# NUS-HPC-AI-Lab/VideoSys

Hardware: AMD Instinct MI355X
Metric: videos/min (Open-Sora 512x512x64f, 30 denoise steps, DiT denoising only) + sec/denoise-step (higher is better)
Workload: dtype bf16; 1 GPU; open-sora-v1.2 STDiT3-XL/2 512x512x64f, latent [4,19,64,64], CFG batch 2 = 38912 token rows, 300 text tokens, depth 28; steps_per_video=30, parallelism=dsp1

## Files before the change

### include/videosys_amd.h

```cpp
#ifndef VIDEOSYS_AMD_H
#define VIDEOSYS_AMD_H

#include <stdint.h>

#ifdef __cplusplus
extern "C" {
#endif

#define VSYS_ABI_VERSION 1

#define VSYS_ERR_SHAPE  (-1)
#define VSYS_ERR_ALIGN  (-2)
#define VSYS_ERR_ARG    (-3)
#define VSYS_ERR_LAUNCH (-4)

#define VSYS_EPI_BIAS      0
#define VSYS_EPI_BIAS_GELU 1
#define VSYS_EPI_GATE_RES  2

#define VSYS_ACT_NONE      0
#define VSYS_ACT_SILU      1
#define VSYS_ACT_GELU_TANH 2

int vsys_abi_version(void);
const char* vsys_strerror(int code);
int vsys_device_count(void);

int vsys_tune_gemm_variant(int variant);
int vsys_tune_flash_variant(int variant);
int vsys_gemm_raster_probe(int64_t tile, int64_t nbm, int64_t nbn, int64_t gw, int64_t ph, int64_t* bm, int64_t* bn);

int vsys_gemm_bf16(const void* x, int64_t ldx, const void* w, int64_t ldw, const void* bias, void* out, int64_t ldo,
                   int64_t M, int64_t N, int64_t K, int epilogue, const void* gate, int64_t gate_sample_stride,
                   int64_t rows_per_sample, const void* res, int64_t ldr, void* aux, int64_t ldaux, void* stream);

int vsys_gemm_bf16_ln(const void* x, int64_t ldx, const void* wp, int64_t ldw, const void* cs, const void* cv, void* out, int64_t ldo,
                      int64_t M, int64_t N, int64_t K, int epilogue, const void* stats, int64_t stats_ld, float eps, void* stream);

int vsys_gemm_bf16_ln_qkv_kv(const void* x, int64_t ldx, const void* wp, int64_t ldw, const void* cs, const void* cv, const void* stats,
                             int64_t stats_ld, const void* k_norm_w, void* q, int64_t ldq, void* kp, void* vt, int64_t M, int64_t K,
                             int64_t S, int64_t heads, float eps, float k_eps, void* stream);
int vsys_gemm_bf16_ln_qkv_kv_dispatched(int64_t M, int64_t N, int64_t K);

int vsys_gemm_bf16_stats(const void* x, int64_t ldx, const void* w, int64_t ldw, const void* bias, void* out, int64_t ldo, int64_t M,
                         int64_t N, int64_t K, const void* gate, int64_t gate_sample_stride, int64_t rows_per_sample, const void* res,
                         int64_t ldr, void* stats, int64_t stats_ld, void* stream);

int vsys_gemm_bf16_gate_res_add(const void* x, int64_t ldx, const void* w, int64_t ldw, const void* bias, void* out, int64_t ldo,
                                int64_t M, int64_t N, int64_t K, const void* gate, int64_t gate_sample_stride, int64_t rows_per_sample,
                                const void* res, int64_t ldr, void* aux, const void* add1, const void* add2, void* stats,
                                int64_t stats_ld, void* stream);

int vsys_adaln_prescale(const void* sites, int64_t nsites, int64_t nblocks, const void* mod, void* stream);

int vsys_ln_row_stats(const void* x, int64_t rows, int64_t C, void* stats, int64_t stats_ld, void* stream);

int vsys_linear_small(const void* x, int64_t ldx, const void* w, int64_t ldw, const void* bias, void* out, int64_t ldo,
                      int64_t M, int64_t N, int64_t K, int act_in, int act_out, void* stream);

int vsys_adaln_modulate(const void* x, const void* shift, const void* scale, void* y, int64_t rows, int64_t C,
                        int64_t rows_per_sample, int64_t mod_sample_stride, float eps, void* stream);

int vsys_mod_table(const void* table, const void* t_mlp, void* out, int64_t nblk, int64_t B, int64_t C6, void* stream);

int vsys_timestep_embedding(const void* t_f32, void* out, int64_t B, int64_t dim, void* stream);

int vsys_patch_embed(const void* z_f32, int64_t Bz, const void* w, const void* bias, const void* pos, void* out, int64_t B,
                     int64_t Cin, int64_t T, int64_t H, int64_t W, int64_t ph, int64_t pw, int64_t C, void* stream);

int vsys_final_layer(const void* x, const void* table, const void* tvec, const void* w, const void* bias, void* out_f32,
                     int64_t B, int64_t T, int64_t Hp, int64_t Wp, int64_t H, int64_t W, int64_t ph, int64_t pw,
                     int64_t Cout, int64_t C, float eps, void* stream);

int vsys_patch_embed_shard(const void* z_f32, int64_t Bz, const void* w, const void* bias, const void* pos, void* out, int64_t B,
                           int64_t Cin, int64_t T, int64_t H, int64_t W, int64_t ph, int64_t pw, int64_t C, int64_t s0, int64_t Sl,
                           void* stream);
int vsys_final_layer_tokens(const void* x, const void* table, const void* tvec, const void* w, const void* bias, void* tokens_f32,
                            int64_t B, int64_t T, int64_t Sl, int64_t n_out, int64_t C, float eps, void* stream);
int vsys_unpatchify_tokens(const void* tokens_f32, void* out_f32, int64_t P, int64_t B, int64_t T, int64_t Sl, int64_t Hp,
                           int64_t Wp, int64_t H, int64_t W, int64_t ph, int64_t pw, int64_t Cout, void* stream);

int vsys_cfg_euler_step(void* z_f32, const void* model_out_f32, int64_t Bz, int64_t Cin, int64_t Cout, int64_t thw,
                        float guidance, float dt, void* stream);

int vsys_cfg_linear_step(void* z_f32, const void* model_out_f32, int64_t Bz, int64_t Cin, int64_t Cout, int64_t thw,
                         float guidance, float c_z, float c_eps, int cond_first, void* stream);

int vsys_add_bcast_rows(void* x, const void* e, int64_t rows, int64_t C, int64_t group, int64_t period, void* stream);

int vsys_add_rows(void* x, const void* y, int64_t n, void* stream);

int vsys_copy_4d(const void* src, void* dst, int64_t n0, int64_t n1, int64_t n2, int64_t C, int64_t ss0, int64_t ss1,
                 int64_t ss2, int64_t ds0, int64_t ds1, int64_t ds2, int64_t n1_valid, int64_t n2_valid, void* stream);

// ... 252 lines not shown
```

### videosys_amd/_opcodes.py

```python
OPCODES = {
    "vsys_gemm_bf16": 1,
    "vsys_linear_small": 2,
    "vsys_adaln_modulate": 3,
    "vsys_mod_table": 4,
    "vsys_timestep_embedding": 5,
    "vsys_patch_embed": 6,
    "vsys_final_layer": 7,
    "vsys_cfg_euler_step": 8,
    "vsys_add_rows": 9,
    "vsys_copy_4d_batch": 10,
    "vsys_attn_prep_kv": 11,
    "vsys_flash_attn_d72": 12,
    "vsys_attn_temporal_d72": 13,
    "vsys_add_bcast_rows": 14,
    "vsys_gemm_bf16_gate2": 15,
    "vsys_ln_modulate": 16,
    "vsys_gate_add_rows": 17,
    "vsys_attn_prep_kv64": 18,
    "vsys_flash_attn_d64": 19,
    "vsys_patch_embed_shard": 20,
    "vsys_final_layer_tokens": 21,
    "vsys_unpatchify_tokens": 22,
    "vsys_gemm_bf16_ln": 23,
    "vsys_gemm_bf16_stats": 24,
    "vsys_adaln_prescale": 25,
    "vsys_ln_row_stats": 26,
    "vsys_gemm_bf16_gate_res_add": 27,
    "vsys_flash_attn_d72_kb": 28,
    "vsys_flash_attn_d64_kb": 29,
    "vsys_flash_attn_d72_exact": 30,
    "vsys_p2p_exchange": 31,
    "vsys_cfg_linear_step": 32,
    "vsys_copy_4d": 33,
    "vsys_im2col_patch": 34,
    "vsys_unpatchify_cvx": 35,
    "vsys_gather_rows": 36,
    "vsys_rms_norm_rows": 37,
    "vsys_geglu": 38,
    "vsys_splitk_reduce_t": 39,
    "vsys_t5_attention": 40,
    "vsys_gemm_skinny_slices": 41,
    "vsys_splitk_reduce": 42,
    "vsys_t5_attention_mfma": 43,
    "vsys_conv_bf16": 44,
    "vsys_gn_stats": 45,
    "vsys_gn_apply": 46,
    "vsys_regrid": 47,
    "vsys_subsample": 48,
    "vsys_spatial_norm_apply": 49,
    "vsys_blend_edge": 50,
    "vsys_d2s_time": 51,
    "vsys_vae_first_im2col": 52,
    "vsys_extract_planar": 53,
    "vsys_softmax_rows": 54,
    "vsys_attn_prep_kv_varlen": 55,
    "vsys_flash_attn_d72_varlen": 56,
    "vsys_gemm_bf16_ln_qkv_kv": 57,
    "vsys_attn_temporal_d64": 58,
    "vsys_scale_add_rows": 59,
}
N_INT, N_FLOAT = 23, 3
ENTRY_POINTS = {
    "vsys_abi_version": ("", "i"),
    "vsys_strerror": ("i", "s"),
    "vsys_device_count": ("", "i"),
    "vsys_tune_gemm_variant": ("i", "i"),
    "vsys_tune_flash_variant": ("i", "i"),
    "vsys_gemm_raster_probe": ("lllllpp", "i"),
    "vsys_gemm_bf16": ("plplppllllipllplplp", "i"),
    "vsys_gemm_bf16_ln": ("plplppplllliplfp", "i"),
    "vsys_gemm_bf16_ln_qkv_kv": ("plplppplpplppllllffp", "i"),
    "vsys_gemm_bf16_ln_qkv_kv_dispatched": ("lll", "i"),
    "vsys_gemm_bf16_stats": ("plplppllllpllplplp", "i"),
    "vsys_gemm_bf16_gate_res_add": ("plplppllllpllplpppplp", "i"),
    "vsys_adaln_prescale": ("pllpp", "i"),
    "vsys_ln_row_stats": ("pllplp", "i"),
    "vsys_linear_small": ("plplpplllliip", "i"),
    "vsys_adaln_modulate": ("ppppllllfp", "i"),
    "vsys_mod_table": ("ppplllp", "i"),
    "vsys_timestep_embedding": ("ppllp", "i"),
    "vsys_patch_embed": ("plppppllllllllp", "i"),
    "vsys_final_layer": ("ppppppllllllllllfp", "i"),
    "vsys_patch_embed_shard": ("plppppllllllllllp", "i"),
    "vsys_final_layer_tokens": ("pppppplllllfp", "i"),
    "vsys_unpatchify_tokens": ("pplllllllllllp", "i"),
    "vsys_cfg_euler_step": ("ppllllffp", "i"),
    "vsys_cfg_linear_step": ("ppllllfffip", "i"),
    "vsys_add_bcast_rows": ("ppllllp", "i"),
    "vsys_add_rows": ("pplp", "i"),
    "vsys_copy_4d": ("ppllllllllllllp", "i"),
    "vsys_attn_prep_kv": ("plplpppllllfp", "i"),
    "vsys_flash_attn_d72": ("plppppllllllfp", "i"),
    "vsys_flash_attn_d72_exact": ("plppppllllllfp", "i"),
    "vsys_attn_prep_kv_varlen": ("plplppppplllfp", "i"),
    "vsys_flash_attn_d72_varlen": ("plpppppplllllfp", "i"),
    "vsys_flash_attn_d72_kb": ("plppppllllllffp", "i"),
    "vsys_gemm_bf16_gate2": ("plplppllllpllllplplp", "i"),
    "vsys_ln_modulate": ("ppppppllllllfp", "i"),
    "vsys_gate_add_rows": ("pppllllllp", "i"),
    "vsys_im2col_patch": ("plpllllllp", "i"),
    "vsys_unpatchify_cvx": ("plpllllllp", "i"),
    "vsys_attn_prep_kv64": ("plplppppllppllllfp", "i"),
    "vsys_flash_attn_d64": ("plppppllpppllllllfp", "i"),
    "vsys_flash_attn_d64_kb": ("plppppllpppllllllffp", "i"),
    "vsys_attn_prep_kv96": ("plplppppllllp", "i"),
    "vsys_flash_attn_d96": ("plppppppllllllp", "i"),
    "vsys_attn_prep_kv96_img": ("plplppppllllllp", "i"),
    "vsys_flash_attn_d96_img": ("plpppppplllllllllp", "i"),
    "vsys_attn_prep_kv_rope": ("plplppppllllp", "i"),
    "vsys_flash_attn_d72_rope": ("plpppppllllllp", "i"),
    "vsys_attn_temporal_d72": ("pllppppplllllfp", "i"),
    "vsys_attn_temporal_d64": ("plplplplplplppplpllllllp", "i"),
    "vsys_attn_temporal_d64_img": ("plplplplplplppplplllllllllp", "i"),
    "vsys_scale_add_rows": ("plplplllfp", "i"),
    "vsys_copy_4d_batch": ("pplpp", "i"),
    "vsys_p2p_exchange": ("plppllplp", "i"),
    "vsys_p2p_alloc": ("llp", "i"),
    "vsys_p2p_free": ("p", "i"),
    "vsys_p2p_ipc_export": ("pp", "i"),
    "vsys_p2p_ipc_open": ("pp", "i"),
    "vsys_p2p_ipc_close": ("p", "i"),
    "vsys_gather_rows": ("ppplllp", "i"),
    "vsys_rms_norm_rows": ("pppllfp", "i"),
    "vsys_geglu": ("ppllp", "i"),
# ... 33 lines not shown
```

### videosys_amd/csrc/adaln_fold.hip

```cpp
#include "common.h"
#include "vsys_internal.h"

namespace vsys {
namespace {

constexpr int SITE_WORDS = 10;

__global__ __launch_bounds__(256) void adaln_prescale_kernel(const int64_t* __restrict__ sites, int nsites,
                                                             const bf16_t* __restrict__ mod) {
  const int lane = threadIdx.x & 63, wave = threadIdx.x >> 6;
  int lo = 0, hi = nsites - 1;
  while (lo < hi) {
    const int mid = (lo + hi + 1) >> 1;
    if (sites[(int64_t)mid * SITE_WORDS + 9] <= (int64_t)blockIdx.x) lo = mid;
    else hi = mid - 1;
  }
  const int64_t* s = sites + (int64_t)lo * SITE_WORDS;
  const bf16_t* W = reinterpret_cast<const bf16_t*>(s[0]);
  const bf16_t* bias = reinterpret_cast<const bf16_t*>(s[1]);
  bf16_t* Wp = reinterpret_cast<bf16_t*>(s[2]);
  float* cs = reinterpret_cast<float*>(s[3]);
  float* cv = reinterpret_cast<float*>(s[4]);
  const bf16_t* shift = mod + s[5];
  const bf16_t* scale = mod + s[6];
  const int N = (int)(s[7] & 0xffffffff), kv_heads = (int)(s[7] >> 32), K = (int)s[8];
  const int n = ((int)blockIdx.x - (int)s[9]) * 4 + wave;
  if (n >= N) return;
  const int nd = (kv_heads > 0 && N == 216 * kv_heads && kv_heads % 4 == 0) ? qkv_kv_column(n, kv_heads) : n;
  const bf16_t* wr = W + (int64_t)n * K;
  bf16_t* wo = Wp + (int64_t)nd * K;
  float a_cs = 0.f, a_cv = 0.f;
  for (int c = lane; c < (K >> 3); c += 64) {
    float w[8], sc[8], sh[8], o[8];
    unpack8(*reinterpret_cast<const uint4*>(wr + c * 8), w);
    unpack8(*reinterpret_cast<const uint4*>(scale + c * 8), sc);
    unpack8(*reinterpret_cast<const uint4*>(shift + c * 8), sh);
#pragma unroll
    for (int e = 0; e < 8; ++e) {
      o[e] = w[e] * (1.0f + sc[e]);
      a_cv = fmaf(sh[e], w[e], a_cv);
    }
    const uint4 pk = pack8(o);
    *reinterpret_cast<uint4*>(wo + c * 8) = pk;
    float r[8];
    unpack8(pk, r);
#pragma unroll
    for (int e = 0; e < 8; ++e) a_cs += r[e];
  }
  a_cs = wave_sum(a_cs);
  a_cv = wave_sum(a_cv);
  if (lane == 0) {
    cs[nd] = a_cs;
    cv[nd] = a_cv + (bias != nullptr ? bf2f(bias[n]) : 0.f);
  }
}

__global__ __launch_bounds__(256) void ln_row_stats_kernel(const bf16_t* __restrict__ x, int64_t rows, int C, float2* __restrict__ stats,
                                                           int64_t ld) {
  const int lane = threadIdx.x & 63;
  const int64_t row = ((int64_t)blockIdx.x * 4 + (threadIdx.x >> 6)) * 2 + (lane >> 5);
  const int q = lane & 31, b = q >> 1, hi = q & 1;
  const bool act = row < rows && b * LN_BLOCK < C;
  const bf16_t* xr = x + (act ? row : 0) * C + (act ? b : 0) * LN_BLOCK + 4 * hi;
  uint2 u[12];
#pragma unroll
  for (int j = 0; j < 3; ++j)
#pragma unroll
    for (int g = 0; g < 4; ++g) u[4 * j + g] = *reinterpret_cast<const uint2*>(xr + 32 * j + 8 * g);
  LnAcc a;
  a.init(bflo(u[0].x));
#pragma unroll
  for (int k = 0; k < 12; ++k) {
    a.add(bflo(u[k].x)); a.add(bfhi(u[k].x)); a.add(bflo(u[k].y)); a.add(bfhi(u[k].y));
  }
  const float2 mine = a.finish(48.f);
  const float2 other = make_float2(__shfl_xor(mine.x, 1, 64), __shfl_xor(mine.y, 1, 64));
  const float2 blk = ln_merge_equal(mine, other, 48.f);
  if (act && hi == 0) stats[(int64_t)b * ld + row] = blk;
}

}
// ... 17 lines not shown
```

### videosys_amd/csrc/attention.hip

```cpp
#include "common.h"
#include "vsys_internal.h"

#include <cstdlib>
#include <type_traits>

namespace vsys {
namespace {

constexpr int HD = 72;
constexpr int HD_ROWS = 96;
constexpr int KROW = 144;
constexpr int VROW = 128;
constexpr int K_TILE_BYTES = 64 * KROW;
constexpr int V_TILE_BYTES = HD_ROWS * VROW;
constexpr int KV_STAGE = K_TILE_BYTES + V_TILE_BYTES;
constexpr float NEG_BIG = -1.0e30f;

template <int N>
__device__ __forceinline__ void rope_pairs(float* x, const float* c, const float* s) {
#pragma clang fp contract(off)
#pragma unroll
  for (int e = 0; e < N; ++e) {
    const float a = x[2 * e], bb = x[2 * e + 1];
    const float ac = a * c[e], bs = bb * s[e], bc = bb * c[e], as = a * s[e];
// ... 50 lines not shown
    }
    KNorm72::apply(x, rstd, k_norm_w != nullptr ? k_norm_w + part * 24 : nullptr, kscale);
    if (active) {
      bf16_t* dst = kp + (((int64_t)bh * kv_pad) + s) * HD + part * 24;
#pragma unroll
      for (int c = 0; c < 3; ++c) *reinterpret_cast<uint4*>(dst + c * 8) = pack8(x + c * 8);
    }
  }
  __syncthreads();

  for (int q = tid; q < HD * 8; q += 256) {
    const int d = q >> 3, c = q & 7;
    uint4 o;
    uint32_t w[4];
#pragma unroll
    for (int e = 0; e < 4; ++e) w[e] = (uint32_t)vs[c * 8 + 2 * e][d] | ((uint32_t)vs[c * 8 + 2 * e + 1][d] << 16);
    o.x = w[0]; o.y = w[1]; o.z = w[2]; o.w = w[3];
    *reinterpret_cast<uint4*>(vt + ((int64_t)bh * HD_ROWS + d) * kv_pad + s0 + c * 8) = o;
  }
  if (tid < 16) {
    const int d = HD + 4 * (tid >> 3), c = tid & 7;
    uint32_t w[4];
#pragma unroll
    for (int e = 0; e < 4; ++e) {
      const int k0 = s0 + c * 8 + 2 * e;
      w[e] = (k0 < kv_len ? 0x3f80u : 0u) | (k0 + 1 < kv_len ? 0x3f800000u : 0u);
    }
    uint4 o;
    o.x = w[0]; o.y = w[1]; o.z = w[2]; o.w = w[3];
    *reinterpret_cast<uint4*>(vt + ((int64_t)bh * HD_ROWS + d) * kv_pad + s0 + c * 8) = o;
  }
}

struct FlashParams {
  const bf16_t* q; int64_t q_stride;
  union {
    const bf16_t* q_norm_w;
    const float* rope_cos;
  };
  const bf16_t* kp;
  const bf16_t* vt;
  bf16_t* out; int64_t out_stride;
  int heads, q_len, kv_len, kv_pad, nqb;
  int chunks;
  float eps;
  unsigned long long* dbg;
  union {
    const int* kv_lens;
    const float* rope_sin;
  };
};

constexpr int ABL_ROPE = 7;
constexpr int RES_MAX_TILES = 5;
constexpr int RES_Q_BYTES = 5 * 1024;
template <int ABL, int WPS, bool RES = false, bool EXACT = false, bool VARLEN = false>
__global__ __launch_bounds__(RES ? 512 : 256, RES ? 2 : WPS) void flash_attn_d72_kernel(FlashParams p) {
#if __HIP_DEVICE_COMPILE__
  extern __shared__ __attribute__((aligned(16))) char smem[];
  const int tid = threadIdx.x, lane = tid & 63, wave = tid >> 6;
  const int l31 = lane & 31, hi = lane >> 5;
  const int tile_id = xcd_remap(blockIdx.x, gridDim.x);
  const int bh = RES ? tile_id / p.chunks : tile_id / p.nqb;
  const int qb = RES ? tile_id - bh * p.chunks : tile_id - bh * p.nqb;
  const int b = bh / p.heads, h = bh - b * p.heads;
  constexpr int NW = RES ? 8 : 4;
  int q0 = qb * 128 + wave * 32;
  int kv_len_ = p.kv_len;
  if constexpr (VARLEN) {
    static_assert(RES && EXACT, "per-sample key counts: resident-K/V kernel with the padding promise only");
    const int cap = p.kv_pad < RES_MAX_TILES * 64 ? p.kv_pad : RES_MAX_TILES * 64;
    const int n = __builtin_amdgcn_readfirstlane(p.kv_lens[b]);
    kv_len_ = n < 1 ? 1 : (n > cap ? cap : n);
  }
  const int kv_len = kv_len_;

  const int wave_u = __builtin_amdgcn_readfirstlane(wave);
  const bf16_t* kbase = p.kp + (int64_t)bh * p.kv_pad * HD;
  const bf16_t* vbase = p.vt + (int64_t)bh * HD_ROWS * p.kv_pad;
  const auto rsrc_k = __builtin_amdgcn_make_buffer_rsrc((void*)kbase, 0, p.kv_pad * HD * 2, 0x00020000);
  const auto rsrc_v = __builtin_amdgcn_make_buffer_rsrc((void*)vbase, 0, HD_ROWS * p.kv_pad * 2, 0x00020000);
  typedef __attribute__((address_space(3))) void* lds_ptr_t;
  const int k_voff = lane * 16;
  const int v_voff = (lane >> 3) * p.kv_pad * 2 + (((lane & 7) ^ (lane >> 4)) << 4);
  const bool s4k = wave_u == 0;
  const int s4j = wave_u == 1 ? 8 : 9;
  const auto rsrc_4 = __builtin_amdgcn_make_buffer_rsrc((void*)(s4k ? kbase : vbase), 0, s4k ? p.kv_pad * HD * 2 : HD_ROWS * p.kv_pad * 2,
                                                        0x00020000);
  const int voff_4 = s4k ? k_voff : (v_voff ^ ((s4j & 1) << 6));
  const int soff_4 = s4k ? 8 * 1024 : s4j * 8 * p.kv_pad * 2, step_4 = s4k ? K_TILE_BYTES : 128;
  const int lds_4 = s4k ? 8 * 1024 : K_TILE_BYTES + s4j * 1024;
  auto stage = [&](int t, int buf) {
    char* base = smem + buf * KV_STAGE;
    if constexpr (RES) {
#pragma unroll
      for (int idx = 0; idx < 3; ++idx) {
        const int piece = wave_u + NW * idx;
        if (piece < 9) {
          __builtin_amdgcn_raw_ptr_buffer_load_lds(rsrc_k, (lds_ptr_t)(base + piece * 1024), 16, k_voff, t * K_TILE_BYTES + piece * 1024, 0, 0);
        } else if (piece < 19) {
          const int j = piece - 9;
          __builtin_amdgcn_raw_ptr_buffer_load_lds(rsrc_v, (lds_ptr_t)(base + K_TILE_BYTES + j * 1024), 16, v_voff ^ ((j & 1) << 6),
                                                   j * 8 * p.kv_pad * 2 + t * 128, 0, 0);
        }
      }
    } else {
// ... 12 lines not shown
    }
  };
  const int ntiles = (kv_len + 63) / 64;
  if constexpr (RES) {
    for (int t = 0; t < ntiles; ++t) stage(t, t);
    for (int q = tid; q < ntiles * 128; q += 512)
      *reinterpret_cast<uint4*>(smem + (q >> 7) * KV_STAGE + K_TILE_BYTES + 80 * VROW + (q & 127) * 16) = make_uint4(0, 0, 0, 0);
  } else {
    stage(0, 0);
    char* z = smem + (tid >> 7) * KV_STAGE + K_TILE_BYTES + 80 * VROW + (tid & 127) * 16;
    *reinterpret_cast<uint4*>(z) = make_uint4(0, 0, 0, 0);
  }

  bf16x8 qf[5];
  uint4 qraw[5];
  float4 qcs[5], qsn[5];
  auto fetch_q = [&](int q0_) {
    int qs = q0_ + l31;
    qs = qs < p.q_len ? qs : p.q_len - 1;
    const bf16_t* qrow = p.q + ((int64_t)b * p.q_len + qs) * p.q_stride + h * HD;
#pragma unroll
    for (int c = 0; c < 5; ++c) {
      const int d0 = 16 * c + 8 * hi;
      qraw[c] = d0 < HD ? *reinterpret_cast<const uint4*>(qrow + d0) : make_uint4(0, 0, 0, 0);
    }
    if constexpr (ABL == ABL_ROPE) {
      static_assert(ABL != ABL_ROPE || !RES, "the rotation lives in the streaming kernel's prologue only");
#pragma unroll
      for (int c = 0; c < 5; ++c) {
        const int d0 = 16 * c + 8 * hi;
        qcs[c] = qsn[c] = make_float4(0.f, 0.f, 0.f, 0.f);
        if (d0 < HD) {
          qcs[c] = *reinterpret_cast<const float4*>(p.rope_cos + (int64_t)qs * (HD / 2) + (d0 >> 1));
          qsn[c] = *reinterpret_cast<const float4*>(p.rope_sin + (int64_t)qs * (HD / 2) + (d0 >> 1));
        }
      }
    }
  };
  auto finish_q = [&]() {
    if constexpr (ABL == ABL_ROPE) {
#pragma unroll
      for (int c = 0; c < 5; ++c) {
        float x[8];
        unpack8(qraw[c], x);
        rope_pairs<1>(x + 0, &qcs[c].x, &qsn[c].x);
        rope_pairs<1>(x + 2, &qcs[c].y, &qsn[c].y);
        rope_pairs<1>(x + 4, &qcs[c].z, &qsn[c].z);
        rope_pairs<1>(x + 6, &qcs[c].w, &qsn[c].w);
#pragma unroll
        for (int e = 0; e < 8; ++e) qf[c][e] = (__bf16)x[e];
      }
      return;
    }
    if (p.q_norm_w == nullptr) {
#pragma unroll
      for (int c = 0; c < 5; ++c) qf[c] = __builtin_bit_cast(bf16x8, qraw[c]);
      return;
    }
    float x[5][8];
    float ss = 0.f;
#pragma unroll
    for (int c = 0; c < 5; ++c) {
      unpack8(qraw[c], x[c]);
#pragma unroll
      for (int e = 0; e < 8; ++e) ss += x[c][e] * x[c][e];
    }
    {
      ss += __shfl_xor(ss, 32, 64);
      const float rstd = rsqrtf(ss / (float)HD + p.eps);
#pragma unroll
      for (int c = 0; c < 5; ++c) {
        const int d0 = 16 * c + 8 * hi;
        if (d0 < HD) {
          float w[8];
          unpack8(*reinterpret_cast<const uint4*>(p.q_norm_w + d0), w);
#pragma unroll
          for (int e = 0; e < 8; ++e) x[c][e] = bf2f(f2bf(x[c][e] * rstd)) * w[e];
        }
      }
    }
#pragma unroll
    for (int c = 0; c < 5; ++c)
#pragma unroll
      for (int e = 0; e < 8; ++e) qf[c][e] = (__bf16)x[c][e];
  };
  if constexpr (!RES) { fetch_q(q0); finish_q(); }

  const int v_roff = K_TILE_BYTES + l31 * VROW + (((2 * hi) ^ ((l31 >> 1) & 7)) << 4);

  const int krow = 16 * ((l31 >> 2) & 1) + 4 * (l31 >> 3) + (l31 & 3);

  f32x16 o[3];
  f32x16 minit;
  auto reset_acc = [&]() {
#pragma unroll
    for (int dt = 0; dt < 3; ++dt)
#pragma unroll
      for (int r = 0; r < 16; ++r) o[dt][r] = 0.f;
#pragma unroll
    for (int r = 0; r < 16; ++r) minit[r] = 0.f;
  };
  reset_acc();
  asm volatile("s_waitcnt vmcnt(0)" ::: "memory");
  __syncthreads();

  const float defer_thr = 8.0f;

// ... 254 lines not shown
          for (int cc = 0; cc < 2; ++cc)
#pragma unroll
            for (int dt = 0; dt < 3; ++dt) o[dt] = __builtin_amdgcn_mfma_f32_32x32x16_bf16(vf1[cc][dt], pa1[cc], o[dt], 0, 0, 0);
          float mxn = 0.f;
          if constexpr (has_next) mxn = tile_max(t + 1, sn, next_masked);
#pragma unroll
          for (int i = 0; i < 6; ++i) { RES_SGB(0x008, 1); RES_SGB(0x400, 3); RES_SGB(0x002, 2); }
#pragma unroll
          for (int i = 0; i < 6; ++i) { RES_SGB(0x008, 1); RES_SGB(0x002, 5); }
          __builtin_amdgcn_sched_barrier(0);
          if constexpr (has_next) rescale(t + 1, sn, mxn);
        };
        qk(0, sa);
        __builtin_amdgcn_sched_barrier(0);
        next_q();
        __builtin_amdgcn_sched_barrier(0);
        rescale(0, sa, (ragged && ntiles == 1) ? tile_max(0, sa, true) : tile_max(0, sa, false));
        int t = 0;
        for (; t + 2 < ntiles; t += 2) {
          step(std::true_type{}, t, sa, sb, false);
          step(std::true_type{}, t + 1, sb, sa, ragged && t + 2 == ntiles - 1);
        }
        if (t + 1 < ntiles) {
          step(std::true_type{}, t, sa, sb, ragged);
          step(std::false_type{}, t + 1, sb, sa, false);
        } else {
          step(std::false_type{}, t, sa, sb, false);
        }
#undef RES_SGB
      }
      if constexpr (EXACT) {
        if (__builtin_amdgcn_ballot_w64(!(o[2][4] >= 0x1p-100f)) != 0) {
          asm volatile("; exact-keys guard (cold): masked recompute of this query block" ::: "memory");
          reset_acc();
          for (int t = 0; t < ntiles; ++t) tile(t, t, t == ntiles - 1 && (kv_len & 63) != 0);
        }
      }
      store_o();
    }
  } else {
    if (ABL == 2) tprev = __builtin_amdgcn_s_memtime();
    for (int t = 0; t < ntiles - 1; ++t) {
      const int cur = t & 1;
      if (ABL != 1 && ABL != 5 && !DMA_BESIDE_QK) stage(t + 1, cur ^ 1);
      __builtin_amdgcn_sched_barrier(0);
      tile(t, cur, false, true);
      __builtin_amdgcn_sched_barrier(0);
      if (ABL == 5) { __builtin_amdgcn_sched_barrier(0); continue; }
      asm volatile("s_waitcnt vmcnt(0)" ::: "memory");
      FLASH_STAMP(3);
      __syncthreads();
      FLASH_STAMP(4);
    }
    constexpr bool WHOLE_TILES_ONLY = ABL == ABL_ROPE && WPS == 3;
    if (!WHOLE_TILES_ONLY && (kv_len & 63)) tile(ntiles - 1, (ntiles - 1) & 1, true);
    else tile(ntiles - 1, (ntiles - 1) & 1, false);

    if (ABL == 2 && lane == 0 && p.dbg != nullptr) {
#pragma unroll
      for (int i = 0; i < 5; ++i) atomicAdd(p.dbg + i, tacc[i]);
    }
    store_o();
  }
#undef FLASH_STAMP
#endif
}

__global__ void attn_temporal_d72_kernel(const bf16_t* __restrict__ qkv, int64_t row_stride, int C,
                                         const bf16_t* __restrict__ q_norm_w, const bf16_t* __restrict__ k_norm_w,
                                         const float* __restrict__ rope_cos, const float* __restrict__ rope_sin,
                                         bf16_t* __restrict__ out, int64_t out_stride, int B, int T, int S, int heads,
                                         int wpb, float eps, float scale) {
  extern __shared__ __attribute__((aligned(16))) char smem[];
  const int lane = threadIdx.x & 63, wave = threadIdx.x >> 6;
  const int hgroups = (heads + wpb - 1) / wpb;
  const int hg = blockIdx.x % hgroups;
  const int64_t bs = blockIdx.x / hgroups;
  const int s = (int)(bs % S), b = (int)(bs / S);
  const int h = hg * wpb + wave;
  if (h >= heads) return;
  float* ks = reinterpret_cast<float*>(smem) + (size_t)wave * 2 * T * HD;
  float* vs = ks + (size_t)T * HD;
  const int g = lane / 3, part = lane - g * 3;
  const bool lane_ok = lane < 63;
  const int npass = (T + 20) / 21;

  auto norm_rope = [&](float* x, const bf16_t* w, int t) {
    float ss = 0.f;
#pragma unroll
    for (int e = 0; e < 24; ++e) ss += x[e] * x[e];
    const int base = g * 3;
    const float tot = __shfl(ss, base, 64) + __shfl(ss, base + 1, 64) + __shfl(ss, base + 2, 64);
    const float rstd = rsqrtf(tot / (float)HD + eps);
    if (w != nullptr) {
#pragma unroll
      for (int e = 0; e < 24; ++e) x[e] = bf2f(f2bf(bf2f(f2bf(x[e] * rstd)) * bf2f(w[part * 24 + e])));
    }
    if (rope_cos != nullptr) {
      const float* cs = rope_cos + (int64_t)t * HD + part * 24;
      const float* sn = rope_sin + (int64_t)t * HD + part * 24;
#pragma unroll
      for (int e = 0; e < 24; e += 2) {
        const float a = x[e], bb = x[e + 1];
        x[e] = bf2f(f2bf(a * cs[e] - bb * sn[e]));
        x[e + 1] = bf2f(f2bf(bb * cs[e + 1] + a * sn[e + 1]));
      }
    }
// ... 487 lines not shown
  const size_t lds = per_wave * wpb;
  const float scale = 0.11785113019775793f;
  const int g_flash_variant = g_flash_variant_a.load(std::memory_order_relaxed);
  if (T <= 64 && g_flash_variant != 9 && g_flash_variant != 4)
    return launch_attn_temporal_d72_v3(qkv, row_stride, C, q_norm_w, k_norm_w, rope_cos, rope_sin, out, out_stride, B, T, S, heads, eps,
                                       scale, stream,  g_flash_variant == 21,  g_flash_variant == 22);
  if (T <= 20 && g_flash_variant != 9) {
    hipLaunchKernelGGL(attn_temporal_d72_v2_kernel<20>, dim3((unsigned)grid), dim3(64 * wpb), lds, stream, qkv, row_stride, C, q_norm_w,
                       k_norm_w, rope_cos, rope_sin, out, out_stride, B, T, S, heads, wpb, eps, scale);
  } else if (T <= 40 && g_flash_variant != 9) {
    hipLaunchKernelGGL(attn_temporal_d72_v2_kernel<40>, dim3((unsigned)grid), dim3(64 * wpb), lds, stream, qkv, row_stride, C, q_norm_w,
                       k_norm_w, rope_cos, rope_sin, out, out_stride, B, T, S, heads, wpb, eps, scale);
  } else {
    if (lds > 64 * 1024)
      (void)hipFuncSetAttribute((const void*)attn_temporal_d72_kernel, hipFuncAttributeMaxDynamicSharedMemorySize, (int)lds);
    hipLaunchKernelGGL(attn_temporal_d72_kernel, dim3((unsigned)grid), dim3(64 * wpb), lds, stream, qkv, row_stride, C, q_norm_w,
                       k_norm_w, rope_cos, rope_sin, out, out_stride, B, T, S, heads, wpb, eps, scale);
  }
  return hipGetLastError() == hipSuccess ? 0 : VSYS_ERR_LAUNCH;
}

int launch_attn_prep_kv_rope(const bf16_t* k, int64_t k_stride, const bf16_t* v, int64_t v_stride, const float* rope_cos,
                             const float* rope_sin, bf16_t* kp, bf16_t* vt, int batch, int heads, int kv_len, int kv_pad,
                             hipStream_t stream) {
  if (batch <= 0 || heads <= 0 || kv_len <= 0) return 0;
  if (kv_pad % 64 != 0 || kv_pad < kv_len || (k_stride % 8) || (v_stride % 8)) return VSYS_ERR_SHAPE;
  dim3 grid(kv_pad / 64, batch * heads);
  hipLaunchKernelGGL(attn_prep_kv_rope_kernel<false>, grid, dim3(256), 0, stream, k, k_stride, v, v_stride, rope_cos, rope_sin, kp, vt,
                     heads, kv_len, kv_pad, 0.11785113019775793f * 1.4426950408889634f );
  return hipGetLastError() == hipSuccess ? 0 : VSYS_ERR_LAUNCH;
}

int launch_flash_attn_d72_rope(const bf16_t* q, int64_t q_stride, const float* rope_cos, const float* rope_sin, const bf16_t* kp,
                               const bf16_t* vt, bf16_t* out, int64_t out_stride, int batch, int heads, int q_len, int kv_len,
                               int kv_pad, hipStream_t stream) {
  if (batch <= 0 || heads <= 0 || q_len <= 0) return 0;
  if (kv_len <= 0 || kv_pad % 64 != 0 || kv_pad < kv_len || (q_stride % 8) || (out_stride % 4)) return VSYS_ERR_SHAPE;
  FlashParams p;
  p.q = q; p.q_stride = q_stride; p.rope_cos = rope_cos; p.kp = kp; p.vt = vt; p.out = out; p.out_stride = out_stride;
  p.heads = heads; p.q_len = q_len; p.kv_len = kv_len; p.kv_pad = kv_pad; p.eps = 0.f;
  p.rope_sin = rope_sin;
  p.dbg = nullptr;
  p.nqb = (q_len + 127) / 128;
  p.chunks = 1;
  const int64_t nblk = (int64_t)p.nqb * batch * heads;
  if (nblk > 0x7fffffff) return VSYS_ERR_SHAPE;
  const size_t lds = 2 * KV_STAGE;
  static const bool wps3_ok = [] { const char* e = getenv("VSYS_FLASH_WPS3"); return !(e && e[0] == '0'); }();
  if (wps3_ok && kv_len >= 512 && (kv_len & 63) == 0) hipLaunchKernelGGL((flash_attn_d72_kernel<ABL_ROPE, 3>), dim3((unsigned)nblk), dim3(256), lds, stream, p);
  else hipLaunchKernelGGL((flash_attn_d72_kernel<ABL_ROPE, 2>), dim3((unsigned)nblk), dim3(256), lds, stream, p);
  return hipGetLastError() == hipSuccess ? 0 : VSYS_ERR_LAUNCH;
}

}
```

### videosys_amd/csrc/attention_w64.hip

```cpp
#include "flash_w64.h"

namespace vsys {
namespace {

using w64::VROW;
using w64::make_rsrc;
using w64::u32x4;
constexpr int HD = 72, HD_ROWS = 96, KROW = 144;
constexpr int K_TILE_BYTES = 64 * KROW;
constexpr int KV_STAGE = K_TILE_BYTES + HD_ROWS * VROW;
constexpr int W64_STAGES = w64::STAGES;

struct FlashW64Params {
  const bf16_t* q; int64_t q_stride;
  const bf16_t* q_norm_w;
  const bf16_t* kp;
  const bf16_t* vt;
  bf16_t* out; int64_t out_stride;
  int heads, q_len, kv_len, kv_pad, nqb;
  float eps;
  float k_bound;
  unsigned long long* dbg;
};

// ... 95 lines not shown
  else if constexpr (VAR == 10)
    asm volatile(FLASH72_W64_ASM_V10 : W64_STAMPS : FLASH72_W64_OPERANDS : FLASH72_W64_CLOBBERS_PHASE);
  else if constexpr (VAR == 8) W64_LOOP(FLASH72_W64_ASM_V8);
  else if constexpr (VAR == 9) W64_LOOP(FLASH72_W64_ASM_V9);
#endif
#undef W64_STAMPS
#undef W64_LOOP

#pragma unroll
  for (int blk = 0; blk < 2; ++blk) {
    float o[3][16];
    if (blk == 0) FLASH72_W64_READ_O_A(o);
    else FLASH72_W64_READ_O_B(o);
    const float inv = 1.0f / o[2][4];
    const int qs = q0 + 32 * blk + l31;
    bf16_t* orow = p.out + ((int64_t)b * p.q_len + (qs < p.q_len ? qs : p.q_len - 1)) * p.out_stride + h * HD + 8 * hi;
#pragma unroll
    for (int dt = 0; dt < 3; ++dt) {
      uint2 w[4];
#pragma unroll
      for (int g = 0; g < 4; ++g) {
        w[g].x = pack2bf(o[dt][4 * g + 0] * inv, o[dt][4 * g + 1] * inv);
        w[g].y = pack2bf(o[dt][4 * g + 2] * inv, o[dt][4 * g + 3] * inv);
      }
#pragma unroll
      for (int k = 0; k < 2; ++k) {
        const auto sx = __builtin_amdgcn_permlane32_swap(w[2 * k].x, w[2 * k + 1].x, false, false);
        const auto sy = __builtin_amdgcn_permlane32_swap(w[2 * k].y, w[2 * k + 1].y, false, false);
        const int d0 = dt * 32 + 16 * k;
        if (qs < p.q_len && d0 + 8 * hi + 8 <= HD) *reinterpret_cast<uint4*>(orow + d0) = make_uint4(sx[0], sy[0], sx[1], sy[1]);
      }
    }
  }
  if constexpr (VAR == 7 || VAR == 10) {
    asm volatile("s_waitcnt vmcnt(0)" ::: "memory");
    stamp[5] = __builtin_amdgcn_s_memtime();
    if (lane == 0 && p.dbg != nullptr) {
      unsigned long long* d = p.dbg + ((size_t)blockIdx.x * 4 + wave) * 8;
#pragma unroll
      for (int i = 0; i < 6; ++i) d[i] = stamp[i];
    }
  }
#endif
}

constexpr int W64P_QIMG = 64 * KROW;

__device__ __forceinline__ unsigned long long uniform_addr(const void* ptr) {
  const unsigned long long a = reinterpret_cast<unsigned long long>(ptr);
  const unsigned lo = __builtin_amdgcn_readfirstlane((unsigned)a), hi_ = __builtin_amdgcn_readfirstlane((unsigned)(a >> 32) & 0xffffu);
  return ((unsigned long long)hi_ << 32) | lo;
}

template <bool STAMP, bool SM = false>
__global__ __launch_bounds__(256, 1) void flash_attn_d72_w64p_kernel(FlashW64Params p, int total_items) {
#if __HIP_DEVICE_COMPILE__
  extern __shared__ __attribute__((aligned(16))) char smem[];
  const int tid = threadIdx.x, lane = tid & 63, wave = tid >> 6;
  const int l31 = lane & 31, hi = lane >> 5;
  const int wave_u = __builtin_amdgcn_readfirstlane(wave);
  const int wgp = xcd_remap(blockIdx.x, gridDim.x), istep = (int)gridDim.x;
  const int i0 = wgp, i1 = total_items;
  if (i0 >= i1) return;

  const unsigned kbytes = (unsigned)(p.kv_pad * HD * 2), vbytes = (unsigned)(HD_ROWS * p.kv_pad * 2);
  const bool s4k = wave_u == 0;
  const int s4j = wave_u == 1 ? 8 : 9;
  const int kvo = lane * 16;
  const int v_voff0 = (lane >> 3) * p.kv_pad * 2 + (((lane & 7) ^ (lane >> 4)) << 4);
  const int vvo = v_voff0 ^ ((wave_u & 1) << 6);
  const int v4o = s4k ? kvo : (v_voff0 ^ ((s4j & 1) << 6));
  const int wl = wave_u * 1024, kvp2 = p.kv_pad * 2;
  const int s4 = s4k ? 8 * 1024 : s4j * 8 * p.kv_pad * 2, st4 = s4k ? K_TILE_BYTES : 128;
  const int l4 = s4k ? 8 * 1024 : K_TILE_BYTES + s4j * 1024;
  const int lb = w64::lds_base(smem);
  const int qlds = lb + W64_STAGES * KV_STAGE + wave_u * W64P_QIMG;
  const int nt = p.kv_len >> 6;
  for (int u = tid; u < W64_STAGES * 128; u += 256)
    *reinterpret_cast<uint4*>(smem + (u >> 7) * KV_STAGE + K_TILE_BYTES + 80 * VROW + (u & 127) * 16) = make_uint4(0, 0, 0, 0);
  const int kfa = w64::frag_krow(l31) * KROW + 16 * hi;
  const w64::VtFrag vf = w64::vt_frag<K_TILE_BYTES>(l31, hi);
  const int vfa0 = vf.vfa0, vfa1 = vf.vfa1, vfa2 = vf.vfa2, vfa3 = vf.vfa3;

  auto item_bh = [&](int it) { return it / p.nqb; };
  auto q_rsrc = [&](int it) {
    const int bh = item_bh(it), b = bh / p.heads, h = bh - b * p.heads;
    return make_rsrc(p.q + (int64_t)b * p.q_len * p.q_stride + h * HD, (unsigned)((int64_t)p.q_len * p.q_stride * 2));
  };
  auto q_row_voff = [&](int it) {
    const int qb = it - item_bh(it) * p.nqb;
    int r = qb * 256 + wave * 64 + lane;
    r = r < p.q_len ? r : p.q_len - 1;
    return r * (int)p.q_stride * 2;
  };
  typedef __attribute__((address_space(3))) void* lds_ptr_t;

  {
    const int bh = item_bh(i0);
    const bf16_t* kbase = p.kp + (int64_t)bh * p.kv_pad * HD;
    const bf16_t* vbase = p.vt + (int64_t)bh * HD_ROWS * p.kv_pad;
    const auto rk = __builtin_amdgcn_make_buffer_rsrc((void*)kbase, 0, (int)kbytes, 0x00020000);
    const auto rv = __builtin_amdgcn_make_buffer_rsrc((void*)vbase, 0, (int)vbytes, 0x00020000);
    const int bq = bh / p.heads, hq = bh - bq * p.heads;
    const auto rq = __builtin_amdgcn_make_buffer_rsrc((void*)(p.q + (int64_t)bq * p.q_len * p.q_stride + hq * HD), 0,
                                                      (int)((int64_t)p.q_len * p.q_stride * 2), 0x00020000);
    const int qv = q_row_voff(i0);
#pragma unroll
    for (int pc = 0; pc < 9; ++pc)
      __builtin_amdgcn_raw_ptr_buffer_load_lds(rq, (lds_ptr_t)(smem + W64_STAGES * KV_STAGE + wave_u * W64P_QIMG + pc * 1024), 16, qv, pc * 16, 0, 0);
#pragma unroll
    for (int t = 0; t < 4; ++t) {
      char* st = smem + t * KV_STAGE;
      __builtin_amdgcn_raw_ptr_buffer_load_lds(rk, (lds_ptr_t)(st + wl), 16, kvo, t * K_TILE_BYTES + wl, 0, 0);
      __builtin_amdgcn_raw_ptr_buffer_load_lds(rk, (lds_ptr_t)(st + wl + 4096), 16, kvo, t * K_TILE_BYTES + wl + 4096, 0, 0);
      __builtin_amdgcn_raw_ptr_buffer_load_lds(rv, (lds_ptr_t)(st + K_TILE_BYTES + wl), 16, vvo, wave_u * 8 * kvp2 + t * 128, 0, 0);
      __builtin_amdgcn_raw_ptr_buffer_load_lds(rv, (lds_ptr_t)(st + K_TILE_BYTES + wl + 4096), 16, vvo, (wave_u + 4) * 8 * kvp2 + t * 128, 0, 0);
      if (s4k) __builtin_amdgcn_raw_ptr_buffer_load_lds(rk, (lds_ptr_t)(st + l4), 16, v4o, s4 + t * st4, 0, 0);
      else __builtin_amdgcn_raw_ptr_buffer_load_lds(rv, (lds_ptr_t)(st + l4), 16, v4o, s4 + t * st4, 0, 0);
    }
  }

  uint4 qnw[5];
#pragma unroll
  for (int c = 0; c < 5; ++c) {
    const int d0 = 16 * c + 8 * hi;
    qnw[c] = (p.q_norm_w != nullptr && d0 < HD) ? *reinterpret_cast<const uint4*>(p.q_norm_w + d0) : make_uint4(0, 0, 0, 0);
  }
  unsigned long long acc[8] = {0, 0, 0, 0, 0, 0, 0, 0}, ta = 0, tb = 0;
  int ring = 0;
  for (int it = i0; it < i1; it += istep) {
    const int bh = item_bh(it), qb = it - bh * p.nqb;
    const int b = bh / p.heads, h = bh - b * p.heads;
    const int q0 = qb * 256 + wave_u * 64;
    unsigned long long t0 = 0, t1 = 0, t2 = 0, t3 = 0, t4 = 0;
    if constexpr (STAMP) t0 = __builtin_amdgcn_s_memtime();
    asm volatile("s_waitcnt vmcnt(0)" ::: "memory");
    if constexpr (STAMP) t1 = __builtin_amdgcn_s_memtime();
    uint4 qw[2][5];
    float nmv[2] = {0.f, 0.f};
#pragma unroll
    for (int blk = 0; blk < 2; ++blk) {
      const char* qimg = smem + W64_STAGES * KV_STAGE + wave_u * W64P_QIMG + (32 * blk + l31) * 16;
      uint4 qraw[5];
#pragma unroll
      for (int c = 0; c < 5; ++c) {
        const int ch = 2 * c + hi;
        qraw[c] = ch < 9 ? *reinterpret_cast<const uint4*>(qimg + ch * 1024) : make_uint4(0, 0, 0, 0);
      }
      float x[5][8];
      float ss = 0.f;
#pragma unroll
      for (int c = 0; c < 5; ++c) {
        unpack8(qraw[c], x[c]);
#pragma unroll
        for (int e = 0; e < 8; ++e) ss += x[c][e] * x[c][e];
      }
      if (p.q_norm_w != nullptr) {
        ss += __shfl_xor(ss, 32, 64);
        const float rstd = rsqrtf(ss / (float)HD + p.eps);
#pragma unroll
        for (int c = 0; c < 5; ++c) {
          const int d0 = 16 * c + 8 * hi;
          if (d0 < HD) {
            float w[8];
            unpack8(qnw[c], w);
#pragma unroll
            for (int e = 0; e < 8; ++e) x[c][e] = bf2f(f2bf(x[c][e] * rstd)) * w[e];
          }
        }
      }
      if constexpr (SM) nmv[blk] = w64::neg_row_bound<5>(x, p.k_bound);
#pragma unroll
      for (int c = 0; c < 5; ++c) qw[blk][c] = pack8(x[c]);
    }
    asm volatile("s_waitcnt lgkmcnt(0)" ::: "memory");
    FLASH72_W64_WRITE_Q_A(qw[0]);
    FLASH72_W64_WRITE_Q_B(qw[1]);
    const float nma = nmv[0], nmb = nmv[1];

    const bool has_next = it + istep < i1;
    const int nit = has_next ? it + istep : it;
    const int nbh = item_bh(nit);
    const unsigned long long kb = uniform_addr(p.kp + (int64_t)bh * p.kv_pad * HD), vb = uniform_addr(p.vt + (int64_t)bh * HD_ROWS * p.kv_pad);
    const unsigned long long kbn = uniform_addr(p.kp + (int64_t)nbh * p.kv_pad * HD), vbn = uniform_addr(p.vt + (int64_t)nbh * HD_ROWS * p.kv_pad);
    const u32x4 rqn = q_rsrc(nit);
    const int qvo = q_row_voff(nit);
    const int hn = __builtin_amdgcn_readfirstlane(has_next ? 1 : 0);
    const int st0 = lb + ring * KV_STAGE, st1 = lb + ((ring + 1) & 3) * KV_STAGE, st2 = lb + ((ring + 2) & 3) * KV_STAGE;
    ring = (ring + nt) & 3;
    if constexpr (STAMP) {
      t2 = __builtin_amdgcn_s_memtime();
#ifdef VSYS_LAB
      asm volatile(FLASH72_W64P_ASM_STAMP : [t0] "=s"(ta), [t1] "=s"(tb) : FLASH72_W64P_OPERANDS : FLASH72_W64_CLOBBERS);
#endif
      t3 = __builtin_amdgcn_s_memtime();
    } else if constexpr (SM)
      asm volatile(FLASH72_W64P_ASM_S : : FLASH72_W64P_OPERANDS_S : FLASH72_W64_CLOBBERS);
    else
      asm volatile(FLASH72_W64P_ASM : : FLASH72_W64P_OPERANDS : FLASH72_W64_CLOBBERS);

// ... 62 lines not shown
  return p;
}

bool flash_w64p_supports(int q_len, int kv_len, int kv_pad, int64_t q_stride) {
  return kv_len >= 256 && kv_len % 64 == 0 && q_len >= 256 && (int64_t)q_len * q_stride * 2 < 0x7fffffff;
}

int launch_flash_attn_d72_w64p(const bf16_t* q, int64_t q_stride, const bf16_t* q_norm_w, const bf16_t* kp, const bf16_t* vt, bf16_t* out,
                               int64_t out_stride, int batch, int heads, int q_len, int kv_len, int kv_pad, float eps, bool stamp,
                               float k_bound, hipStream_t stream) {
  FlashW64Params p = w64_params(q, q_stride, q_norm_w, kp, vt, out, out_stride, heads, q_len, kv_len, kv_pad, eps, k_bound, nullptr);
  const int64_t total = (int64_t)p.nqb * batch * heads;
  if (total > 0x7fffffff) return VSYS_ERR_SHAPE;
  const int ncu = cu_count_this_device();
  const unsigned grid = (unsigned)(total < ncu ? total : ncu);
  const size_t lds = (size_t)W64_STAGES * KV_STAGE + 4 * W64P_QIMG;
  (void)stamp;
#ifdef VSYS_LAB
  if (!stamp)
#endif
    return !(k_bound > 0.f && q_norm_w != nullptr) ? w64::launch<flash_attn_d72_w64p_kernel<false>>(grid, lds, stream, p, (int)total)
                                                    : w64::launch<flash_attn_d72_w64p_kernel<false, true>>(grid, lds, stream, p, (int)total);
#ifdef VSYS_LAB
  p.dbg = reinterpret_cast<unsigned long long*>(get_lab_debug_buffer());
  return w64::launch<flash_attn_d72_w64p_kernel<true>>(grid, lds, stream, p, (int)total);
#endif
}

int launch_flash_attn_d72_w64(const bf16_t* q, int64_t q_stride, const bf16_t* q_norm_w, const bf16_t* kp, const bf16_t* vt, bf16_t* out,
                              int64_t out_stride, int batch, int heads, int q_len, int kv_len, int kv_pad, float eps, int var,
                              float k_bound, hipStream_t stream) {
  const FlashW64Params p = w64_params(q, q_stride, q_norm_w, kp, vt, out, out_stride, heads, q_len, kv_len, kv_pad, eps, k_bound,
                                      reinterpret_cast<unsigned long long*>(get_lab_debug_buffer()));
  const int64_t nblk = (int64_t)p.nqb * batch * heads;
  if (nblk > 0x7fffffff) return VSYS_ERR_SHAPE;
  const size_t lds = (size_t)W64_STAGES * KV_STAGE;
#define W64_CASE(VAR_) w64::launch<flash_attn_d72_w64_kernel<VAR_>>((unsigned)nblk, lds, stream, p)
  switch (var) {
    case 0: return W64_CASE(0);
    case 1: return W64_CASE(1);
    case 3: return W64_CASE(3);
    case 5: return k_bound > 0.f && q_norm_w != nullptr ? W64_CASE(5) : VSYS_ERR_ARG;
#ifdef VSYS_LAB
    case 7: return W64_CASE(7);
    case 10: return W64_CASE(10);
    case 8: return W64_CASE(8);
    case 9: return W64_CASE(9);
#endif
    default: return VSYS_ERR_ARG;
  }
#undef W64_CASE
}

}
```

### videosys_amd/csrc/capi.hip

```cpp
#include "common.h"
#include "vsys_internal.h"

using namespace vsys;

namespace {
inline hipStream_t S(void* s) { return reinterpret_cast<hipStream_t>(s); }
inline const bf16_t* B16(const void* p) { return reinterpret_cast<const bf16_t*>(p); }
inline bf16_t* B16(void* p) { return reinterpret_cast<bf16_t*>(p); }
template <class... T> inline bool fits_int(T... v) { return ((v >= 0 && v <= 0x7fffffff) && ...); }
inline GemmParams gemm_head(const void* a, int64_t lda, const void* w, int64_t ldw, const void* bias, void* out, int64_t ldo, int64_t M,
                            int64_t N, int64_t K) {
  GemmParams p;
  p.A = B16(a); p.lda = lda; p.W = B16(w); p.ldw = ldw; p.bias = B16(bias); p.out = B16(out); p.ldo = ldo;
  p.M = (int)M; p.N = (int)N; p.K = (int)K;
  return p;
}

inline bool to_copy_desc(const int64_t* d, CopyDesc& o) {
  if (!fits_int(d[2], d[3], d[4], d[5], d[12], d[13]) || d[0] < 0 || d[1] < 0) return false;
  o.src_off = d[0]; o.dst_off = d[1];
  o.n0 = (int)d[2]; o.n1 = (int)d[3]; o.n2 = (int)d[4]; o.C = (int)d[5];
  o.ss0 = d[6]; o.ss1 = d[7]; o.ss2 = d[8]; o.ds0 = d[9]; o.ds1 = d[10]; o.ds2 = d[11];
  o.n1_valid = (int)d[12]; o.n2_valid = (int)d[13];
  return true;
// ... 78 lines not shown
  std::vector<int4> v;
  int m = 0;
  if (!sk_plan(ntiles, nt, grid, v, m)) return 0;
  if ((int)v.size() > cap_rows) return VSYS_ERR_ARG;
  for (size_t i = 0; i < v.size(); ++i) {
    segs[4 * i] = v[i].x; segs[4 * i + 1] = v[i].y; segs[4 * i + 2] = v[i].z; segs[4 * i + 3] = v[i].w;
  }
  *nseg_max = m;
  return (int)v.size();
}

int vsys_lab_flash_debug_buffer(void* dev_u64x5) {
  set_flash_debug_buffer(dev_u64x5);
  return 0;
}
#endif

int vsys_gemm_bf16(const void* x, int64_t ldx, const void* w, int64_t ldw, const void* bias, void* out, int64_t ldo,
                   int64_t M, int64_t N, int64_t K, int epilogue, const void* gate, int64_t gate_sample_stride,
                   int64_t rows_per_sample, const void* res, int64_t ldr, void* aux, int64_t ldaux, void* stream) {
  if (!x || !w || !out) return VSYS_ERR_ARG;
  if (!fits_int(M, N, K, rows_per_sample)) return VSYS_ERR_SHAPE;
  if (epilogue != VSYS_EPI_GATE_RES && (gate || res || aux)) return VSYS_ERR_ARG;
  GemmParams p = gemm_head(x, ldx, w, ldw, bias, out, ldo, M, N, K);
  p.gate = B16(gate); p.gate_stride = gate_sample_stride; p.res = B16(res); p.ldr = ldr; p.aux = B16(aux); p.ldaux = ldaux;
  p.rows_per_sample = (int)rows_per_sample;
  return launch_gemm(p, epilogue, S(stream));
}

int vsys_gemm_bf16_ln(const void* x, int64_t ldx, const void* wp, int64_t ldw, const void* cs, const void* cv, void* out, int64_t ldo,
                      int64_t M, int64_t N, int64_t K, int epilogue, const void* stats, int64_t stats_ld, float eps, void* stream) {
  if (!x || !wp || !cs || !cv || !out || !stats) return VSYS_ERR_ARG;
  if (!fits_int(M, N, K)) return VSYS_ERR_SHAPE;
  if (epilogue != VSYS_EPI_BIAS && epilogue != VSYS_EPI_BIAS_GELU) return VSYS_ERR_ARG;
  if (K % LN_BLOCK != 0 || K / LN_BLOCK > 12) return VSYS_ERR_SHAPE;
  GemmParams p = gemm_head(x, ldx, wp, ldw, nullptr, out, ldo, M, N, K);
  p.cs = reinterpret_cast<const float*>(cs); p.cv = reinterpret_cast<const float*>(cv);
  p.ln_stats = reinterpret_cast<const float2*>(stats); p.ln_ld = stats_ld; p.ln_nb = (int)(K / LN_BLOCK); p.ln_eps = eps;
  return launch_gemm(p, epilogue == VSYS_EPI_BIAS ? EPI_LN_BIAS : EPI_LN_GELU, S(stream));
}

int vsys_gemm_bf16_ln_qkv_kv(const void* x, int64_t ldx, const void* wp, int64_t ldw, const void* cs, const void* cv, const void* stats,
                             int64_t stats_ld, const void* k_norm_w, void* q, int64_t ldq, void* kp, void* vt, int64_t M, int64_t K,
                             int64_t S_, int64_t heads, float eps, float k_eps, void* stream) {
  if (!x || !wp || !cs || !cv || !stats || !k_norm_w || !q || !kp || !vt) return VSYS_ERR_ARG;
  if (!fits_int(M, K, S_) || heads <= 0 || heads > 4096) return VSYS_ERR_SHAPE;
  if (K % LN_BLOCK != 0 || K / LN_BLOCK > 12) return VSYS_ERR_SHAPE;
  GemmParams p = gemm_head(x, ldx, wp, ldw, nullptr, q, ldq, M, 216 * heads, K);
  p.cs = reinterpret_cast<const float*>(cs); p.cv = reinterpret_cast<const float*>(cv);
  p.ln_stats = reinterpret_cast<const float2*>(stats); p.ln_ld = stats_ld; p.ln_nb = (int)(K / LN_BLOCK); p.ln_eps = eps;
  p.kp = B16(kp); p.vt = B16(vt); p.k_norm_w = B16(k_norm_w); p.kv_S = (int)S_; p.kv_heads = (int)heads; p.k_eps = k_eps;
  p.kscale = 0.11785113019775793f * 1.4426950408889634f;
  return launch_gemm_qkv_kv(p, S(stream));
}

int vsys_gemm_bf16_ln_qkv_kv_dispatched(int64_t M, int64_t N, int64_t K) { return gemm_ln_qkv_kv_dispatched(M, N, K) ? 1 : 0; }

int vsys_gemm_bf16_stats(const void* x, int64_t ldx, const void* w, int64_t ldw, const void* bias, void* out, int64_t ldo, int64_t M,
                         int64_t N, int64_t K, const void* gate, int64_t gate_sample_stride, int64_t rows_per_sample, const void* res,
                         int64_t ldr, void* stats, int64_t stats_ld, void* stream) {
  if (!x || !w || !out || !stats) return VSYS_ERR_ARG;
  if (!fits_int(M, N, K, rows_per_sample)) return VSYS_ERR_SHAPE;
  GemmParams p = gemm_head(x, ldx, w, ldw, bias, out, ldo, M, N, K);
  p.gate = B16(gate); p.gate_stride = gate_sample_stride; p.res = B16(res); p.ldr = ldr;
  p.rows_per_sample = (int)rows_per_sample;
  p.stats_out = reinterpret_cast<float2*>(stats); p.stats_ld = stats_ld;
  return launch_gemm(p, EPI_GATE_RES_STATS, S(stream));
}

int vsys_gemm_bf16_gate_res_add(const void* x, int64_t ldx, const void* w, int64_t ldw, const void* bias, void* out, int64_t ldo,
                                int64_t M, int64_t N, int64_t K, const void* gate, int64_t gate_sample_stride, int64_t rows_per_sample,
                                const void* res, int64_t ldr, void* aux, const void* add1, const void* add2, void* stats,
                                int64_t stats_ld, void* stream) {
  if (!x || !w || !out || !res) return VSYS_ERR_ARG;
  if (!fits_int(M, N, K, rows_per_sample)) return VSYS_ERR_SHAPE;
  GemmParams p = gemm_head(x, ldx, w, ldw, bias, out, ldo, M, N, K);
  p.gate = B16(gate); p.gate_stride = gate_sample_stride; p.res = B16(res); p.ldr = ldr; p.aux = B16(aux); p.ldaux = ldr;
  p.rows_per_sample = (int)rows_per_sample;
  p.add1 = B16(add1 ? add1 : add2); p.add2 = add1 ? B16(add2) : nullptr;
  p.stats_out = reinterpret_cast<float2*>(stats); p.stats_ld = stats_ld;
  return launch_gemm(p, EPI_GATE_RES, S(stream));
}

int vsys_adaln_prescale(const void* sites, int64_t nsites, int64_t nblocks, const void* mod, void* stream) {
  if (!sites || !mod) return VSYS_ERR_ARG;
  if (!fits_int(nsites)) return VSYS_ERR_SHAPE;
  return launch_adaln_prescale(reinterpret_cast<const int64_t*>(sites), (int)nsites, nblocks, B16(mod), S(stream));
}

int vsys_ln_row_stats(const void* x, int64_t rows, int64_t C, void* stats, int64_t stats_ld, void* stream) {
  if (!x || !stats) return VSYS_ERR_ARG;
  if (!fits_int(C)) return VSYS_ERR_SHAPE;
  return launch_ln_row_stats(B16(x), rows, (int)C, reinterpret_cast<float2*>(stats), stats_ld, S(stream));
}

int vsys_gemm_bf16_gate2(const void* x, int64_t ldx, const void* w, int64_t ldw, const void* bias, void* out, int64_t ldo,
                         int64_t M, int64_t N, int64_t K, const void* gate, int64_t gate_sample_stride,
                         int64_t rows_per_sample, int64_t seg_split, int64_t gate_alt, const void* res, int64_t ldr,
                         void* aux, int64_t ldaux, void* stream) {
  if (!x || !w || !out || !gate) return VSYS_ERR_ARG;
  if (!fits_int(M, N, K, rows_per_sample, seg_split)) return VSYS_ERR_SHAPE;
  if (seg_split < 0 || seg_split > rows_per_sample) return VSYS_ERR_SHAPE;
  GemmParams p = gemm_head(x, ldx, w, ldw, bias, out, ldo, M, N, K);
  p.gate = B16(gate); p.gate_stride = gate_sample_stride; p.res = B16(res); p.ldr = ldr; p.aux = B16(aux); p.ldaux = ldaux;
  p.rows_per_sample = (int)rows_per_sample;
  p.seg_split = (int)seg_split; p.gate_alt = gate_alt;
// ... 642 lines not shown
```

### videosys_amd/csrc/common.h

```cpp
#pragma once
#include <hip/hip_runtime.h>
#include <stdint.h>

namespace vsys {

typedef uint16_t bf16_t;
typedef __attribute__((ext_vector_type(8))) __bf16 bf16x8;
typedef __attribute__((ext_vector_type(4))) __bf16 bf16x4;
typedef __attribute__((ext_vector_type(16))) float f32x16;
typedef __attribute__((ext_vector_type(4))) float f32x4;

__device__ __forceinline__ float bf2f(bf16_t v) { return __uint_as_float(((uint32_t)v) << 16); }
__device__ __forceinline__ bf16_t f2bf(float f) { return __builtin_bit_cast(bf16_t, (__bf16)f); }
__device__ __forceinline__ uint32_t pack2bf(float lo, float hi) {
  return (uint32_t)f2bf(lo) | ((uint32_t)f2bf(hi) << 16);
}
typedef __attribute__((ext_vector_type(2))) float f32x2;
typedef __attribute__((ext_vector_type(2))) __bf16 bf16x2;
__device__ __forceinline__ uint32_t pack2bf(f32x2 v) { return __builtin_bit_cast(uint32_t, __builtin_convertvector(v, bf16x2)); }
__device__ __forceinline__ float bflo(uint32_t u) { return __uint_as_float(u << 16); }
__device__ __forceinline__ float bfhi(uint32_t u) { return __uint_as_float(u & 0xffff0000u); }

__device__ __forceinline__ void unpack8(const uint4& v, float* f) {
  f[0] = bflo(v.x); f[1] = bfhi(v.x); f[2] = bflo(v.y); f[3] = bfhi(v.y);
  f[4] = bflo(v.z); f[5] = bfhi(v.z); f[6] = bflo(v.w); f[7] = bfhi(v.w);
}
__device__ __forceinline__ uint4 pack8(const float* f) {
  uint4 v;
  v.x = pack2bf(f[0], f[1]); v.y = pack2bf(f[2], f[3]); v.z = pack2bf(f[4], f[5]); v.w = pack2bf(f[6], f[7]);
  return v;
}

__device__ __forceinline__ float wave_sum(float v) {
#pragma unroll
  for (int o = 32; o > 0; o >>= 1) v += __shfl_xor(v, o, 64);
  return v;
}
__device__ __forceinline__ float wave_max(float v) {
#pragma unroll
  for (int o = 32; o > 0; o >>= 1) v = fmaxf(v, __shfl_xor(v, o, 64));
  return v;
}

__device__ __forceinline__ float gelu_tanh(float x) {
  const float k0 = 0.7978845608028654f, k1 = 0.044715f;
  const float u = k0 * x * (1.0f + k1 * x * x);
  const float e = __builtin_amdgcn_exp2f(u * -2.8853900817779268f);
  return x * __builtin_amdgcn_rcpf(1.0f + e);
}
__device__ __forceinline__ float silu(float x) { return x / (1.0f + __expf(-x)); }

struct KNorm72 {
  static __device__ __forceinline__ float sumsq(const float* x) {
    float ss = 0.f;
#pragma unroll
    for (int e = 0; e < 24; ++e) ss += x[e] * x[e];
    return ss;
  }
  static __device__ __forceinline__ float rstd(float ss0, float ss1, float ss2, float eps) {
    const float tot = ss0 + ss1 + ss2;
    return rsqrtf(tot / 72.0f + eps);
  }
  static __device__ __forceinline__ void apply(float* x, float rstd_, const bf16_t* w24, float kscale) {
    if (w24 != nullptr) {
#pragma unroll
      for (int e = 0; e < 24; ++e) {
        const float nrm = bf2f(f2bf(x[e] * rstd_));
        x[e] = nrm * bf2f(w24[e]);
      }
    }
#pragma unroll
    for (int e = 0; e < 24; ++e) x[e] *= kscale;
  }
};

__device__ __forceinline__ void ln_combine(const float2* __restrict__ st, int64_t ld, int nb, int64_t row, float eps, float& mu,
                                           float& rstd) {
  float2 v[12];
#pragma unroll
  for (int b = 0; b < 12; ++b) v[b] = b < nb ? st[b * ld + row] : make_float2(0.f, 0.f);
  float sd = 0.f, sdd = 0.f, m2 = v[0].y;
#pragma unroll
  for (int b = 1; b < 12; ++b) {
    if (b < nb) {
      const float d = v[b].x - v[0].x;
      sd += d;
      sdd += d * d;
      m2 += v[b].y;
    }
  }
  const float inv = 1.0f / (float)nb;
  mu = v[0].x + sd * inv;
  m2 += 96.0f * (sdd - sd * sd * inv);
  rstd = rsqrtf(fmaxf(m2, 0.f) / (96.0f * (float)nb) + eps);
}
__device__ __forceinline__ void ln_stage_tile(float2* __restrict__ lds, const float2* __restrict__ st, int64_t ld, int nb, float eps,
                                              int M, int row0, int nrows, const float* __restrict__ cs, const float* __restrict__ cv,
                                              int col0, int ncols, int tid, int nthreads) {
  const int c = nthreads - 1 - tid;
  float c_s = 0.f, c_v = 0.f;
  if (c < ncols) {
    c_s = cs[col0 + c];
    c_v = cv[col0 + c];
  }
  if (tid < nrows) {
    int grow = row0 + tid;
    grow = grow < M ? grow : M - 1;
    float mu, rstd;
    ln_combine(st, ld, nb, grow, eps, mu, rstd);
    lds[tid] = make_float2(mu, rstd);
  }
  if (c < ncols) lds[nrows + c] = make_float2(c_s, c_v);
}

struct LnAcc {
  float p, s1, s2;
  __device__ __forceinline__ void init(float pivot) { p = pivot; s1 = 0.f; s2 = 0.f; }
  __device__ __forceinline__ void add(float x) { const float d = x - p; s1 += d; s2 = fmaf(d, d, s2); }
  __device__ __forceinline__ void add2(f32x2 x) {
    const f32x2 d = x - f32x2{p, p};
    s1 += d.x; s2 = fmaf(d.x, d.x, s2);
    s1 += d.y; s2 = fmaf(d.y, d.y, s2);
  }
  __device__ __forceinline__ float2 finish(float n) const { return make_float2(p + s1 / n, fmaxf(s2 - s1 * s1 / n, 0.f)); }
};
// ... 52 lines not shown
```

### videosys_amd/csrc/gemm2_bf16.hip

```cpp
#include "common.h"
#include "vsys_internal.h"

namespace vsys {
namespace {

constexpr int BM = 256, BK = 32;
constexpr int A_SLOT = BM * BK * 2;
constexpr int W_BASE = 3 * A_SLOT;
constexpr int OUT_ROW_BYTES = 96 * 2 + 16;
constexpr int OUT_WAVE_BYTES = 64 * OUT_ROW_BYTES;

template <int NWN>
struct G2 {
  static constexpr int NW = 2 * NWN;
  static constexpr int NT = 64 * NW;
  static constexpr int BN = 96 * NWN;
  static constexpr int NA = 16 / NW;
  static constexpr int W_SLOT = BN * BK * 2;
  static constexpr int WLEAD = NWN == 4 ? 2 : 1;
  static constexpr int NWSLOT = WLEAD + 1;
  static constexpr int STAGING = W_BASE + NWSLOT * W_SLOT;
  static constexpr int LDS_BYTES = STAGING > NW * OUT_WAVE_BYTES ? STAGING : NW * OUT_WAVE_BYTES;
  static constexpr int LN_BYTES = (BM + BN) * 8;
  static constexpr int KW_BYTES = 160;
};

template <int EPI, int NWN, int STAMP = 0, int MF = 0>
__global__ __launch_bounds__(G2<NWN>::NT, 2) void gemm2_kernel(GemmParams p) {
  using G = G2<NWN>;
  constexpr int BN = G::BN, NA = G::NA, W_SLOT = G::W_SLOT, WLEAD = G::WLEAD;
#if __HIP_DEVICE_COMPILE__
  extern __shared__ __attribute__((aligned(16))) char smem[];
  const int tid = threadIdx.x, lane = tid & 63, wave = tid >> 6;
  const int wm = wave / NWN, wn = wave % NWN;
  const int l31 = lane & 31, hi = lane >> 5;
  const int l15 = lane & 15, lq = lane >> 4;
  static_assert(!MF || (EPI != EPI_F32_SLICES && !STAMP), "the 16x16x32 form covers the token-row epilogues only");
  static_assert(EPI != EPI_LN_QKV_KV || (MF && NWN == 2), "the K/V epilogue exists on the 256 x 192 tile of the 16x16x32 form only");
  const int wave_u = __builtin_amdgcn_readfirstlane(wave);
  const int nbn = p.N / BN;
  int tile = xcd_remap(blockIdx.x, gridDim.x);
  int kslice = 0;
  if constexpr (EPI == EPI_F32_SLICES) {
    const int ntile = ((p.M + BM - 1) / BM) * nbn;
    kslice = tile / ntile;
    tile -= kslice * ntile;
  }
  int bm, bn;
  gemm_raster(tile, (p.M + BM - 1) / BM, nbn, p.raster_gw, p.raster_ph, bm, bn);
  const int row0 = bm * BM, col0 = bn * BN;

  const int dchunk = ((lane & 3) ^ (MF ? ((0x78 >> (2 * ((lane >> 4) & 3))) & 3) : ((lane >> 4) & 3))) * 16;
  int a_off[NA], b_off[3];
#pragma unroll
  for (int i = 0; i < NA; ++i) {
    const int r = wave_u * (16 * NA) + i * 16 + (lane >> 2);
    const int rl = row0 + r < p.M ? r : p.M - 1 - row0;
    a_off[i] = rl * (int)p.lda * 2 + dchunk;
  }
#pragma unroll
  for (int i = 0; i < 3; ++i) b_off[i] = (wave_u * 48 + i * 16 + (lane >> 2)) * (int)p.ldw * 2 + dchunk;
  const int64_t a_bytes = ((int64_t)(p.M - 1 - row0) * p.lda + p.K) * 2, b_bytes = ((int64_t)(p.N - 1 - col0) * p.ldw + p.K) * 2;
  const auto rsrc_a = __builtin_amdgcn_make_buffer_rsrc((void*)(p.A + (int64_t)row0 * p.lda), 0,
                                                        (int)(a_bytes < 0x7fffffff ? a_bytes : 0x7fffffff), 0x00020000);
  const auto rsrc_b = __builtin_amdgcn_make_buffer_rsrc((void*)(p.W + (int64_t)col0 * p.ldw), 0,
                                                        (int)(b_bytes < 0x7fffffff ? b_bytes : 0x7fffffff), 0x00020000);
  typedef __attribute__((address_space(3))) void* lds_ptr_t;
  const int kbase2 = EPI == EPI_F32_SLICES ? kslice * p.ks * 2 : 0;
  auto dma_a = [&](int i, int t, int slot) {
    __builtin_amdgcn_raw_ptr_buffer_load_lds(rsrc_a, (lds_ptr_t)(smem + slot * A_SLOT + (wave_u * (16 * NA) + i * 16) * 64), 16, a_off[i],
                                             kbase2 + t * (BK * 2), 0, 0);
  };
  auto dma_w = [&](int i, int t, int slot) {
    __builtin_amdgcn_raw_ptr_buffer_load_lds(rsrc_b, (lds_ptr_t)(smem + W_BASE + slot * W_SLOT + (wave_u * 48 + i * 16) * 64), 16,
                                             b_off[i], kbase2 + t * (BK * 2), 0, 0);
  };

  const int fsw = MF ? ((lq ^ ((0x78 >> (2 * ((l15 >> 2) & 3))) & 3)) << 4) : ((hi ^ ((l31 >> 2) & 3)) << 4);
  const int frow = MF ? l15 : l31;
  const int xo = (wm * 128 + frow) * 64 + fsw;
  const int wo = W_BASE + (wn * 96 + frow) * 64 + fsw;

  f32x16 acc[MF ? 1 : 4][MF ? 1 : 3];
  f32x4 acc16[MF ? 8 : 1][MF ? 6 : 1];
#pragma unroll
  for (int i = 0; i < (MF ? 1 : 4); ++i)
#pragma unroll
    for (int j = 0; j < (MF ? 1 : 3); ++j)
#pragma unroll
      for (int r = 0; r < 16; ++r) acc[i][j][r] = 0.f;
#pragma unroll
  for (int i = 0; i < (MF ? 8 : 1); ++i)
#pragma unroll
    for (int j = 0; j < (MF ? 6 : 1); ++j)
#pragma unroll
      for (int r = 0; r < 4; ++r) acc16[i][j][r] = 0.f;

  constexpr bool LN = EPI == EPI_LN_BIAS || EPI == EPI_LN_GELU || EPI == EPI_LN_QKV_KV;
  float2* ln_lds = reinterpret_cast<float2*>(smem + G::LDS_BYTES);
  const int nt = (EPI == EPI_F32_SLICES ? (p.ks < p.K - kslice * p.ks ? p.ks : p.K - kslice * p.ks) : p.K) / BK;
#pragma unroll
  for (int i = 0; i < NA; ++i) dma_a(i, 0, 0);
#pragma unroll
  for (int i = 0; i < 3; ++i) dma_w(i, 0, 0);
  if (nt > 1) {
#pragma unroll
    for (int i = 0; i < NA; ++i) dma_a(i, 1, 1);
    if constexpr (WLEAD == 2) {
#pragma unroll
      for (int i = 0; i < 3; ++i) dma_w(i, 1, 1);
    }
  }
  if constexpr (LN) {
    __builtin_amdgcn_sched_barrier(0);
    ln_stage_tile(ln_lds, p.ln_stats, p.ln_ld, p.ln_nb, p.ln_eps, p.M, row0, BM, p.cs, p.cv, col0, BN, tid, G::NT);
    if constexpr (EPI == EPI_LN_QKV_KV) {
      if (tid < 9) *reinterpret_cast<uint4*>(smem + G::LDS_BYTES + G::LN_BYTES + tid * 16) = *reinterpret_cast<const uint4*>(p.k_norm_w + tid * 8);
    }
    __builtin_amdgcn_sched_barrier(0);
  }
  if (nt > 1) {
    if constexpr (WLEAD == 2) {
      asm volatile("s_waitcnt vmcnt(5)" ::: "memory");
    } else if constexpr (NA == 4) {
      asm volatile("s_waitcnt vmcnt(4)" ::: "memory");
    } else {
      asm volatile("s_waitcnt vmcnt(2)" ::: "memory");
    }
  } else {
    asm volatile("s_waitcnt vmcnt(0)" ::: "memory");
  }
  if constexpr (LN) asm volatile("s_waitcnt lgkmcnt(0)" ::: "memory");
  __builtin_amdgcn_sched_barrier(0);
  __builtin_amdgcn_s_barrier();
  __builtin_amdgcn_sched_barrier(0);

  int sa = 0, sw = 0;
  uint64_t st_read = 0, st_mfma = 0, st_wait = 0, st_bar = 0, st_t0 = 0, st_begin = 0;
  if constexpr (STAMP) { st_begin = __builtin_amdgcn_s_memtime(); st_t0 = st_begin; }
  for (int t = 0; t < nt; ++t) {
    const int sa1 = sa == 2 ? 0 : sa + 1, sa2 = sa1 == 2 ? 0 : sa1 + 1;
    const int sw1 = WLEAD == 2 ? sa1 : (sw ^ 1);
    const int swn = WLEAD == 2 ? sa2 : sw1;
    const int tw = t + WLEAD;
    const bool n2 = t + 2 < nt;
    const bool n1 = WLEAD == 2 ? n2 : (t + 1 < nt);
    const char* ab = smem + sa * A_SLOT;
    const char* wb = smem + sw * W_SLOT;
    bf16x8 x0, x1, x2, x3, w0, w1, w2, v0, v1, v2;
    if constexpr (MF) {
      x0 = *reinterpret_cast<const bf16x8*>(ab + xo);
      w0 = *reinterpret_cast<const bf16x8*>(wb + wo);
      w1 = *reinterpret_cast<const bf16x8*>(wb + wo + 1024);
      w2 = *reinterpret_cast<const bf16x8*>(wb + wo + 2048);
      v0 = *reinterpret_cast<const bf16x8*>(wb + wo + 3072);
      v1 = *reinterpret_cast<const bf16x8*>(wb + wo + 4096);
      v2 = *reinterpret_cast<const bf16x8*>(wb + wo + 5120);
      x1 = *reinterpret_cast<const bf16x8*>(ab + xo + 1024);
      x2 = *reinterpret_cast<const bf16x8*>(ab + xo + 2048);
      x3 = *reinterpret_cast<const bf16x8*>(ab + xo + 3072);
      __builtin_amdgcn_sched_barrier(0);
#define G16_ROW(i_, X_)                                                                                \
  acc16[i_][0] = __builtin_amdgcn_mfma_f32_16x16x32_bf16(w0, X_, acc16[i_][0], 0, 0, 0);               \
  acc16[i_][1] = __builtin_amdgcn_mfma_f32_16x16x32_bf16(w1, X_, acc16[i_][1], 0, 0, 0);               \
  acc16[i_][2] = __builtin_amdgcn_mfma_f32_16x16x32_bf16(w2, X_, acc16[i_][2], 0, 0, 0);               \
  acc16[i_][3] = __builtin_amdgcn_mfma_f32_16x16x32_bf16(v0, X_, acc16[i_][3], 0, 0, 0);               \
  acc16[i_][4] = __builtin_amdgcn_mfma_f32_16x16x32_bf16(v1, X_, acc16[i_][4], 0, 0, 0);               \
  acc16[i_][5] = __builtin_amdgcn_mfma_f32_16x16x32_bf16(v2, X_, acc16[i_][5], 0, 0, 0)
      G16_ROW(0, x0);
      __builtin_amdgcn_sched_barrier(0);
// ... 326 lines not shown
        gate_row = p.gate + (int64_t)sample * p.gate_stride + ncol0 + 4 * hi;
        if (p.seg_split > 0 && grow - sample * p.rows_per_sample < p.seg_split) gate_row += p.gate_alt;
      }
#pragma unroll
      for (int j = 0; j < 3; ++j) {
        uint2 gg[4];
        if (EPI == EPI_GATE_RES) {
#pragma unroll
          for (int g = 0; g < 4; ++g) gg[g] = make_uint2(0x3f803f80u, 0x3f803f80u);
          if (gate_row != nullptr) {
#pragma unroll
            for (int g = 0; g < 4; ++g) gg[g] = *reinterpret_cast<const uint2*>(gate_row + j * 32 + 8 * g);
          }
        }
#pragma unroll
        for (int g = 0; g < 4; ++g) {
          const int n_local = j * 32 + 8 * g + 4 * hi;
          float v[4];
#pragma unroll
          for (int r = 0; r < 4; ++r) v[r] = acc[i][j][4 * g + r];
          v[0] += bflo(bb[j][g].x); v[1] += bfhi(bb[j][g].x); v[2] += bflo(bb[j][g].y); v[3] += bfhi(bb[j][g].y);
          if (EPI == EPI_BIAS_GELU) {
#pragma unroll
            for (int r = 0; r < 4; ++r) v[r] = gelu_tanh(v[r]);
          }
          if (EPI == EPI_GATE_RES) {
            v[0] *= bflo(gg[g].x); v[1] *= bfhi(gg[g].x); v[2] *= bflo(gg[g].y); v[3] *= bfhi(gg[g].y);
          }
          uint2 o;
          o.x = pack2bf(v[0], v[1]);
          o.y = pack2bf(v[2], v[3]);
          *reinterpret_cast<uint2*>(st + m_local * OUT_ROW_BYTES + n_local * 2) = o;
        }
      }
    }
    }
    uint4 rres[12];
    if (EPI == EPI_GATE_RES && !MF) {
#pragma unroll
      for (int it = 0; it < 12; ++it) rres[it] = make_uint4(0, 0, 0, 0);
      if (p.res != nullptr) {
#pragma unroll
        for (int it = 0; it < 12; ++it) {
          const int q = lane + 64 * it;
          const int m_local = q / 12, c = q - m_local * 12;
          int grow = wrow0 + m_local;
          grow = grow < p.M ? grow : p.M - 1;
          rres[it] = *reinterpret_cast<const uint4*>(p.res + (int64_t)grow * p.ldr + ncol0 + c * 8);
        }
      }
    }
    asm volatile("s_waitcnt lgkmcnt(0)" ::: "memory");
    __builtin_amdgcn_wave_barrier();
    if constexpr (EPI == EPI_LN_QKV_KV) {
      const int H = p.kv_heads, nq = (H * 3) >> 2;
      const int win = __builtin_amdgcn_readfirstlane(ncol0 / 96);
      if (win >= nq) {
        if (wrow0 < p.M) {
          const int bt = __builtin_amdgcn_readfirstlane(wrow0 / p.kv_S), key0 = __builtin_amdgcn_readfirstlane(wrow0 - bt * p.kv_S);
          int vf0 = 24 * H + 96 * (win - nq - H);
          if (win < nq + H) {
            const int h = win - nq;
            vf0 = 24 * h;
            char* rowp = st + lane * OUT_ROW_BYTES;
            const uint4* wl = reinterpret_cast<const uint4*>(smem + G::LDS_BYTES + G::LN_BYTES);
            uint4 kk[9];
#pragma unroll
            for (int c = 0; c < 9; ++c) kk[c] = *reinterpret_cast<const uint4*>(rowp + c * 16);
            float ss[3];
#pragma unroll
            for (int part = 0; part < 3; ++part) {
              float x[24];
#pragma unroll
              for (int c = 0; c < 3; ++c) unpack8(kk[part * 3 + c], x + c * 8);
              ss[part] = KNorm72::sumsq(x);
            }
            const float rstd = KNorm72::rstd(ss[0], ss[1], ss[2], p.k_eps);
#pragma unroll
            for (int part = 0; part < 3; ++part) {
              float x[24];
              union { uint4 u[3]; bf16_t w[24]; } kw;
#pragma unroll
              for (int c = 0; c < 3; ++c) {
                unpack8(kk[part * 3 + c], x + c * 8);
                kw.u[c] = wl[part * 3 + c];
              }
              KNorm72::apply(x, rstd, kw.w, p.kscale);
#pragma unroll
              for (int c = 0; c < 3; ++c) *reinterpret_cast<uint4*>(rowp + (part * 3 + c) * 16) = pack8(x + c * 8);
            }
            asm volatile("s_waitcnt lgkmcnt(0)" ::: "memory");
            __builtin_amdgcn_wave_barrier();
            bf16_t* kdst = p.kp + (((int64_t)bt * H + h) * p.kv_S + key0) * 72;
            uint4 kq[9];
#pragma unroll
            for (int it = 0; it < 9; ++it) {
              const int q = lane + 64 * it;
              const int m_local = q / 9, c = q - m_local * 9;
              kq[it] = *reinterpret_cast<const uint4*>(st + m_local * OUT_ROW_BYTES + c * 16);
            }
#pragma unroll
            for (int it = 0; it < 9; ++it) *reinterpret_cast<uint4*>(kdst + (lane + 64 * it) * 8) = kq[it];
          }
          const bool kwin = win < nq + H;
          bf16_t* vdst = p.vt + (int64_t)bt * H * 96 * p.kv_S + key0;
#pragma unroll
          for (int g = 0; g < 3; ++g) {
            uint4 o[4];
            int64_t off[4];
#pragma unroll
            for (int k = 0; k < 4; ++k) {
              const int it = g * 4 + k;
              if (kwin && it >= 3) continue;
              int col, c;
              if (kwin) {
                const int q = lane + 64 * it;
                c = q / 24;
                col = q - c * 24;
              } else {
                col = (it >> 2) * 32 + (lane & 31);
                c = 2 * (it & 3) + (lane >> 5);
              }
              const int f = vf0 + col, hv = f / 72, d = f - hv * 72;
              off[k] = ((int64_t)hv * 96 + d) * p.kv_S + c * 8;
              const char* src = st + (c * 8) * OUT_ROW_BYTES + ((kwin ? 72 : 0) + col) * 2;
              uint32_t w[4];
#pragma unroll
              for (int e = 0; e < 4; ++e)
                w[e] = (uint32_t)*reinterpret_cast<const uint16_t*>(src + (2 * e) * OUT_ROW_BYTES) |
                       ((uint32_t)*reinterpret_cast<const uint16_t*>(src + (2 * e + 1) * OUT_ROW_BYTES) << 16);
              o[k] = make_uint4(w[0], w[1], w[2], w[3]);
            }
#pragma unroll
            for (int k = 0; k < 4; ++k)
              if (!(kwin && g * 4 + k >= 3)) *reinterpret_cast<uint4*>(vdst + off[k]) = o[k];
            if (kwin) break;
          }
        }
        asm volatile("s_waitcnt lgkmcnt(0)" ::: "memory");
        __builtin_amdgcn_wave_barrier();
        continue;
      }
    }
    uint4 val[12];
#pragma unroll
    for (int it = 0; it < 12; ++it) {
      const int q = lane + 64 * it;
      const int m_local = q / 12, c = q - m_local * 12;
      val[it] = *reinterpret_cast<const uint4*>(st + m_local * OUT_ROW_BYTES + c * 16);
    }
#pragma unroll
    for (int it = 0; it < 12; ++it) {
      const int q = lane + 64 * it;
      const int m_local = q / 12, c = q - m_local * 12;
      const int64_t grow = wrow0 + m_local;
      const int gcol = ncol0 + c * 8;
      const bool ok = full || grow < p.M;
// ... 12 lines not shown
      if (ok) *reinterpret_cast<uint4*>(p.out + grow * p.ldo + gcol) = v;
    }
    asm volatile("s_waitcnt lgkmcnt(0)" ::: "memory");
    __builtin_amdgcn_wave_barrier();
  }
  if constexpr (STAMP) {
    if (lane == 0 && p.aux != nullptr) {
      int64_t* d = reinterpret_cast<int64_t*>(p.aux) + ((int64_t)blockIdx.x * G::NW + wave) * 8;
      const uint64_t end = __builtin_amdgcn_s_memtime();
      d[0] = (int64_t)st_read; d[1] = (int64_t)st_mfma; d[2] = (int64_t)st_wait; d[3] = (int64_t)st_bar;
      d[4] = (int64_t)(st_t0 - st_begin); d[5] = (int64_t)(end - st_t0); d[6] = (int64_t)st_begin; d[7] = nt;
    }
  }
#endif
}

}

template <int NWN, int MF = 0>
static int launch_gemm2_t(const GemmParams& p, int epi, hipStream_t stream) {
  using G = G2<NWN>;
  if (p.N % G::BN != 0) return VSYS_ERR_SHAPE;
  const int nbm = (p.M + BM - 1) / BM, nbn = p.N / G::BN;
  const int grid = nbm * nbn;
  static std::atomic<unsigned long long> attr_seen{0};
  for (DeviceOnce once(attr_seen); once.todo(); once.done()) {
    (void)hipFuncSetAttribute((const void*)gemm2_kernel<EPI_BIAS, NWN, 0, MF>, hipFuncAttributeMaxDynamicSharedMemorySize, G::LDS_BYTES);
    (void)hipFuncSetAttribute((const void*)gemm2_kernel<EPI_BIAS_GELU, NWN, 0, MF>, hipFuncAttributeMaxDynamicSharedMemorySize, G::LDS_BYTES);
    (void)hipFuncSetAttribute((const void*)gemm2_kernel<EPI_GATE_RES, NWN, 0, MF>, hipFuncAttributeMaxDynamicSharedMemorySize, G::LDS_BYTES);
    (void)hipFuncSetAttribute((const void*)gemm2_kernel<EPI_LN_BIAS, NWN, 0, MF>, hipFuncAttributeMaxDynamicSharedMemorySize, G::LDS_BYTES + G::LN_BYTES);
    (void)hipFuncSetAttribute((const void*)gemm2_kernel<EPI_LN_GELU, NWN, 0, MF>, hipFuncAttributeMaxDynamicSharedMemorySize, G::LDS_BYTES + G::LN_BYTES);
    if constexpr (MF)
      (void)hipFuncSetAttribute((const void*)gemm2_kernel<EPI_GATE_RES_STATS, NWN, 0, MF>, hipFuncAttributeMaxDynamicSharedMemorySize, G::LDS_BYTES);
  }
  switch (epi) {
    case EPI_LN_BIAS: hipLaunchKernelGGL((gemm2_kernel<EPI_LN_BIAS, NWN, 0, MF>), dim3(grid), dim3(G::NT), G::LDS_BYTES + G::LN_BYTES, stream, p); break;
    case EPI_LN_GELU: hipLaunchKernelGGL((gemm2_kernel<EPI_LN_GELU, NWN, 0, MF>), dim3(grid), dim3(G::NT), G::LDS_BYTES + G::LN_BYTES, stream, p); break;
    case EPI_BIAS: hipLaunchKernelGGL((gemm2_kernel<EPI_BIAS, NWN, 0, MF>), dim3(grid), dim3(G::NT), G::LDS_BYTES, stream, p); break;
    case EPI_BIAS_GELU: hipLaunchKernelGGL((gemm2_kernel<EPI_BIAS_GELU, NWN, 0, MF>), dim3(grid), dim3(G::NT), G::LDS_BYTES, stream, p); break;
    case EPI_GATE_RES:
      if (MF && (p.aux || p.add1 || p.add2 || p.stats_out)) return VSYS_ERR_ARG;
      hipLaunchKernelGGL((gemm2_kernel<EPI_GATE_RES, NWN, 0, MF>), dim3(grid), dim3(G::NT), G::LDS_BYTES, stream, p); break;
    case EPI_GATE_RES_STATS:
      if constexpr (MF) {
        hipLaunchKernelGGL((gemm2_kernel<EPI_GATE_RES_STATS, NWN, 0, MF>), dim3(grid), dim3(G::NT), G::LDS_BYTES, stream, p);
        break;
      }
      return VSYS_ERR_ARG;
    default: return VSYS_ERR_ARG;
  }
  return hipGetLastError() == hipSuccess ? 0 : VSYS_ERR_LAUNCH;
}

int launch_gemm2_qkv_kv(const GemmParams& p_, hipStream_t stream) {
  using G = G2<2>;
  if (p_.M <= 0) return 0;
  GemmParams p = p_;
  const int H = p.kv_heads;
  if (H <= 0 || H % 8 != 0 || p.N != 216 * H || p.kv_S <= 0 || p.kv_S % 64 != 0 || p.M % p.kv_S != 0 || p.K <= 0 || p.K % BK != 0)
    return VSYS_ERR_SHAPE;
  if (!p.cs || !p.cv || !p.ln_stats || p.ln_nb < 1 || p.ln_nb > 12 || p.ln_nb * LN_BLOCK != p.K || p.ln_ld < p.M) return VSYS_ERR_SHAPE;
  if (!p.out || !p.kp || !p.vt || !p.k_norm_w || p.ldo < 72 * H) return VSYS_ERR_ARG;
  if ((p.lda % 8) || (p.ldw % 8) || (p.ldo % 8) || ((uintptr_t)p.kp % 16) || ((uintptr_t)p.vt % 16) || ((uintptr_t)p.k_norm_w % 16)) return VSYS_ERR_ALIGN;
  if (p.lda * 512 + (int64_t)p.K * 2 >= 0x7fffffff || p.ldw * 384 + (int64_t)p.K * 2 >= 0x7fffffff) return VSYS_ERR_SHAPE;
  constexpr int LDS = G::LDS_BYTES + G::LN_BYTES + G::KW_BYTES;
  static std::atomic<unsigned long long> attr_seen{0};
  for (DeviceOnce once(attr_seen); once.todo(); once.done())
    (void)hipFuncSetAttribute((const void*)gemm2_kernel<EPI_LN_QKV_KV, 2, 0, 1>, hipFuncAttributeMaxDynamicSharedMemorySize, LDS);
  const int grid = ((p.M + BM - 1) / BM) * (p.N / G::BN);
  hipLaunchKernelGGL((gemm2_kernel<EPI_LN_QKV_KV, 2, 0, 1>), dim3(grid), dim3(G::NT), LDS, stream, p);
  return hipGetLastError() == hipSuccess ? 0 : VSYS_ERR_LAUNCH;
}

#ifdef VSYS_LAB
int launch_gemm2_stamp(const GemmParams& p_, hipStream_t stream) {
  using G = G2<4>;
  GemmParams p = p_;
  p.aux = reinterpret_cast<bf16_t*>(get_lab_debug_buffer());
  if (p.N % G::BN != 0 || p.aux == nullptr) return VSYS_ERR_SHAPE;
  const int grid = ((p.M + BM - 1) / BM) * (p.N / G::BN);
  (void)hipFuncSetAttribute((const void*)gemm2_kernel<EPI_BIAS, 4, 1>, hipFuncAttributeMaxDynamicSharedMemorySize, G::LDS_BYTES);
  hipLaunchKernelGGL((gemm2_kernel<EPI_BIAS, 4, 1>), dim3(grid), dim3(G::NT), G::LDS_BYTES, stream, p);
  return hipGetLastError() == hipSuccess ? 0 : VSYS_ERR_LAUNCH;
}

#endif

int launch_gemm2_slices(const GemmParams& p, int slices, hipStream_t stream) {
  using G = G2<4>;
  if (p.M <= 0) return 0;
  if (p.N % G::BN != 0 || slices < 1 || slices > 65535 || p.ks <= 0 || p.ks % BK != 0 || p.K % BK != 0 || (int64_t)p.ks * slices < p.K ||
      (int64_t)p.ks * (slices - 1) >= p.K || p.out32 == nullptr || (p.lda % 8) || (p.ldw % 8) || p.rows_per_sample <= 0)
    return VSYS_ERR_SHAPE;
  if (p.lda * 512 + (int64_t)p.K * 2 >= 0x7fffffff || p.ldw * 768 + (int64_t)p.K * 2 >= 0x7fffffff) return VSYS_ERR_SHAPE;
  const int nbm = (p.M + BM - 1) / BM, nbn = p.N / G::BN;
  static std::atomic<unsigned long long> attr_seen{0};
  for (DeviceOnce once(attr_seen); once.todo(); once.done())
    (void)hipFuncSetAttribute((const void*)gemm2_kernel<EPI_F32_SLICES, 4>, hipFuncAttributeMaxDynamicSharedMemorySize, G::LDS_BYTES);
  hipLaunchKernelGGL((gemm2_kernel<EPI_F32_SLICES, 4>), dim3(nbm * nbn * slices), dim3(G::NT), G::LDS_BYTES, stream, p);
  return hipGetLastError() == hipSuccess ? 0 : VSYS_ERR_LAUNCH;
}

int launch_gemm2(const GemmParams& p, int epi, int wide, hipStream_t stream) {
  if (wide == 2) return launch_gemm2_t<2, 1>(p, epi, stream);
  if (wide == 3) return launch_gemm2_t<4, 1>(p, epi, stream);
  return wide ? launch_gemm2_t<4>(p, epi, stream) : launch_gemm2_t<2>(p, epi, stream);
}

}
```

### videosys_amd/csrc/gemm_bf16.hip

```cpp
#include <map>
#include <mutex>

#include "common.h"
#include "vsys_internal.h"

namespace vsys {

namespace {

constexpr int BN = 192, BK = 64;
constexpr int B_BYTES = BN * BK * 2;
constexpr int OUT_ROW_BYTES = 96 * 2 + 16;
constexpr int OUT_WAVE_BYTES = 64 * OUT_ROW_BYTES;

template <int BM_>
struct Geo {
  static constexpr int NW = BM_ / 32;
  static constexpr int NT = NW * 64;
  static constexpr int A_BYTES = BM_ * BK * 2;
  static constexpr int STAGE = A_BYTES + B_BYTES;
  static constexpr int NA = 4;
  static constexpr int NB = BN / NW / 8;
  static_assert(NW * OUT_WAVE_BYTES <= 2 * STAGE, "epilogue image must fit in the staging buffers");
};
// ... 1183 lines not shown
  return on;
}

namespace {
struct SplitKWs { float* ws = nullptr; int* flags = nullptr; int tiles = 0; };
std::mutex g_splitk_mutex;
std::map<hipStream_t, SplitKWs> g_splitk_ws;
}
static bool splitk_workspace(hipStream_t stream, int tiles, GemmParams& p) {
  std::lock_guard<std::mutex> lock(g_splitk_mutex);
  SplitKWs& w = g_splitk_ws[stream];
  if (w.ws == nullptr) {
    const int cap = cu_count_this_device();
    hipStreamCaptureStatus cs = hipStreamCaptureStatusNone;
    if (hipStreamIsCapturing(stream, &cs) == hipSuccess && cs != hipStreamCaptureStatusNone) return false;
    if (hipMalloc(&w.ws, (size_t)cap * 4 * 24 * 64 * sizeof(float4)) != hipSuccess) { w.ws = nullptr; return false; }
    if (hipMalloc(&w.flags, (size_t)cap * 4 * sizeof(int)) != hipSuccess || hipMemset(w.flags, 0, (size_t)cap * 4 * sizeof(int)) != hipSuccess) {
      (void)hipFree(w.ws);
      w.ws = nullptr;
      return false;
    }
    (void)hipDeviceSynchronize();
    w.tiles = cap;
  }
  if (tiles > w.tiles) return false;
  p.sk_ws = w.ws;
  p.sk_flags = w.flags;
  return true;
}
static int launch_rows128(const GemmParams& p_, int epi, hipStream_t stream, bool force_split = false) {
  if (!mf16_default() && !force_split) return launch_gemm_t<3, 128>(p_, epi, stream);
  static const bool splitk_on = [] { const char* e = getenv("VSYS_GEMM_SPLITK"); return e && e[0] == '1'; }();
  const int tiles = ((p_.M + 127) / 128) * (p_.N / BN);
  if ((splitk_on || force_split) && tiles >= 64 && tiles <= cu_count_this_device() && p_.K / BK >= 8) {
    GemmParams p = p_;
    if (splitk_workspace(stream, tiles, p)) return launch_gemm_t<3, 128, 1, 0, 1, 1>(p, epi, stream);
  }
  static const bool s8_on = [] { const char* e = getenv("VSYS_GEMM_ROWS128_S8"); return e && e[0] == '1'; }();
  if (s8_on && tiles <= cu_count_this_device() && p_.K / BK >= 3) return launch_gemm_t<8, 128, 1, 0, 1>(p_, epi, stream);
  static const bool ring_off = [] { const char* e = getenv("VSYS_GEMM_ROWS128_RING"); return e && e[0] == '0'; }();
  if (!ring_off && tiles <= cu_count_this_device() && p_.K / BK >= 3) return launch_gemm_t<9, 128, 1, 0, 1>(p_, epi, stream);
  return launch_gemm_t<3, 128, 1, 0, 1>(p_, epi, stream);
}
static int launch_sched8(const GemmParams& p, int epi, hipStream_t stream) {
  return mf16_default() ? launch_gemm_t<8, 256, 1, 0, 1>(p, epi, stream) : launch_gemm_t<8, 256>(p, epi, stream);
}

static bool ln_on_two_workgroup_tile(int64_t M, int64_t N, int64_t K) {
  return (int64_t)((M + 255) / 256) * (N / BN) >= 400 && K <= 1536 && N >= 2304 && g_gemm_variant_a.load(std::memory_order_relaxed) != 8;
}
bool gemm_ln_qkv_kv_dispatched(int64_t M, int64_t N, int64_t K) {
  return N > 0 && N % BN == 0 && K > 0 && K % BK == 0 && ln_on_two_workgroup_tile(M, N, K) && mf16_default();
}
int launch_gemm_qkv_kv(const GemmParams& p_, hipStream_t stream) {
  GemmParams p = p_;
  const int ras = g_gemm_raster_a.load(std::memory_order_relaxed);
  p.raster_gw = ras / 100;
  p.raster_ph = ras % 100;
  return launch_gemm2_qkv_kv(p, stream);
}

int launch_gemm(const GemmParams& p_, int epi, hipStream_t stream) {
  if (p_.M <= 0) return 0;
  GemmParams p = p_;
  {
    const int ras = g_gemm_raster_a.load(std::memory_order_relaxed);
    p.raster_gw = ras / 100;
    p.raster_ph = ras % 100;
  }
  if (p.N % BN != 0 || p.K % BK != 0 || p.N <= 0 || p.K <= 0) return VSYS_ERR_SHAPE;
  if ((p.lda % 8) || (p.ldw % 8) || (p.ldo % 8) || (p.res && (p.ldr % 8)) || (p.aux && (p.ldaux % 8))) return VSYS_ERR_ALIGN;
  if (p.lda * 512 + (int64_t)p.K * 2 >= 0x7fffffff || p.ldw * 384 + (int64_t)p.K * 2 >= 0x7fffffff) return VSYS_ERR_SHAPE;
  if ((epi == EPI_GATE_RES || epi == EPI_GATE_RES_STATS) && p.gate && p.rows_per_sample <= 0) return VSYS_ERR_SHAPE;
  if ((epi == EPI_GATE_RES || epi == EPI_GATE_RES_STATS) && (p.ldo * 128 >= 0x7fffffff || (p.res && p.ldr * 128 >= 0x7fffffff) || (p.aux && p.ldaux * 128 >= 0x7fffffff)))
    return VSYS_ERR_SHAPE;
  const bool ln = epi == EPI_LN_BIAS || epi == EPI_LN_GELU;
  if (ln && (!p.cs || !p.cv || !p.ln_stats || p.ln_nb < 1 || p.ln_nb > 12 || p.ln_nb * LN_BLOCK != p.K || p.ln_ld < p.M)) return VSYS_ERR_SHAPE;
  if (epi == EPI_GATE_RES_STATS && (!p.stats_out || p.stats_ld < p.M || p.aux)) return VSYS_ERR_ARG;
  if (epi != EPI_GATE_RES && (p.add1 || p.add2)) return VSYS_ERR_ARG;
  if (epi == EPI_GATE_RES && (p.add1 || p.add2 || p.stats_out)) {
    if ((p.add2 && !p.add1) || ((p.add1 || p.add2) && (!p.res || (p.ldr % 8))) || (p.stats_out && p.stats_ld < p.M)) return VSYS_ERR_ARG;
    if ((int64_t)((p.M + 255) / 256) * (p.N / BN) < 400) return launch_rows128(p, epi, stream, g_gemm_variant_a.load(std::memory_order_relaxed) == 123);
    return g_gemm_variant_a.load(std::memory_order_relaxed) == 8 ? launch_gemm_t<8, 256>(p, epi, stream) : launch_sched8(p, epi, stream);
  }
  if (epi == EPI_GATE_RES_STATS) {
    if ((int64_t)((p.M + 255) / 256) * (p.N / BN) < 400) return launch_rows128(p, epi, stream, g_gemm_variant_a.load(std::memory_order_relaxed) == 123);
    if (g_gemm_variant_a.load(std::memory_order_relaxed) == 24) return launch_gemm2(p, epi, 2, stream);
    return g_gemm_variant_a.load(std::memory_order_relaxed) == 8 ? launch_gemm_t<8, 256>(p, epi, stream) : launch_sched8(p, epi, stream);
  }
  if (ln) {
    if ((int64_t)((p.M + 255) / 256) * (p.N / BN) < 400) return launch_rows128(p, epi, stream, g_gemm_variant_a.load(std::memory_order_relaxed) == 123);
    if (ln_on_two_workgroup_tile(p.M, p.N, p.K)) return launch_gemm2(p, epi, mf16_default() ? 2 : 0, stream);
    return g_gemm_variant_a.load(std::memory_order_relaxed) == 8 ? launch_gemm_t<8, 256>(p, epi, stream) : launch_sched8(p, epi, stream);
  }
  const int g_gemm_variant = g_gemm_variant_a.load(std::memory_order_relaxed);
  switch (g_gemm_variant == 50 ? 0 : g_gemm_variant) {
    case 6: return launch_gemm_t<6, 256>(p, epi, stream);
#ifdef VSYS_LAB
    case 18: return launch_gemm_t<18, 256>(p, epi, stream);
    case 48: return launch_gemm_t<48, 256>(p, epi, stream);
    case 38: return launch_gemm_t<38, 256>(p, epi, stream);
    case 40: return launch_gemm3(p, epi, stream);
    case 31: return (epi == EPI_BIAS && p.N % 384 == 0) ? launch_gemm2_stamp(p, stream) : VSYS_ERR_ARG;
    case 61: case 62: case 63: case 64: return epi == EPI_BIAS ? launch_gemm4_lab(p, g_gemm_variant - 60, 0, stream) : VSYS_ERR_ARG;
    case 71: case 72: case 73: case 74: case 78: return epi == EPI_BIAS ? launch_gemm4_lab(p, g_gemm_variant - 70, 1, stream) : VSYS_ERR_ARG;
    case 60: case 70: case 80:
      if (!gemm4_supports(p, epi)) return launch_gemm_t<8, 256>(p, epi, stream);
      return launch_gemm4(p, epi, (g_gemm_variant - 60) / 10, stream);
    case 81: case 82: case 83: case 84:
      return gemm4_supports(p, epi) ? launch_gemm4(p, epi, 2 + g_gemm_variant - 80, stream) : VSYS_ERR_ARG;
#endif
    case 103: return launch_gemm_t<3, 128>(p, epi, stream);
    case 113: return launch_gemm_t<3, 128, 1, 0, 1>(p, epi, stream);
// ... 38 lines not shown
```

### videosys_amd/csrc/gen/program_gen.py

```python
#!/usr/bin/env python
import os
import re
import sys

ROOT = os.path.dirname(os.path.dirname(os.path.dirname(os.path.dirname(os.path.abspath(__file__)))))
HDR = os.path.join(ROOT, "include", "videosys_amd.h")
LAB_HDR = os.path.join(ROOT, "include", "videosys_amd_lab.h")
INC = os.path.join(ROOT, "videosys_amd", "csrc", "program_ops.inc")
PYM = os.path.join(ROOT, "videosys_amd", "_opcodes.py")
NO_OP = {"vsys_vae_first_im2col_nc", "vsys_pixels_to_u8", "vsys_clip_attention_d64", "vsys_splitk_reduce_bias_act",
         "vsys_attn_temporal_d64_img", "vsys_attn_prep_kv96", "vsys_flash_attn_d96", "vsys_upsample_trilinear2x",
         "vsys_cfg_ancestral_step", "vsys_pixels_to_u8_trunc", "vsys_attn_prep_kv96_img", "vsys_flash_attn_d96_img",
         "vsys_attn_prep_kv_rope", "vsys_flash_attn_d72_rope", "vsys_upsample_time2x", "vsys_cfg_pndm_step"}
BEGIN, END = "/* >>> VSYS_OP codes (generated: csrc/gen/program_gen.py) */", "/* <<< VSYS_OP codes */"


def parse(h):
    out = []
    for ret, name, args in re.findall(r"\n(int|const char\*) (vsys_\w+)\(([^;]*?)\);", h, flags=re.S):
        params = [x.strip() for x in re.sub(r"\s+", " ", args).split(",")]
        kinds = []
        for p in ([] if params == ["void"] else params):
            ty = p.rsplit(" ", 1)[0].strip()
            kind = "f" if ty == "float" else "p" if ty.endswith("*") else {"int64_t": "l", "int": "i"}.get(ty)
            if kind is None:
                raise SystemExit(f"{name}: parameter type {ty!r} has no vsys_cmd / ctypes representation")
            kinds.append((kind, ty))
        out.append((name, kinds, "i" if ret == "int" else "s", params[-1] == "void* stream"))
    return out


def ops_of(protos):
    return [(name, kinds[:-1]) for name, kinds, _, launches in protos if launches and name not in NO_OP]


def build():
    h = open(HDR).read()
    protos, lab_protos = parse(h), parse(open(LAB_HDR).read())
    entries = ops_of(protos)
    old = {m.group(1): int(m.group(2)) for m in re.finditer(r"#define VSYS_OP_(\w+)\s+(\d+)", h) if m.group(1) != "COUNT"}
    codes, nxt = {}, max(old.values(), default=0) + 1
    for name, _ in entries:
        key = name[len("vsys_"):].upper()
        if key in old:
            codes[name] = old[key]
    for name, _ in entries:
        if name not in codes:
            codes[name] = nxt
            nxt += 1
    count = max(codes.values()) + 1
    by_code = sorted(entries, key=lambda e: codes[e[0]])
    max_i = max(sum(1 for k, _ in kinds if k != "f") for _, kinds in entries)
    max_f = max(sum(1 for k, _ in kinds if k == "f") for _, kinds in entries)
    lines = [BEGIN]
    for name, _ in by_code:
        lines.append(f"#define VSYS_OP_{name[5:].upper():28s} {codes[name]}")
    lines += [f"#define VSYS_OP_COUNT {count}", END]
    block = "\n".join(lines)
    if BEGIN in h:
        h2 = h[:h.index(BEGIN)] + block + h[h.index(END) + len(END):]
    else:
        m = list(re.finditer(r"#define VSYS_OP_\w+[^\n]*\n", h))
        h2 = h[:m[0].start()] + block + "\n" + h[m[-1].end():]
    inc = ["// GENERATED by csrc/gen/program_gen.py from include/videosys_amd.h — do not edit.",
           f"static_assert(VSYS_CMD_MAX_INT >= {max_i} && VSYS_CMD_MAX_FLOAT >= {max_f}, \"vsys_cmd is too small for the widest entry point\");",
           "#ifdef VSYS_PROGRAM_TABLE", "constexpr OpInfo kOps[VSYS_OP_COUNT] = {", "    {0, 0},"]
# ... 51 lines not shown
```

### videosys_amd/csrc/vsys_internal.h

```cpp
#pragma once
#include <hip/hip_runtime.h>
#include <stdint.h>

#include <atomic>
#include <vector>

#include "../../include/videosys_amd.h"

namespace vsys {

typedef uint16_t bf16_t;

class DeviceOnce {
 public:
  explicit DeviceOnce(std::atomic<unsigned long long>& seen) : seen_(seen) {
    int dev = 0;
    if (hipGetDevice(&dev) == hipSuccess && dev >= 0 && dev <= 63) bit_ = 1ull << dev;
    todo_ = bit_ == 0 || (seen_.load(std::memory_order_acquire) & bit_) == 0;
  }
  bool todo() const { return todo_; }
  void done() {
    if (bit_ != 0) seen_.fetch_or(bit_, std::memory_order_release);
    todo_ = false;
  }

 private:
  std::atomic<unsigned long long>& seen_;
  unsigned long long bit_ = 0;
  bool todo_ = false;
};
inline int cu_count_this_device() {
  static std::atomic<int> cache[64];
  int dev = 0;
  if (hipGetDevice(&dev) != hipSuccess || dev < 0 || dev > 63) return 256;
  int n = cache[dev].load(std::memory_order_relaxed);
  if (n == 0) {
    hipDeviceProp_t prop;
    n = (hipGetDeviceProperties(&prop, dev) == hipSuccess && prop.multiProcessorCount > 0) ? prop.multiProcessorCount : 256;
    cache[dev].store(n, std::memory_order_relaxed);
  }
  return n;
}

enum { EPI_BIAS = VSYS_EPI_BIAS, EPI_BIAS_GELU = VSYS_EPI_BIAS_GELU, EPI_GATE_RES = VSYS_EPI_GATE_RES,
       EPI_LN_BIAS = 3, EPI_LN_GELU = 4,
       EPI_GATE_RES_STATS = 5,
       EPI_LN_QKV_KV = 6,
       EPI_F32_SLICES = 100  };
constexpr int LN_BLOCK = 96;
enum { ACT_NONE = VSYS_ACT_NONE, ACT_SILU = VSYS_ACT_SILU, ACT_GELU_TANH = VSYS_ACT_GELU_TANH };

struct GemmParams {
  const bf16_t* A = nullptr; int64_t lda = 0;
  const bf16_t* W = nullptr; int64_t ldw = 0;
  const bf16_t* bias = nullptr;
  bf16_t* out = nullptr; int64_t ldo = 0;
  int M = 0, N = 0, K = 0;
  const bf16_t* gate = nullptr; int64_t gate_stride = 0;
  const bf16_t* res = nullptr; int64_t ldr = 0;
  bf16_t* aux = nullptr; int64_t ldaux = 0;
  int rows_per_sample = 0;
  int seg_split = 0; int64_t gate_alt = 0;
  int ks = 0; float* out32 = nullptr; int64_t slab = 0, ldo32 = 0;
  const float* cs = nullptr; const float* cv = nullptr;
  const float2* ln_stats = nullptr; int64_t ln_ld = 0; int ln_nb = 0; float ln_eps = 0.f;
  float2* stats_out = nullptr; int64_t stats_ld = 0;
  const bf16_t* add1 = nullptr; const bf16_t* add2 = nullptr;
  int raster_gw = 6, raster_ph = 0;
  float* sk_ws = nullptr; int* sk_flags = nullptr;
  bf16_t* kp = nullptr; bf16_t* vt = nullptr; const bf16_t* k_norm_w = nullptr;
  int kv_S = 0, kv_heads = 0; float k_eps = 0.f, kscale = 0.f;
};

__host__ __device__ inline int qkv_kv_column(int n, int heads) {
  const int C = 72 * heads, nq = C / 96;
  if (n < C) return n;
  if (n < 2 * C) return (nq + (n - C) / 72) * 96 + (n - C) % 72;
  const int f = n - 2 * C;
  return f < 24 * heads ? (nq + f / 24) * 96 + 72 + f % 24 : (nq + heads) * 96 + (f - 24 * heads);
}

struct ConvParams {
  const bf16_t* A = nullptr; int64_t lda = 0;
  const bf16_t* W = nullptr; int64_t ldw = 0;
  const bf16_t* bias = nullptr;
  const bf16_t* res = nullptr; int64_t ldr = 0;
  bf16_t* out = nullptr; float* out32 = nullptr; int64_t ldo = 0;
  int M = 0, N = 0, K = 0;
  int cin = 0, taps = 0, cshift = 0, taps_hw = 0, kw = 0, row_pitch = 0, plane_pitch = 0, max_tap_rows = 0;
  int batch = 0; int64_t batch_a = 0, batch_w = 0, batch_o = 0;
  float out_scale = 0.f;
};
int launch_conv(const ConvParams& p, hipStream_t stream);

struct VaeGrid {
  int T, H, W, pad, tf;
  int64_t sample_rows;
};
int launch_gn_stats(const bf16_t* x, const VaeGrid& g, int N, int C, int groups, float eps, float* partial, int nblk, float* stats,
                    hipStream_t stream);
int launch_gn_apply(const bf16_t* x, const VaeGrid& gs, bf16_t* y, const VaeGrid& gd, int N, int C, int groups, const float* stats,
                    const bf16_t* gamma, const bf16_t* beta, int act, hipStream_t stream);
int launch_regrid(const bf16_t* x, const VaeGrid& gs, bf16_t* y, const VaeGrid& gd, int N, int C, int up, int tmode, hipStream_t stream);
int launch_subsample(const bf16_t* x, const VaeGrid& gs, bf16_t* y, const VaeGrid& gd, int N, int C, int st, int ss, int t0, int s0,
                     hipStream_t stream);
int launch_spatial_norm_apply(const bf16_t* x, const VaeGrid& gs, bf16_t* y, const VaeGrid& gd, int N, int C, int groups,
                              const float* stats, const bf16_t* gamma, const bf16_t* beta, const bf16_t* yb, int zT, int zH, int zW,
                              hipStream_t stream);
int launch_blend_edge(const bf16_t* a, bf16_t* b, int64_t outer, int Ha, int Wa, int Hb, int Wb, int ext, int axis, hipStream_t stream);
int launch_d2s_time(const bf16_t* x, const VaeGrid& gs, bf16_t* y, const VaeGrid& gd, int N, int Cout, hipStream_t stream);
int launch_vae_first_im2col(const bf16_t* z, int F, int H, int W, int kt, int kcols, const float* scale, const float* shift,
                            const float* pq_w, const float* pq_b, bf16_t* out, hipStream_t stream);
int launch_extract_planar(const bf16_t* x, const VaeGrid& g, int N, int ldx, int nc, int tskip, bf16_t* out, int64_t Ftot, int f0,
                          hipStream_t stream);
int launch_softmax_rows(const float* s, bf16_t* p, int64_t rows, int n, int ld, hipStream_t stream);

int launch_vae_first_im2col_nc(const float* z, int F, int Cz, int H, int W, int kcols, float scaling, float shift, bf16_t* out,
                               hipStream_t stream);
int launch_pixels_to_u8(const bf16_t* x, const VaeGrid& g, int N, int64_t ldx, uint8_t* out, int64_t Ftot, int64_t f0,
                        hipStream_t stream);
int launch_upsample_trilinear2x(const bf16_t* x, const VaeGrid& gs, bf16_t* y, const VaeGrid& gd, int N, int C, hipStream_t stream);
int launch_cfg_ancestral_step(float* z, const float* model_out, const float* noise, bf16_t* model_in, int Bz, int Cin, int Cout,
                              int64_t thw, float guidance, float dt, float sigma_up, float in_scale, hipStream_t stream);
int launch_pixels_to_u8_trunc(const bf16_t* x, const VaeGrid& g, int N, int64_t ldx, uint8_t* out, int64_t Ftot, int64_t f0,
                              hipStream_t stream);
int launch_upsample_time2x(const bf16_t* x, const VaeGrid& gs, bf16_t* y, const VaeGrid& gd, bf16_t* y_res, const VaeGrid* g_res,
                           float alpha, int N, int C, hipStream_t stream);
int launch_cfg_pndm_step(const float* model_out, float* e_out, const float* const* src, const float* base, float* z_out, float* aux_out,
                         bf16_t* model_in, int Bz, int Cin, int Cout, int64_t thw, const double* coef, hipStream_t stream);

int launch_gather_rows(const bf16_t* table, const int64_t* ids, bf16_t* out, int64_t n, int C, int64_t vocab, hipStream_t stream);
int launch_rms_norm_rows(const bf16_t* x, const bf16_t* w, bf16_t* y, int64_t rows, int C, float eps, hipStream_t stream);
int launch_geglu(const bf16_t* h, bf16_t* out, int64_t rows, int F, hipStream_t stream);
int launch_t5_attention(const bf16_t* qkv, int64_t row_stride, int inner, const float* relbias, const int* klen, bf16_t* out,
                        int64_t out_stride, int B, int L, int heads, hipStream_t stream);
int launch_splitk_reduce_t(const float* part, int S, int64_t slab, int ldp, const bf16_t* res, int64_t ldr, bf16_t* out, int64_t ldo,
                           int M, int N, hipStream_t stream);
int launch_splitk_reduce(const float* part, int S, int64_t slab, int64_t ldp, const bf16_t* res, int64_t ldr, bf16_t* out, int64_t ldo,
                         int M, int N, hipStream_t stream);
int launch_t5_attention_mfma(const bf16_t* qkv, int64_t row_stride, int inner, const float* bias, int bias_ld, int bias_center,
                             int kv_len, bf16_t* kp, bf16_t* vt, bf16_t* out, int64_t out_stride, int L, int heads,
                             hipStream_t stream);

int launch_clip_attention_d64(const bf16_t* qkv, int64_t row_stride, int inner, bf16_t* out, int64_t out_stride, int B, int L,
                              hipStream_t stream);
int launch_splitk_reduce_bias_act(const float* part, int S, int64_t slab, int64_t ldp, const bf16_t* res, int64_t ldr, bf16_t* out,
                                  int64_t ldo, int M, int N, const bf16_t* bias, int act, hipStream_t stream);

int launch_gemm(const GemmParams& p, int epi, hipStream_t stream);
int launch_gemm2(const GemmParams& p, int epi, int wide, hipStream_t stream);
int launch_gemm2_qkv_kv(const GemmParams& p, hipStream_t stream);
int launch_gemm_qkv_kv(const GemmParams& p, hipStream_t stream);
bool gemm_ln_qkv_kv_dispatched(int64_t M, int64_t N, int64_t K);
int launch_gemm2_slices(const GemmParams& p, int slices, hipStream_t stream);
int launch_gemm3(const GemmParams& p, int epi, hipStream_t stream);
int launch_gemm4(const GemmParams& p, int epi, int persistent, hipStream_t stream);
bool gemm4_supports(const GemmParams& p, int epi);
bool sk_plan(int ntiles, int nt, int grid, std::vector<int4>& segs, int& nseg_max);
int launch_gemm4_lab(const GemmParams& p, int abl, int persistent, hipStream_t stream);
int launch_gemm2_stamp(const GemmParams& p, hipStream_t stream);
int set_gemm_variant(int v);
int set_flash_variant(int v);
int get_flash_variant();
void set_flash_debug_buffer(void* p);
void* get_lab_debug_buffer();
int launch_linear_small(const bf16_t* x, int64_t ldx, const bf16_t* w, int64_t ldw, const bf16_t* bias, bf16_t* out,
                        int64_t ldo, int M, int N, int K, int act_in, int act_out, hipStream_t stream);
int launch_adaln_modulate(const bf16_t* x, const bf16_t* shift, const bf16_t* scale, bf16_t* y, int64_t rows, int C,
                          int64_t rows_per_sample, int64_t mod_stride, float eps, hipStream_t stream);
int launch_adaln_prescale(const int64_t* sites, int nsites, int64_t nblocks, const bf16_t* mod, hipStream_t stream);
int launch_ln_row_stats(const bf16_t* x, int64_t rows, int C, float2* stats, int64_t ld, hipStream_t stream);
int launch_mod_table(const bf16_t* table, const bf16_t* t_mlp, bf16_t* out, int nblk, int B, int C6, hipStream_t stream);
int launch_timestep_embedding(const float* t, bf16_t* out, int B, int dim, hipStream_t stream);
int launch_patch_embed(const float* x, int Bz, const bf16_t* w, const bf16_t* bias, const bf16_t* pos, bf16_t* out, int B,
                       int Cin, int T, int H, int W, int ph, int pw, int C, int s0, int Sl, hipStream_t stream);
int launch_unpatchify_tokens(const float* tok, float* out, int P, int B, int T, int Sl, int Hp, int Wp, int H, int W, int ph,
                             int pw, int Cout, hipStream_t stream);
int launch_final_layer(const bf16_t* x, const bf16_t* table, const bf16_t* tvec, const bf16_t* w, const bf16_t* bias,
                       float* out, int B, int T, int Hp, int Wp, int H, int W, int ph, int pw, int Cout, int C, float eps,
                       int Sl, float* tokens, hipStream_t stream);
int launch_cfg_euler(float* z, const float* model_out, int Bz, int Cin, int Cout, int64_t thw, float guidance, float dt,
                     hipStream_t stream);
int launch_cfg_axpby(float* z, const float* model_out, int Bz, int Cin, int Cout, int64_t thw, float guidance, float c_z,
                     float c_eps, int cond_first, hipStream_t stream);
int launch_add_bcast_rows(bf16_t* x, const bf16_t* e, int64_t rows, int C, int64_t group, int64_t period, hipStream_t stream);
int launch_add_rows(bf16_t* x, const bf16_t* y, int64_t n, hipStream_t stream);
int launch_copy_4d(const bf16_t* src, bf16_t* dst, int n0, int n1, int n2, int C, int64_t ss0, int64_t ss1, int64_t ss2,
                   int64_t ds0, int64_t ds1, int64_t ds2, int n1_valid, int n2_valid, hipStream_t stream);
constexpr int VSYS_COPY_BATCH_MAX = 16;
struct CopyDesc {
  int64_t src_off, dst_off;
  int n0, n1, n2, C;
  int64_t ss0, ss1, ss2, ds0, ds1, ds2;
  int n1_valid, n2_valid;
};
int launch_copy_4d_batch(const bf16_t* src, bf16_t* dst, const CopyDesc* ops, int nops, hipStream_t stream);
int launch_p2p_exchange(const bf16_t* src, const CopyDesc* ops, bf16_t* const* dsts, unsigned* const* peer_flags, const int* remote, int nops,
                        const unsigned* my_flags, int n_flags, int self_index, unsigned* state, long long timeout_ticks,
                        hipStream_t stream);
int launch_attn_prep_kv(const bf16_t* k, int64_t k_stride, const bf16_t* v, int64_t v_stride, const bf16_t* k_norm_w,
                        bf16_t* kp, bf16_t* vt, int batch, int heads, int kv_len, int kv_pad, float eps,
                        hipStream_t stream);
int launch_flash_attn_d72(const bf16_t* q, int64_t q_stride, const bf16_t* q_norm_w, const bf16_t* kp, const bf16_t* vt,
                          bf16_t* out, int64_t out_stride, int batch, int heads, int q_len, int kv_len, int kv_pad,
                          float eps, float k_bound, hipStream_t stream,
                          bool keys_exact = false);
int launch_attn_prep_kv_varlen(const bf16_t* k, int64_t k_stride, const bf16_t* v, int64_t v_stride, const bf16_t* k_norm_w,
                               const int* cu_seqlens, const int* cu_seqlens_host, bf16_t* kp, bf16_t* vt, int batch, int heads,
                               int kv_pad, float eps, hipStream_t stream);
int launch_flash_attn_d72_varlen(const bf16_t* q, int64_t q_stride, const bf16_t* q_norm_w, const bf16_t* kp, const bf16_t* vt,
                                 const int* kv_lens, const int* kv_lens_host, bf16_t* out, int64_t out_stride, int batch, int heads,
                                 int q_len, int kv_pad, float eps, hipStream_t stream);
bool flash_w64_supports(int q_len, int kv_len, int kv_pad);
int launch_flash_attn_d72_w64(const bf16_t* q, int64_t q_stride, const bf16_t* q_norm_w, const bf16_t* kp, const bf16_t* vt, bf16_t* out,
                              int64_t out_stride, int batch, int heads, int q_len, int kv_len, int kv_pad, float eps, int var,
                              float k_bound, hipStream_t stream);
bool flash64_w64_supports(int q_len, int kv_len);
int launch_flash_attn_d64_w64(const bf16_t* q, int64_t q_stride, const bf16_t* ln_w, const bf16_t* ln_b, const float* rope_cos,
                              const float* rope_sin, int rope_start, int rope_len, const bf16_t* kp, const bf16_t* vt, bf16_t* out,
                              int64_t out_stride, int batch, int heads, int q_len, int kv_len, int kv_pad, float eps, int var,
                              float k_bound, hipStream_t stream);
bool flash_w64p_supports(int q_len, int kv_len, int kv_pad, int64_t q_stride);
int launch_flash_attn_d72_w64p(const bf16_t* q, int64_t q_stride, const bf16_t* q_norm_w, const bf16_t* kp, const bf16_t* vt, bf16_t* out,
                               int64_t out_stride, int batch, int heads, int q_len, int kv_len, int kv_pad, float eps, bool stamp,
                               float k_bound, hipStream_t stream);
int launch_attn_prep_kv64(const bf16_t* k, int64_t k_stride, const bf16_t* v, int64_t v_stride, const bf16_t* ln_w,
                          const bf16_t* ln_b, const float* rope_cos, const float* rope_sin, int rope_start, int rope_len,
                          bf16_t* kp, bf16_t* vt, int batch, int heads, int kv_len, int kv_pad, float eps, hipStream_t stream);
int launch_flash_attn_d64(const bf16_t* q, int64_t q_stride, const bf16_t* ln_w, const bf16_t* ln_b, const float* rope_cos,
                          const float* rope_sin, int rope_start, int rope_len, const bf16_t* kp, const bf16_t* vt, bf16_t* out,
                          int64_t out_stride, int batch, int heads, int q_len, int kv_len, int kv_pad, float eps, float k_bound,
                          hipStream_t stream);
int launch_attn_prep_kv_rope(const bf16_t* k, int64_t k_stride, const bf16_t* v, int64_t v_stride, const float* rope_cos,
                             const float* rope_sin, bf16_t* kp, bf16_t* vt, int batch, int heads, int kv_len, int kv_pad,
                             hipStream_t stream);
int launch_flash_attn_d72_rope(const bf16_t* q, int64_t q_stride, const float* rope_cos, const float* rope_sin, const bf16_t* kp,
                               const bf16_t* vt, bf16_t* out, int64_t out_stride, int batch, int heads, int q_len, int kv_len,
                               int kv_pad, hipStream_t stream);
int launch_attn_prep_kv96(const bf16_t* k, int64_t k_stride, const bf16_t* v, int64_t v_stride, const float* rope_cos,
                          const float* rope_sin, bf16_t* kp, bf16_t* vt, int batch, int heads, int kv_len, int kv_pad,
                          hipStream_t stream);
int launch_flash_attn_d96(const bf16_t* q, int64_t q_stride, const float* rope_cos, const float* rope_sin, const bf16_t* kp,
                          const bf16_t* vt, const int* kv_lens, bf16_t* out, int64_t out_stride, int batch, int heads, int q_len,
                          int kv_len, int kv_pad, hipStream_t stream);
int launch_attn_prep_kv96_img(const bf16_t* k, int64_t k_stride, const bf16_t* v, int64_t v_stride, const float* rope_cos,
                              const float* rope_sin, bf16_t* kp, bf16_t* vt, int batch, int heads, int kv_len, int kv_pad, int seg_len,
                              int64_t slab_rows, hipStream_t stream);
int launch_flash_attn_d96_img(const bf16_t* q, int64_t q_stride, const float* rope_cos, const float* rope_sin, const bf16_t* kp,
                              const bf16_t* vt, const int* kv_lens, bf16_t* out, int64_t out_stride, int batch, int heads, int q_len,
                              int kv_len, int kv_pad, int seg_len, int64_t q_slab_rows, int64_t out_slab_rows, hipStream_t stream);
int launch_ln_modulate(const bf16_t* x, const bf16_t* ln_w, const bf16_t* ln_b, const bf16_t* shift, const bf16_t* scale,
                       bf16_t* y, int64_t rows, int C, int64_t rows_per_sample, int64_t mod_stride, int64_t seg_split,
                       int64_t mod_alt, float eps, hipStream_t stream);
int launch_gate_add_rows(bf16_t* x, const bf16_t* y, const bf16_t* gate, int64_t rows, int C, int64_t rows_per_sample,
                         int64_t gate_stride, int64_t seg_split, int64_t gate_alt, hipStream_t stream);
int launch_unpatchify_cvx(const bf16_t* x, int64_t ldx, float* out, int B, int F, int Hp, int Wp, int Cout, int p,
                          hipStream_t stream);
int launch_im2col_patch(const float* z, int Bz, bf16_t* out, int B, int F, int Cin, int H, int W, int p, hipStream_t stream);
int launch_attn_temporal_d72_v3(const bf16_t* qkv, int64_t row_stride, int C, const bf16_t* q_norm_w, const bf16_t* k_norm_w,
                                const float* rope_cos, const float* rope_sin, bf16_t* out, int64_t out_stride, int B, int T, int S,
                                int heads, float eps, float scale, hipStream_t stream, bool ref_rounding = false,
                                bool no_v5 = false);
int launch_attn_temporal_d72(const bf16_t* qkv, int64_t row_stride, int C, const bf16_t* q_norm_w, const bf16_t* k_norm_w,
                             const float* rope_cos, const float* rope_sin, bf16_t* out, int64_t out_stride, int B, int T,
                             int S, int heads, float eps, hipStream_t stream);

int launch_attn_temporal_d64(const bf16_t* q_vid, int64_t q_vid_ld, const bf16_t* k_vid, int64_t k_vid_ld, const bf16_t* v_vid,
                             int64_t v_vid_ld, const bf16_t* q_txt, int64_t q_txt_ld, const bf16_t* k_txt, int64_t k_txt_ld,
                             const bf16_t* v_txt, int64_t v_txt_ld, const float* rope_cos, const float* rope_sin, bf16_t* out_vid,
                             int64_t out_vid_ld, bf16_t* out_txt, int64_t out_txt_ld, int B, int T, int S, int L, int heads,
                             hipStream_t stream);
int launch_attn_temporal_d64_img(const bf16_t* q_vid, int64_t q_vid_ld, const bf16_t* k_vid, int64_t k_vid_ld, const bf16_t* v_vid,
                                 int64_t v_vid_ld, const bf16_t* q_txt, int64_t q_txt_ld, const bf16_t* k_txt, int64_t k_txt_ld,
                                 const bf16_t* v_txt, int64_t v_txt_ld, const float* rope_cos, const float* rope_sin, bf16_t* out_vid,
                                 int64_t out_vid_ld, bf16_t* out_txt, int64_t out_txt_ld, int B, int T, int Tl, int64_t slab_vid,
                                 int64_t slab_txt, int S, int L, int heads, hipStream_t stream);
int launch_scale_add_rows(const bf16_t* a, int64_t lda, const bf16_t* b, int64_t ldb, bf16_t* out, int64_t ldo, int64_t rows, int C,
                          float scale, hipStream_t stream);

}
```

### videosys_amd/ops.py

```python
from __future__ import annotations

import os
from typing import Optional

import torch

from . import _lib, program

EPI_BIAS, EPI_BIAS_GELU, EPI_GATE_RES = 0, 1, 2
ACT_NONE, ACT_SILU, ACT_GELU_TANH = 0, 1, 2
HEAD_DIM = 72
VT_ROWS = 96


class _TPtr(int):
    """A device address that remembers its tensor: ctypes and the launch-program recorder see the integer, the custom-op route
    (torch.ops.vsys.launch) hands the TENSOR to the dispatcher."""


def _p(t: Optional[torch.Tensor]):
    if t is None:
        return None
    if program.active() is not None:
        program.keep(t)
# ... 282 lines not shown


def copy_4d_batch(src, dst, descs):
    import ctypes

    _chk(src, dst)
    _bf16(src, dst)
    for i in range(0, len(descs), 16):
        part = descs[i:i + 16]
        flat = [int(v) for d in part for v in d]
        arr = (ctypes.c_int64 * len(flat))(*flat)
        _call("vsys_copy_4d_batch", _p(src), _p(dst), len(part), arr)


def kv_pad_len(kv_len: int) -> int:
    return (kv_len + 63) // 64 * 64


def alloc_kv_buffers(batch, heads, kv_len, device):
    kv_pad = kv_pad_len(kv_len)
    kp = torch.zeros(batch, heads, kv_pad, HEAD_DIM, dtype=torch.bfloat16, device=device)
    vt = torch.zeros(batch, heads, VT_ROWS, kv_pad, dtype=torch.bfloat16, device=device)
    return kp, vt


def _fused_kv_default() -> bool:
    return os.environ.get("VSYS_FUSED_KV", "1") != "0"


FUSED_KV = _fused_kv_default()


def qkv_kv_column_order(heads: int) -> torch.Tensor:
    assert heads > 0 and heads % 4 == 0
    C, nq = 72 * heads, 72 * heads // 96
    n = torch.arange(3 * C, dtype=torch.int64)
    k, f = n - C, n - 2 * C
    kcol = (nq + k // 72) * 96 + k % 72
    vcol = torch.where(f < 24 * heads, (nq + f // 24) * 96 + 72 + f % 24, (nq + heads) * 96 + (f - 24 * heads))
    return torch.where(n < C, n, torch.where(n < 2 * C, kcol, vcol))


def gemm_ln_qkv_kv_dispatched(M: int, N: int, K: int) -> bool:
    return bool(_lib.load().vsys_gemm_bf16_ln_qkv_kv_dispatched(M, N, K))


def kv_set_constant_rows(vt):
    assert vt.shape[2] == VT_ROWS
    vt[:, :, HEAD_DIM:] = 0
    vt[:, :, HEAD_DIM] = 1.0
    vt[:, :, HEAD_DIM + 4] = 1.0


def gemm_ln_qkv_kv(x, wp, cs, cv, stats, k_norm_w, q, kp, vt, S, heads, eps=1e-6, k_eps=1e-6):
    _chk(x, wp, cs, cv, stats, k_norm_w, q, kp, vt)
    _bf16(x, wp, k_norm_w, q, kp, vt)
    assert x.dim() == 2 and x.stride(1) == 1 and wp.stride(1) == 1 and q.stride(1) == 1 and cs.dtype == torch.float32 and cv.dtype == torch.float32
    M, K = x.shape
    assert wp.shape == (216 * heads, K) and cs.numel() == cv.numel() == 216 * heads and k_norm_w.numel() == HEAD_DIM and k_norm_w.is_contiguous()
    assert S > 0 and M % S == 0 and q.shape[0] == M and q.shape[1] >= HEAD_DIM * heads and kp.is_contiguous() and vt.is_contiguous()
    assert tuple(kp.shape) == (M // S, heads, S, HEAD_DIM) and tuple(vt.shape) == (M // S, heads, VT_ROWS, S)
    ld = _stats_ld(stats, M, K // LN_BLOCK)
    _call("vsys_gemm_bf16_ln_qkv_kv", _p(x), x.stride(0), _p(wp), wp.stride(0), _p(cs), _p(cv), _p(stats), ld, _p(k_norm_w), _p(q),
          q.stride(0), _p(kp), _p(vt), M, K, S, heads, float(eps), float(k_eps))
    return q


def attn_prep_kv(k, v, k_norm_w, kp, vt, batch, heads, kv_len, eps=1e-6):
    _chk(k, v, k_norm_w, kp, vt)
    _bf16(k, v, k_norm_w, kp, vt)
    assert k.stride(1) == 1 and v.stride(1) == 1 and kp.is_contiguous() and vt.is_contiguous()
    kv_pad = kp.shape[2]
    assert vt.shape[3] == kv_pad and vt.shape[2] == VT_ROWS
    _call("vsys_attn_prep_kv", _p(k), k.stride(0), _p(v), v.stride(0), _p(k_norm_w), _p(kp), _p(vt), batch, heads,
                                     kv_len, kv_pad, eps)


def flash_attn(q, q_norm_w, kp, vt, out, batch, heads, q_len, kv_len, eps=1e-6, k_norm_bound=None, keys_exact=False):
    _chk(q, q_norm_w, kp, vt, out)
    _bf16(q, q_norm_w, kp, vt, out)
    assert q.stride(1) == 1 and out.stride(1) == 1
    kv_pad = kp.shape[2]
    if keys_exact and not k_norm_bound:
        _call("vsys_flash_attn_d72_exact", _p(q), q.stride(0), _p(q_norm_w), _p(kp), _p(vt), _p(out), out.stride(0), batch, heads,
              q_len, kv_len, kv_pad, eps)
    elif k_norm_bound:
        _call("vsys_flash_attn_d72_kb", _p(q), q.stride(0), _p(q_norm_w), _p(kp), _p(vt), _p(out), out.stride(0), batch, heads,
              q_len, kv_len, kv_pad, eps, float(k_norm_bound))
    else:
        _call("vsys_flash_attn_d72", _p(q), q.stride(0), _p(q_norm_w), _p(kp), _p(vt), _p(out), out.stride(0), batch, heads,
              q_len, kv_len, kv_pad, eps)
    return out


class VarlenKeys:

    def __init__(self, lens, device):
        import ctypes

        self.lens = tuple(int(n) for n in lens)
        cu = [0]
        for n in self.lens:
            cu.append(cu[-1] + n)
        self.batch = len(self.lens)
        self.total = cu[-1]
        self.max_len = max(self.lens) if self.lens else 0
        self.cu_host = (ctypes.c_int32 * len(cu))(*cu)
# ... 416 lines not shown
```

### videosys_amd/stdit3.py

```python
from __future__ import annotations

import math
import os
from types import SimpleNamespace
from typing import Dict, Optional

import torch

from . import dsp, ops, pab, program
from .utils import same_tensor
from .workspace import Workspace


class STDiT3Config:

    model_type = "STDiT3"

    def __init__(self, input_size=(None, None, None), input_sq_size=512, in_channels=4, patch_size=(1, 2, 2),
                 hidden_size=1152, depth=28, num_heads=16, mlp_ratio=4.0, class_dropout_prob=0.1, pred_sigma=True,
                 drop_path=0.0, caption_channels=4096, model_max_length=300, qk_norm=True, enable_flash_attn=False,
                 only_train_temporal=False, freeze_y_embedder=False, skip_y_embedder=False, **kwargs):
        self.input_size = input_size
        self.input_sq_size = input_sq_size
        self.in_channels = in_channels
        self.patch_size = tuple(patch_size)
        self.hidden_size = hidden_size
        self.depth = depth
        self.num_heads = num_heads
        self.mlp_ratio = mlp_ratio
        self.class_dropout_prob = class_dropout_prob
        self.pred_sigma = pred_sigma
        self.drop_path = drop_path
        self.caption_channels = caption_channels
        self.model_max_length = model_max_length
        self.qk_norm = qk_norm
        self.enable_flash_attn = enable_flash_attn
        self.only_train_temporal = only_train_temporal
        self.freeze_y_embedder = freeze_y_embedder
        self.skip_y_embedder = skip_y_embedder
        for k, v in kwargs.items():
            setattr(self, k, v)


def pos_embed_2d(dim: int, h: int, w: int, scale: float, base_size: int) -> torch.Tensor:
    half = dim // 2
    inv_freq = 1.0 / (10000 ** (torch.arange(0, half, 2).float() / half))
    gh = torch.arange(h) / scale
    gw = torch.arange(w) / scale
    gh = gh * (base_size / h)
    gw = gw * (base_size / w)
    gh, gw = torch.meshgrid(gw, gh, indexing="ij")
    gh = gh.t().reshape(-1)
    gw = gw.t().reshape(-1)

    def sincos(t):
        out = torch.einsum("i,d->id", t, inv_freq)
        return torch.cat((torch.sin(out), torch.cos(out)), dim=-1)

    return torch.cat([sincos(gh), sincos(gw)], dim=-1)


def rope_tables(freqs: torch.Tensor, T: int, pos_dtype: torch.dtype):
# ... 30 lines not shown
    for n in lens:
        cu.append(cu[-1] + n)
    if packed_rows is not None and int(packed_rows) != cu[-1]:
        raise ValueError(f"y holds {int(packed_rows)} tokens, y_lens sum to {cu[-1]}")
    return lens, cu


class STDiT3:

    config_class = STDiT3Config

    def __init__(self, config: STDiT3Config, device="cuda", dtype=torch.bfloat16):
        if dtype != torch.bfloat16:
            raise ValueError("the MI355X path computes in bf16 (fp32 accumulate); got %s" % dtype)
        from . import _lib

        _lib.load()
        self.config = config
        self.device = torch.device(device)
        self.dtype = dtype
        self.pred_sigma = config.pred_sigma
        self.in_channels = config.in_channels
        self.out_channels = config.in_channels * 2 if config.pred_sigma else config.in_channels
        self.depth = config.depth
        self.hidden_size = config.hidden_size
        self.num_heads = config.num_heads
        self.patch_size = tuple(config.patch_size)
        self.input_sq_size = config.input_sq_size
        if self.hidden_size // self.num_heads != ops.HEAD_DIM:
            raise ValueError("attention kernels are built for head_dim 72 (STDiT3-XL/2)")
        if self.patch_size[0] != 1:
            raise ValueError("temporal patch size must be 1")
        self.w: Dict[str, torch.Tensor] = {}
        self.rope_freqs: Optional[torch.Tensor] = None
        self.parallel_manager = SimpleNamespace(sp_size=1, cp_size=1, dp_size=1, dp_rank=0, sp_group=None, cp_group=None)
        self._sp: Optional[dsp.SequenceParallel] = None
        self._overlap, self._switch, self._scatter, self._side = False, "auto", "flat", None
        self.states = [pab.BlockState(i // 2, bool(i % 2)) for i in range(2 * self.depth)]
        self._pos_cache = {}
        self._rope_cache = {}
        self._text_cache = None
        self._fps_cache = {}
        self._ws = Workspace(self.device, dtype)
        self._buf = self._ws.buf
        self._hidden_tap = None
        self.pab_elide_unused = os.environ.get("VSYS_PAB_ELIDE", "1") != "0"
        self.pab_fold_adds = os.environ.get("VSYS_PAB_FOLD", "1") != "0"
        self._bc, self._folded = None, {}
        self._kbounds = {}
        self.use_programs = os.environ.get("VSYS_PROGRAMS", "1") != "0"
        self.adaln_fold = os.environ.get("VSYS_ADALN_FOLD", "1") != "0"
        self.fold_spatial_qkv = True
        self.fused_kv = ops.FUSED_KV
        self._fold = None
        self._stats_fresh = False
        self._programs = {}
        self.program_stats = dict(recorded=0, replayed=0, eager=0)
        self.x_embedder = SimpleNamespace(proj=SimpleNamespace(weight=torch.empty(0, dtype=dtype)))
        self.y_embedder = SimpleNamespace(y_embedding=None)

    def block_prefix(self, i):
        return f"{'temporal' if i % 2 else 'spatial'}_blocks.{i // 2}"

    def load_state_dict(self, sd: Dict[str, torch.Tensor], strict: bool = True):
        need = self.expected_keys()
        self._kbounds = {}
        missing = [k for k in need if k not in sd]
        if strict and missing:
            raise KeyError(f"missing keys: {missing[:8]}{'...' if len(missing) > 8 else ''}")
        for k in need:
            if k not in sd:
                continue
            t = sd[k]
            if k == "rope.freqs":
                self.rope_freqs = t.detach().cpu().clone()
                continue
            if k == "x_embedder.proj.weight":
                t = t.reshape(t.shape[0], -1)
            self.w[k] = t.detach().to(device=self.device, dtype=self.dtype).contiguous()
        tabs = [self.w[self.block_prefix(i) + ".scale_shift_table"].reshape(-1) for i in range(2 * self.depth)]
        self.w["_all_tables"] = torch.stack(tabs).contiguous()
        self.x_embedder.proj.weight = self.w["x_embedder.proj.weight"]
        self.y_embedder.y_embedding = self.w["y_embedder.y_embedding"]
        self._text_cache = None
        self._rope_cache = {}
        self._programs = {}
        self._fold = None
        return self

    def expected_keys(self):
        keys = ["x_embedder.proj.weight", "x_embedder.proj.bias", "t_block.1.weight", "t_block.1.bias",
                "y_embedder.y_proj.fc1.weight", "y_embedder.y_proj.fc1.bias", "y_embedder.y_proj.fc2.weight",
                "y_embedder.y_proj.fc2.bias", "y_embedder.y_embedding", "rope.freqs",
                "final_layer.scale_shift_table", "final_layer.linear.weight", "final_layer.linear.bias"]
        for e in ("t_embedder", "fps_embedder"):
            for l in ("0", "2"):
                keys += [f"{e}.mlp.{l}.weight", f"{e}.mlp.{l}.bias"]
        for i in range(2 * self.depth):
            p = self.block_prefix(i)
            keys += [p + ".scale_shift_table", p + ".attn.q_norm.weight", p + ".attn.k_norm.weight"]
            for l in ("attn.qkv", "attn.proj", "cross_attn.q_linear", "cross_attn.kv_linear", "cross_attn.proj", "mlp.fc1",
                      "mlp.fc2"):
                keys += [f"{p}.{l}.weight", f"{p}.{l}.bias"]
        return keys

    def state_dict(self):
# ... 87 lines not shown
        h = ops.linear_small(yb, w["y_embedder.y_proj.fc1.weight"], w["y_embedder.y_proj.fc1.bias"], act_out=ops.ACT_GELU_TANH)
        ye = ops.linear_small(h, w["y_embedder.y_proj.fc2.weight"], w["y_embedder.y_proj.fc2.bias"]).view(B, L, C)
        if mask is not None:
            m = mask
            if m.shape[0] != B:
                m = m.repeat(B // m.shape[0], 1)
            m = m.reshape(B, L)
            y_lens = [int(v) for v in m.sum(dim=1).tolist()]
            if len(set(y_lens)) != 1:
                y_lens, _ = text_lengths(mask=(m != 0).to("cpu"))
            idx = torch.nonzero(m.reshape(-1) != 0, as_tuple=False).reshape(-1).to(self.device)
            yp = ye.reshape(B * L, C).index_select(0, idx).contiguous()
        else:
            y_lens = [L] * B
            yp = ye.reshape(B * L, C)
        return self._text_kv(y, mask, yp, y_lens, B)

    def _text_kv(self, y, mask, yp, y_lens, B, lens_key=None):
        w, C, H = self.w, self.hidden_size, self.num_heads
        ragged = len(set(y_lens)) != 1
        if ragged and self.device.type != "cuda":
            raise ValueError(f"text lengths {list(y_lens)} differ per sample: a ragged batch needs the model on a HIP device "
                             f"(this one is on {self.device}); off the device cross-attention takes equal text lengths only")
        keys = ops.VarlenKeys(y_lens, self.device) if ragged else None
        Lk = y_lens[0] if keys is None else keys.max_len
        if keys is not None and lens_key is None:
            lens_key = keys.lens
        nblk = 2 * self.depth
        kv_pad = ops.kv_pad_len(Lk)
        kps = torch.zeros(nblk, B, H, kv_pad, ops.HEAD_DIM, dtype=self.dtype, device=self.device)
        vts = torch.zeros(nblk, B, H, ops.VT_ROWS, kv_pad, dtype=self.dtype, device=self.device)
        kv = torch.empty(sum(y_lens), 2 * C, dtype=self.dtype, device=self.device)
        for i in range(nblk):
            p = self.block_prefix(i) + ".cross_attn.kv_linear"
            if (2 * C) % 192 == 0 and C % 64 == 0:
                ops.gemm(yp, w[p + ".weight"], w[p + ".bias"], out=kv)
            else:
                ops.linear_small(yp, w[p + ".weight"], w[p + ".bias"], out=kv)
            if keys is None:
                ops.attn_prep_kv(kv[:, :C], kv[:, C:], None, kps[i], vts[i], B, H, Lk)
            else:
                ops.attn_prep_kv_varlen(kv[:, :C], kv[:, C:], None, keys, kps[i], vts[i], H)
        self._text_cache = dict(y=y, y_version=y._version, mask=mask, mask_version=None if mask is None else mask._version,
                                y_lens=y_lens, kp=kps, vt=vts, Lk=Lk, lens_key=lens_key, varlen=keys)
        return self._text_cache

    def _fold_ok(self, ts_host, fkey, x_mask):
        C = self.hidden_size
        return (self.adaln_fold and x_mask is None and C % ops.LN_BLOCK == 0 and C // ops.LN_BLOCK <= 12
                and bool((ts_host == ts_host[0]).all()) and len(set(fkey[:-1])) == 1)

    def _fused_kv_ok(self, N, S):
        C, H = self.hidden_size, self.num_heads
        return bool(self.fused_kv and self._sp is None and self.fold_spatial_qkv and C == 72 * H and H % 8 == 0 and S % 64 == 0
                    and ops.gemm_ln_qkv_kv_dispatched(N, 3 * C, C))

    def _fold_tables(self, B, fused_kv=False):
        f = self._fold or None
        if f is not None and f["B"] == B and f["fused_kv"] == fused_kv:
            return f
        w, C, dev = self.w, self.hidden_size, self.device
        bufs = f["bufs"] if f is not None else {}
        rows, blk = [], 0
        for i in range(2 * self.depth):
            p = self.block_prefix(i)
            for name, s_sh, s_sc in ((p + ".attn.qkv", 0, C), (p + ".mlp.fc1", 3 * C, 4 * C)):
                W, b = w[name + ".weight"], w[name + ".bias"]
                N, K = W.shape
                if name not in bufs:
                    bufs[name] = (torch.empty_like(W), torch.empty(N, dtype=torch.float32, device=dev),
                                  torch.empty(N, dtype=torch.float32, device=dev))
                Wp, cs, cv = bufs[name]
                base = i * B * 6 * C
                order = self.num_heads << 32 if (fused_kv and i % 2 == 0 and s_sh == 0) else 0
                rows.append([W.data_ptr(), b.data_ptr(), Wp.data_ptr(), cs.data_ptr(), cv.data_ptr(), base + s_sh, base + s_sc,
                             N | order, K, blk])
                blk += -(-N // 4)
        self._fold = dict(B=B, fused_kv=fused_kv, bufs=bufs, sites=torch.tensor(rows, dtype=torch.int64).to(dev), nblocks=blk)
        return self._fold

    def _ln_stats(self, N):
        return self._ws.once(("ln_stats", N), lambda: ops.ln_stats_buffer(N, self.hidden_size, self.device))

    def reset_text_cache(self):
        self._text_cache = None
        self._programs = {}

    @torch.no_grad()
    def forward(self, x, timestep, y, all_timesteps=None, mask=None, x_mask=None, fps=None, height=None, width=None,
                **kwargs):
        w, C, H = self.w, self.hidden_size, self.num_heads
        pm = self.parallel_manager
        cp = getattr(pm, "cp_size", 1) or 1
        if cp > 1:
            Bfull = x.shape[0]
            if Bfull % cp:
                raise ValueError(f"batch {Bfull} is not divisible by cp_size {cp}")
            Bl = Bfull // cp
            sl = slice(pm.cp_rank * Bl, (pm.cp_rank + 1) * Bl)
            rows = lambda v: v[sl] if (torch.is_tensor(v) and v.dim() > 0 and v.shape[0] == Bfull) else v
            if bool(getattr(self.config, "skip_y_embedder", False)) and mask is not None and y.shape[0] != Bfull:
                lens_all = [int(v) for v in (mask.reshape(-1).tolist() if torch.is_tensor(mask) else mask)]
                _, cu = text_lengths(y_lens=lens_all, batch=Bfull, packed_rows=y.reshape(-1, y.shape[-1]).shape[0])
                y = y.reshape(-1, y.shape[-1])[cu[sl.start]:cu[sl.stop]].unsqueeze(0)
                mask = lens_all[sl]
            x, timestep, y, fps, height, width, mask, x_mask = (rows(v) for v in (x, timestep, y, fps, height, width, mask, x_mask))
        B, _, Tx, Hx, Wx = x.shape
        T, Hp, Wp = self.get_dynamic_size(x)
        dev = self.device
        if x_mask is not None and not x_mask.is_cuda and bool(x_mask.to(torch.bool).all()):
            x_mask = None
        if x_mask is not None:
            if tuple(x_mask.shape) != (B, T):
                raise ValueError(f"x_mask must be [B, T] = [{B}, {T}], got {tuple(x_mask.shape)}")
            x_mask = x_mask.to(device=dev, dtype=torch.bool).contiguous()

        ts_host = timestep.detach().to("cpu").to(self.dtype).float()
        timestep_int = int(ts_host[0]) if pab.enable_pab() else None
        valid_depth = kwargs.get("valid_depth", self.depth)
        plan = self._pab_plan(timestep_int, all_timesteps, valid_depth)
        txt = self._encode_text(y, mask)
        pos = self._pos(Hp, Wp, height[0], width[0])
        fkey = tuple(float(v) for v in fps.reshape(-1).tolist()) + (B,)
        if fkey not in self._fps_cache:
            f = fps.to(dev).float().reshape(-1)
            if f.numel() != B:
                f = f.repeat(B // f.numel())
            self._fps_cache[fkey] = self._embed_vec(f, "fps_embedder")
        self._rope(T)
        static = (txt, pos, self._fps_cache[fkey])
        fold = self._fold_ok(ts_host, fkey, x_mask)

        try:
            return self._issue_step(x, ts_host, static, plan, timestep_int, valid_depth, cp, x_mask, fold, fkey, height, width)
        except BaseException:
            for st in self.states:
                st.attn_valid = st.cross_valid = False
            raise

    def _issue_step(self, x, ts_host, static, plan, timestep_int, valid_depth, cp, x_mask, fold, fkey, height, width):
        dev = self.device
        B, _, Tx, Hx, Wx = x.shape
        mlp_action = plan is not None and any(d[2] or d[3] for d in plan)
        if not (self.use_programs and self._hidden_tap is None and not mlp_action and x_mask is None):
            self.program_stats["eager"] += 1
            xz = x.to(device=dev, dtype=torch.float32).contiguous()
            out = self._forward_device(xz, ts_host.to(dev), static, plan, timestep_int, valid_depth, cp, x_mask, fold=fold)
        else:
            sp = self._sp
            key = (B, Tx, Hx, Wx, float(height[0]), float(width[0]), fkey, valid_depth, cp, fold, self.fold_spatial_qkv, self.fused_kv,
                   None if plan is None else tuple(d[:2] + d[5:7] for d in plan),
                   None if static[0]["varlen"] is None else static[0]["varlen"].lens,
                   None if sp is None else (sp.P, sp.rank, self._scatter, self._switch, self._overlap))
            ent = self._programs.get(key)
            if ent is not None:
                prog, xin, tin, out = ent
                xin.copy_(x, non_blocking=True)
                tin.copy_(ts_host, non_blocking=True)
                prog.run()
                self.program_stats["replayed"] += 1
                out = out.clone()
            else:
                xin = torch.empty(B, x.shape[1], Tx, Hx, Wx, dtype=torch.float32, device=dev)
                tin = torch.empty(B, dtype=torch.float32, device=dev)
                xin.copy_(x)
                tin.copy_(ts_host)
                with program.Recorder() as rec:
                    out = self._forward_device(xin, tin, static, plan, timestep_int, valid_depth, cp, fold=fold)
                prog = rec.finish()
                if prog is not None:
                    self._programs[key] = (prog, xin, tin, out)
                    self.program_stats["recorded"] += 1
                    out = out.clone()
                else:
                    self.program_stats["eager"] += 1
        return out

    def _pab_plan(self, timestep_int, all_timesteps, valid_depth):
        if not pab.enable_pab():
            return None
        plan = []
        cfg = pab.PAB_MANAGER.config
        mlp_on = cfg.mlp_broadcast
        if mlp_on and all_timesteps is None:
            raise ValueError("PAB mlp_broadcast needs the sampler's schedule: call the model with all_timesteps=[...]")
        sched = [int(v) for v in all_timesteps] if all_timesteps is not None else None
        ats = sched if mlp_on else None
        t_next = None
        if self.pab_elide_unused and sched is not None and sched.count(timestep_int) == 1 and sched.index(timestep_int) + 1 < len(sched):
            t_next = sched[sched.index(timestep_int) + 1]

        def kept(kind, count_next):
            if t_next is None:
                return True
            on, every, thr = cfg.attn_rule(kind)
            return bool(on) and thr is not None and count_next % every != 0 and thr[0] < t_next < thr[1]

        for i in range(2 * valid_depth):
            st = self.states[i]
            kind = "temporal" if st.temporal else "spatial"
            fn = pab.if_broadcast_temporal if st.temporal else pab.if_broadcast_spatial
            b_attn, st.attn_count = fn(timestep_int, st.attn_count)
            b_cross, st.cross_count = pab.if_broadcast_cross(timestep_int, st.cross_count)
# ... 123 lines not shown
                    j, kk = j + 1, 0
                if j >= len(self._bc) or not self._bc[j][kk]:
                    break
                sj = self.states[j]
                if kk == 2:
                    cached = pab.get_mlp_output(self._bc[j][3], timestep=timestep_int, block_idx=sj.block_idx, is_temporal=sj.temporal)
                else:
                    cached = sj.last_attn if kk == 0 else sj.last_cross
                if cached is None or cached.shape != x.shape or cached.stride() != x.stride():
                    if kk == 2:
                        self._folded[(j, kk)] = (cached, False)
                    break
                self._folded[(j, kk)] = (cached, True)
                got.append(cached)
            return got

        def applied(k):
            return self._folded.get((i, k), (None, False))[1]

        def write_x(a, wname, k, gate=None, aux=None, want_stats=False):
            adds = upcoming(k)
            W, bias = w[wname + ".weight"], w[wname + ".bias"]
            gk = dict(gate=gate, gate_stride=C6, rows_per_sample=rps) if gate is not None else {}
            if adds or (fold and aux is not None and (want_stats or adds)):
                ops.gemm_gate_res_add(a, W, bias, res=x, aux=aux, adds=adds, stats=stats if fold else None, out=x, **gk)
                self._stats_fresh = fold
            elif fold and aux is None and want_stats:
                ops.gemm_stats(a, W, bias, stats, res=x, out=x, **gk)
                self._stats_fresh = True
            else:
                ops.gemm(a, W, bias, epilogue=ops.EPI_GATE_RES, res=x, aux=aux, out=x, **gk)
                self._stats_fresh = False

        sp_order = None
        if sp is not None and not temporal:
            flat = T == 1 or self._scatter == "flat"
            sp_order = self._switch_order(*((1, B * T) if flat else (B, T)), S_full)
        fold_attn = fold and (temporal or (sp is None and self.fold_spatial_qkv) or sp_order == "qkv")

        if broadcast_attn:
            if not applied(0):
                ops.add_rows(x, st.last_attn)
                self._stats_fresh = False
        else:
            xm = None
            fused_kv = fold_attn and not temporal and sp is None and ftab["fused_kv"]
            if fused_kv:
                if not self._stats_fresh:
                    ops.ln_row_stats(x, stats)
                    self._stats_fresh = True
                Wp_, cs_, cv_ = ftab["bufs"][p + ".attn.qkv"]
                kp, vt = self._kv_spatial(B * T, S, constant_rows=True)
                q = _buf("qkv", (N, 3 * C)).view(-1)[:N * C].view(N, C)
                ops.gemm_ln_qkv_kv(x, Wp_, cs_, cv_, stats, w[p + ".attn.k_norm.weight"], q, kp, vt, S, H)
            elif fold_attn and sp_order is None:
                qkv = folded(p + ".attn.qkv", False, _buf("qkv", (N, 3 * C)))
            elif not fold_attn:
                xm = ops.adaln_modulate(x, shift_msa, scale_msa, rps, C6, out=_buf("xm", (N, C)))
            aux = None
            if use_pab and keep_attn:
                st.last_attn = slab(st.last_attn)
                aux = st.last_attn
            if temporal:
                if not fold_attn:
                    qkv = ops.gemm(xm, w[p + ".attn.qkv.weight"], w[p + ".attn.qkv.bias"], out=_buf("qkv", (N, 3 * C)))
                ao = _buf("attn_out", (N, C))
                cos, sin = self._rope(T)
                ops.attn_temporal(qkv, C, w[p + ".attn.q_norm.weight"], w[p + ".attn.k_norm.weight"], cos, sin, ao, B, T, S, H)
            elif fused_kv:
                ao = _buf("attn_out", (N, C))
                ops.flash_attn(q, w[p + ".attn.q_norm.weight"], kp, vt, ao, B * T, H, S, S, k_norm_bound=self._kbound(p))
            elif sp is None:
                if not fold_attn:
                    qkv = ops.gemm(xm, w[p + ".attn.qkv.weight"], w[p + ".attn.qkv.bias"], out=_buf("qkv", (N, 3 * C)))
                kp, vt = self._kv_spatial(B * T, S)
                ops.attn_prep_kv(qkv[:, C:2 * C], qkv[:, 2 * C:], w[p + ".attn.k_norm.weight"], kp, vt, B * T, H, S)
                ao = _buf("attn_out", (N, C))
                ops.flash_attn(qkv[:, :C], w[p + ".attn.q_norm.weight"], kp, vt, ao, B * T, H, S, S, k_norm_bound=self._kbound(p))
            else:
                qkv_rest = None
                if fold_attn:
                    qkv_rest = folded(p + ".attn.qkv", False, self._buf("qkv_rest", (N, 3 * C)))
                ao = self._spatial_attn_sharded(p, xm, B, T, S, S_full, qkv_rest=qkv_rest)
            write_x(ao, p + ".attn.proj", 0, gate=gate_msa, aux=aux)

        if broadcast_cross:
            if not applied(1):
                ops.add_rows(x, st.last_cross)
                self._stats_fresh = False
        else:
            q = ops.gemm(x, w[p + ".cross_attn.q_linear.weight"], w[p + ".cross_attn.q_linear.bias"], out=_buf("xm", (N, C)))
            ao = _buf("attn_out", (N, C))
            if txt["varlen"] is None:
                ops.flash_attn(q, None, txt["kp"][i], txt["vt"][i], ao, B, H, T * S, txt["Lk"], keys_exact=True)
            else:
                ops.flash_attn_varlen(q, None, txt["kp"][i], txt["vt"][i], txt["varlen"], ao, H, T * S)
            aux = None
            if use_pab and keep_cross:
                st.last_cross = slab(st.last_cross)
                aux = st.last_cross
            write_x(ao, p + ".cross_attn.proj", 1, aux=aux, want_stats=not broadcast_mlp or self._bc is not None)

        if broadcast_mlp:
            if (i, 2) in self._folded:
                slab = self._folded[(i, 2)][0]
            else:
                slab = pab.get_mlp_output(skip_range, timestep=timestep_int, block_idx=st.block_idx, is_temporal=temporal)
            if not applied(2):
                ops.add_rows(x, slab)
                self._stats_fresh = False
            if timestep_int == skip_range[-1]:
                self._ws.give_slab(slab)
            return x
        hdim = w[p + ".mlp.fc1.weight"].shape[0]
        if fold:
            hbuf = folded(p + ".mlp.fc1", True, _buf("mlp_h", (N, hdim)))
        else:
            xm = ops.adaln_modulate(x, shift_mlp, scale_mlp, rps, C6, out=_buf("xm", (N, C)))
            hbuf = ops.gemm(xm, w[p + ".mlp.fc1.weight"], w[p + ".mlp.fc1.bias"], epilogue=ops.EPI_BIAS_GELU,
                            out=_buf("mlp_h", (N, hdim)))
        aux = self._ws.take_slab(x) if broadcast_next else None
        write_x(hbuf, p + ".mlp.fc2", 2, gate=gate_mlp, aux=aux, want_stats=True)
        if broadcast_next:
            pab.save_mlp_output(timestep=timestep_int, block_idx=st.block_idx, ff_output=aux, is_temporal=temporal)
# ... 153 lines not shown
```

Baseline: 21.07 videos/min.

## Fuse Q RMS-norm into QKV GEMM epilogue and add q-ready flash attention

Adds a QKV GEMM epilogue that applies the per-head Q RMS-norm and writes normalized Q directly, alongside the existing fused K/V preparation. It also adds flash-attention variants (rows32 and persistent w64 stream forms) that skip in-kernel Q normalization. The column reorder table gains a q-order bit so Q heads land in whole 96-column windows. The goal is to stop re-normalizing Q inside every attention block, at the cost of extra epilogue work in the GEMM and new code paths that must match the old numerics.

```diff
diff --git a/include/videosys_amd.h b/include/videosys_amd.h
--- a/include/videosys_amd.h
+++ b/include/videosys_amd.h
@@ -40,6 +40,11 @@
 int vsys_gemm_bf16_ln_qkv_kv(const void* x, int64_t ldx, const void* wp, int64_t ldw, const void* cs, const void* cv, const void* stats,
                              int64_t stats_ld, const void* k_norm_w, void* q, int64_t ldq, void* kp, void* vt, int64_t M, int64_t K,
                              int64_t S, int64_t heads, float eps, float k_eps, void* stream);
+int vsys_gemm_bf16_ln_qkv_q(const void* x, int64_t ldx, const void* wp, int64_t ldw, const void* cs, const void* cv, const void* stats,
+                            int64_t stats_ld, const void* k_norm_w, const void* q_norm_w, void* q, int64_t ldq, void* kp, void* vt,
+                            int64_t M, int64_t K, int64_t S, int64_t heads, float eps, float k_eps, float q_eps, void* stream);
+int vsys_flash_attn_d72_qready(const void* q, int64_t q_stride, const void* kp, const void* vt, void* out, int64_t out_stride,
+                               int64_t batch, int64_t heads, int64_t q_len, int64_t kv_len, int64_t kv_pad, int64_t form, void* stream);
 int vsys_gemm_bf16_ln_qkv_kv_dispatched(int64_t M, int64_t N, int64_t K);
 
 int vsys_gemm_bf16_stats(const void* x, int64_t ldx, const void* w, int64_t ldw, const void* bias, void* out, int64_t ldo, int64_t M,
diff --git a/videosys_amd/_opcodes.py b/videosys_amd/_opcodes.py
--- a/videosys_amd/_opcodes.py
+++ b/videosys_amd/_opcodes.py
@@ -70,6 +70,8 @@
     "vsys_gemm_bf16": ("plplppllllipllplplp", "i"),
     "vsys_gemm_bf16_ln": ("plplppplllliplfp", "i"),
     "vsys_gemm_bf16_ln_qkv_kv": ("plplppplpplppllllffp", "i"),
+    "vsys_gemm_bf16_ln_qkv_q": ("plplppplppplppllllfffp", "i"),
+    "vsys_flash_attn_d72_qready": ("plppplllllllp", "i"),
     "vsys_gemm_bf16_ln_qkv_kv_dispatched": ("lll", "i"),
     "vsys_gemm_bf16_stats": ("plplppllllpllplplp", "i"),
     "vsys_gemm_bf16_gate_res_add": ("plplppllllpllplpppplp", "i"),
diff --git a/videosys_amd/csrc/adaln_fold.hip b/videosys_amd/csrc/adaln_fold.hip
--- a/videosys_amd/csrc/adaln_fold.hip
+++ b/videosys_amd/csrc/adaln_fold.hip
@@ -23,10 +23,11 @@
   float* cv = reinterpret_cast<float*>(s[4]);
   const bf16_t* shift = mod + s[5];
   const bf16_t* scale = mod + s[6];
-  const int N = (int)(s[7] & 0xffffffff), kv_heads = (int)(s[7] >> 32), K = (int)s[8];
+  const int N = (int)(s[7] & 0xffffffff), kv_heads = (int)((s[7] >> 32) & 0xffff), q_order = (int)((s[7] >> 48) & 1), K = (int)s[8];
   const int n = ((int)blockIdx.x - (int)s[9]) * 4 + wave;
   if (n >= N) return;
-  const int nd = (kv_heads > 0 && N == 216 * kv_heads && kv_heads % 4 == 0) ? qkv_kv_column(n, kv_heads) : n;
+  const int nd = (kv_heads > 0 && N == 216 * kv_heads && kv_heads % 4 == 0) ? (q_order ? qkv_q_column(n, kv_heads) : qkv_kv_column(n, kv_heads))
+                                                                            : n;
   const bf16_t* wr = W + (int64_t)n * K;
   bf16_t* wo = Wp + (int64_t)nd * K;
   float a_cs = 0.f, a_cv = 0.f;
diff --git a/videosys_amd/csrc/attention.hip b/videosys_amd/csrc/attention.hip
--- a/videosys_amd/csrc/attention.hip
+++ b/videosys_amd/csrc/attention.hip
@@ -126,6 +126,7 @@
 };
 
 constexpr int ABL_ROPE = 7;
+constexpr int ABL_QREADY = 8;
 constexpr int RES_MAX_TILES = 5;
 constexpr int RES_Q_BYTES = 5 * 1024;
 template <int ABL, int WPS, bool RES = false, bool EXACT = false, bool VARLEN = false>
@@ -244,7 +245,7 @@
       }
       return;
     }
-    if (p.q_norm_w == nullptr) {
+    if (ABL == ABL_QREADY || p.q_norm_w == nullptr) {
 #pragma unroll
       for (int c = 0; c < 5; ++c) qf[c] = __builtin_bit_cast(bf16x8, qraw[c]);
       return;
@@ -605,7 +606,7 @@
       __syncthreads();
       FLASH_STAMP(4);
     }
-    constexpr bool WHOLE_TILES_ONLY = ABL == ABL_ROPE && WPS == 3;
+    constexpr bool WHOLE_TILES_ONLY = (ABL == ABL_ROPE || ABL == ABL_QREADY) && WPS == 3;
     if (!WHOLE_TILES_ONLY && (kv_len & 63)) tile(ntiles - 1, (ntiles - 1) & 1, true);
     else tile(ntiles - 1, (ntiles - 1) & 1, false);
 
@@ -1199,4 +1200,29 @@
   return hipGetLastError() == hipSuccess ? 0 : VSYS_ERR_LAUNCH;
 }
 
-}
+int launch_flash_attn_d72_qready(const bf16_t* q, int64_t q_stride, const bf16_t* kp, const bf16_t* vt, bf16_t* out, int64_t out_stride,
+                                 int batch, int heads, int q_len, int kv_len, int kv_pad, int form, hipStream_t stream) {
+  if (batch <= 0 || heads <= 0 || q_len <= 0) return 0;
+  if (kv_len <= 0 || kv_pad % 64 != 0 || kv_pad < kv_len || (q_stride % 8) || (out_stride % 4)) return VSYS_ERR_SHAPE;
+  if (form == 1) {
+    if (!flash_w64p_supports(q_len, kv_len, kv_pad, q_stride)) return VSYS_ERR_SHAPE;
+    return launch_flash_attn_d72_w64p_qready(q, q_stride, kp, vt, out, out_stride, batch, heads, q_len, kv_len, kv_pad, stream);
+  }
+  if (form != 0) return VSYS_ERR_ARG;
+  FlashParams p;
+  p.q = q; p.q_stride = q_stride; p.q_norm_w = nullptr; p.kp = kp; p.vt = vt; p.out = out; p.out_stride = out_stride;
+  p.heads = heads; p.q_len = q_len; p.kv_len = kv_len; p.kv_pad = kv_pad; p.eps = 0.f;
+  p.kv_lens = nullptr;
+  p.dbg = nullptr;
+  p.nqb = (q_len + 127) / 128;
+  p.chunks = 1;
+  const int64_t nblk = (int64_t)p.nqb * batch * heads;
+  if (nblk > 0x7fffffff) return VSYS_ERR_SHAPE;
+  const size_t lds = 2 * KV_STAGE;
+  static const bool wps3_ok = [] { const char* e = getenv("VSYS_FLASH_WPS3"); return !(e && e[0] == '0'); }();
+  if (wps3_ok && kv_len >= 512 && (kv_len & 63) == 0) hipLaunchKernelGGL((flash_attn_d72_kernel<ABL_QREADY, 3>), dim3((unsigned)nblk), dim3(256), lds, stream, p);
+  else hipLaunchKernelGGL((flash_attn_d72_kernel<ABL_QREADY, 2>), dim3((unsigned)nblk), dim3(256), lds, stream, p);
+  return hipGetLastError() == hipSuccess ? 0 : VSYS_ERR_LAUNCH;
+}
+
+}
diff --git a/videosys_amd/csrc/attention_w64.hip b/videosys_amd/csrc/attention_w64.hip
--- a/videosys_amd/csrc/attention_w64.hip
+++ b/videosys_amd/csrc/attention_w64.hip
@@ -171,9 +171,10 @@
   return ((unsigned long long)hi_ << 32) | lo;
 }
 
-template <bool STAMP, bool SM = false>
+template <bool STAMP, bool SM = false, bool QR = false>
 __global__ __launch_bounds__(256, 1) void flash_attn_d72_w64p_kernel(FlashW64Params p, int total_items) {
 #if __HIP_DEVICE_COMPILE__
+  static_assert(!QR || (!SM && !STAMP), "Q ready: the plain statement only");
   extern __shared__ __attribute__((aligned(16))) char smem[];
   const int tid = threadIdx.x, lane = tid & 63, wave = tid >> 6;
   const int l31 = lane & 31, hi = lane >> 5;
@@ -243,7 +244,7 @@
 #pragma unroll
   for (int c = 0; c < 5; ++c) {
     const int d0 = 16 * c + 8 * hi;
-    qnw[c] = (p.q_norm_w != nullptr && d0 < HD) ? *reinterpret_cast<const uint4*>(p.q_norm_w + d0) : make_uint4(0, 0, 0, 0);
+    qnw[c] = (!QR && p.q_norm_w != nullptr && d0 < HD) ? *reinterpret_cast<const uint4*>(p.q_norm_w + d0) : make_uint4(0, 0, 0, 0);
   }
   unsigned long long acc[8] = {0, 0, 0, 0, 0, 0, 0, 0}, ta = 0, tb = 0;
   int ring = 0;
@@ -265,6 +266,11 @@
       for (int c = 0; c < 5; ++c) {
         const int ch = 2 * c + hi;
         qraw[c] = ch < 9 ? *reinterpret_cast<const uint4*>(qimg + ch * 1024) : make_uint4(0, 0, 0, 0);
+      }
+      if constexpr (QR) {
+#pragma unroll
+        for (int c = 0; c < 5; ++c) qw[blk][c] = qraw[c];
+        continue;
       }
       float x[5][8];
       float ss = 0.f;
@@ -433,4 +439,15 @@
 #undef W64_CASE
 }
 
-}
+int launch_flash_attn_d72_w64p_qready(const bf16_t* q, int64_t q_stride, const bf16_t* kp, const bf16_t* vt, bf16_t* out,
+                                      int64_t out_stride, int batch, int heads, int q_len, int kv_len, int kv_pad, hipStream_t stream) {
+  const FlashW64Params p = w64_params(q, q_stride, nullptr, kp, vt, out, out_stride, heads, q_len, kv_len, kv_pad, 0.f, 0.f, nullptr);
+  const int64_t total = (int64_t)p.nqb * batch * heads;
+  if (total > 0x7fffffff) return VSYS_ERR_SHAPE;
+  const int ncu = cu_count_this_device();
+  const unsigned grid = (unsigned)(total < ncu ? total : ncu);
+  const size_t lds = (size_t)W64_STAGES * KV_STAGE + 4 * W64P_QIMG;
+  return w64::launch<flash_attn_d72_w64p_kernel<false, false, true>>(grid, lds, stream, p, (int)total);
+}
+
+}
diff --git a/videosys_amd/csrc/capi.hip b/videosys_amd/csrc/capi.hip
--- a/videosys_amd/csrc/capi.hip
+++ b/videosys_amd/csrc/capi.hip
@@ -154,6 +154,32 @@
   p.kp = B16(kp); p.vt = B16(vt); p.k_norm_w = B16(k_norm_w); p.kv_S = (int)S_; p.kv_heads = (int)heads; p.k_eps = k_eps;
   p.kscale = 0.11785113019775793f * 1.4426950408889634f;
   return launch_gemm_qkv_kv(p, S(stream));
+}
+
+int vsys_gemm_bf16_ln_qkv_q(const void* x, int64_t ldx, const void* wp, int64_t ldw, const void* cs, const void* cv, const void* stats,
+                            int64_t stats_ld, const void* k_norm_w, const void* q_norm_w, void* q, int64_t ldq, void* kp, void* vt,
+                            int64_t M, int64_t K, int64_t S_, int64_t heads, float eps, float k_eps, float q_eps, void* stream) {
+  if (!x || !wp || !cs || !cv || !stats || !k_norm_w || !q_norm_w || !q || !kp || !vt) return VSYS_ERR_ARG;
+  if (!fits_int(M, K, S_) || heads <= 0 || heads > 4096) return VSYS_ERR_SHAPE;
+  if (K % LN_BLOCK != 0 || K / LN_BLOCK > 12) return VSYS_ERR_SHAPE;
+  GemmParams p = gemm_head(x, ldx, wp, ldw, nullptr, q, ldq, M, 216 * heads, K);
+  p.cs = reinterpret_cast<const float*>(cs); p.cv = reinterpret_cast<const float*>(cv);
+  p.ln_stats = reinterpret_cast<const float2*>(stats); p.ln_ld = stats_ld; p.ln_nb = (int)(K / LN_BLOCK); p.ln_eps = eps;
+  p.kp = B16(kp); p.vt = B16(vt); p.k_norm_w = B16(k_norm_w); p.kv_S = (int)S_; p.kv_heads = (int)heads; p.k_eps = k_eps;
+  p.kscale = 0.11785113019775793f * 1.4426950408889634f;
+  p.q_norm_w = B16(q_norm_w); p.q_eps = q_eps;
+  return launch_gemm_qkv_q(p, S(stream));
+}
+
+int vsys_flash_attn_d72_qready(const void* q, int64_t q_stride, const void* kp, const void* vt, void* out, int64_t out_stride,
+                               int64_t batch, int64_t heads, int64_t q_len, int64_t kv_len, int64_t kv_pad, int64_t form, void* stream) {
+  if (!q || !kp || !vt || !out) return VSYS_ERR_ARG;
+  if (!fits_int(batch, heads, q_len, kv_len, kv_pad) || batch * heads > 65535 || form < 0 || form > 1) return VSYS_ERR_SHAPE;
+  for (const void* ptr : {q, kp, vt})
+    if (reinterpret_cast<uintptr_t>(ptr) & 15) return VSYS_ERR_ALIGN;
+  if (reinterpret_cast<uintptr_t>(out) & 7) return VSYS_ERR_ALIGN;
+  return launch_flash_attn_d72_qready(B16(q), q_stride, B16(kp), B16(vt), B16(out), out_stride, (int)batch, (int)heads, (int)q_len,
+                                      (int)kv_len, (int)kv_pad, (int)form, S(stream));
 }
 
 int vsys_gemm_bf16_ln_qkv_kv_dispatched(int64_t M, int64_t N, int64_t K) { return gemm_ln_qkv_kv_dispatched(M, N, K) ? 1 : 0; }
diff --git a/videosys_amd/csrc/common.h b/videosys_amd/csrc/common.h
--- a/videosys_amd/csrc/common.h
+++ b/videosys_amd/csrc/common.h
@@ -71,6 +71,31 @@
     }
 #pragma unroll
     for (int e = 0; e < 24; ++e) x[e] *= kscale;
+  }
+};
+
+struct QNorm72 {
+  static __device__ __forceinline__ float rstd(const uint4* pc, float eps) {
+    float ss[2] = {0.f, 0.f};
+#pragma unroll
+    for (int hi = 0; hi < 2; ++hi)
+#pragma unroll
+      for (int c = 0; 2 * c + hi < 9; ++c) {
+        float x[8];
+        unpack8(pc[2 * c + hi], x);
+#pragma unroll
+        for (int e = 0; e < 8; ++e) ss[hi] += x[e] * x[e];
+      }
+    const float tot = ss[0] + ss[1];
+    return rsqrtf(tot / 72.0f + eps);
+  }
+  static __device__ __forceinline__ uint4 apply(const uint4& piece, float rstd_, const uint4& w8) {
+    float x[8], w[8];
+    unpack8(piece, x);
+    unpack8(w8, w);
+#pragma unroll
+    for (int e = 0; e < 8; ++e) x[e] = bf2f(f2bf(x[e] * rstd_)) * w[e];
+    return pack8(x);
   }
 };
 
diff --git a/videosys_amd/csrc/gemm2_bf16.hip b/videosys_amd/csrc/gemm2_bf16.hip
--- a/videosys_amd/csrc/gemm2_bf16.hip
+++ b/videosys_amd/csrc/gemm2_bf16.hip
@@ -37,6 +37,8 @@
   const int l15 = lane & 15, lq = lane >> 4;
   static_assert(!MF || (EPI != EPI_F32_SLICES && !STAMP), "the 16x16x32 form covers the token-row epilogues only");
   static_assert(EPI != EPI_LN_QKV_KV || (MF && NWN == 2), "the K/V epilogue exists on the 256 x 192 tile of the 16x16x32 form only");
+  static_assert(EPI != EPI_LN_QKV_Q || (MF && NWN == 2), "the Q/K/V epilogue exists on the 256 x 192 tile of the 16x16x32 form only");
+  constexpr bool QKE = EPI == EPI_LN_QKV_Q;
   const int wave_u = __builtin_amdgcn_readfirstlane(wave);
   const int nbn = p.N / BN;
   int tile = xcd_remap(blockIdx.x, gridDim.x);
@@ -96,7 +98,7 @@
 #pragma unroll
       for (int r = 0; r < 4; ++r) acc16[i][j][r] = 0.f;
 
-  constexpr bool LN = EPI == EPI_LN_BIAS || EPI == EPI_LN_GELU || EPI == EPI_LN_QKV_KV;
+  constexpr bool LN = EPI == EPI_LN_BIAS || EPI == EPI_LN_GELU || EPI == EPI_LN_QKV_KV || QKE;
   float2* ln_lds = reinterpret_cast<float2*>(smem + G::LDS_BYTES);
   const int nt = (EPI == EPI_F32_SLICES ? (p.ks < p.K - kslice * p.ks ? p.ks : p.K - kslice * p.ks) : p.K) / BK;
 #pragma unroll
@@ -114,8 +116,12 @@
   if constexpr (LN) {
     __builtin_amdgcn_sched_barrier(0);
     ln_stage_tile(ln_lds, p.ln_stats, p.ln_ld, p.ln_nb, p.ln_eps, p.M, row0, BM, p.cs, p.cv, col0, BN, tid, G::NT);
-    if constexpr (EPI == EPI_LN_QKV_KV) {
+    if constexpr (EPI == EPI_LN_QKV_KV || QKE) {
       if (tid < 9) *reinterpret_cast<uint4*>(smem + G::LDS_BYTES + G::LN_BYTES + tid * 16) = *reinterpret_cast<const uint4*>(p.k_norm_w + tid * 8);
+    }
+    if constexpr (QKE) {
+      if (tid >= 64 && tid < 73)
+        *reinterpret_cast<uint4*>(smem + G::LDS_BYTES + G::LN_BYTES + G::KW_BYTES + (tid - 64) * 16) = *reinterpret_cast<const uint4*>(p.q_norm_w + (tid - 64) * 8);
     }
     __builtin_amdgcn_sched_barrier(0);
   }
@@ -548,16 +554,43 @@
     }
     asm volatile("s_waitcnt lgkmcnt(0)" ::: "memory");
     __builtin_amdgcn_wave_barrier();
-    if constexpr (EPI == EPI_LN_QKV_KV) {
-      const int H = p.kv_heads, nq = (H * 3) >> 2;
+    if constexpr (EPI == EPI_LN_QKV_KV || QKE) {
+      const int H = p.kv_heads, nq = QKE ? 0 : (H * 3) >> 2;
       const int win = __builtin_amdgcn_readfirstlane(ncol0 / 96);
-      if (win >= nq) {
+      if (QKE || win >= nq) {
         if (wrow0 < p.M) {
           const int bt = __builtin_amdgcn_readfirstlane(wrow0 / p.kv_S), key0 = __builtin_amdgcn_readfirstlane(wrow0 - bt * p.kv_S);
-          int vf0 = 24 * H + 96 * (win - nq - H);
-          if (win < nq + H) {
-            const int h = win - nq;
-            vf0 = 24 * h;
+          int vf0 = QKE ? 48 * H + 96 * (win - 2 * H) : 24 * H + 96 * (win - nq - H);
+          const bool headwin = QKE ? win < 2 * H : win < nq + H;
+          if (QKE && win < H) {
+            vf0 = 24 * win;
+            char* rowp = st + lane * OUT_ROW_BYTES;
+            const uint4* wl = reinterpret_cast<const uint4*>(smem + G::LDS_BYTES + G::LN_BYTES + G::KW_BYTES);
+            uint4 qq[9];
+#pragma unroll
+            for (int c = 0; c < 9; ++c) qq[c] = *reinterpret_cast<const uint4*>(rowp + c * 16);
+            const float rstd = QNorm72::rstd(qq, p.q_eps);
+#pragma unroll
+            for (int c = 0; c < 9; ++c) *reinterpret_cast<uint4*>(rowp + c * 16) = QNorm72::apply(qq[c], rstd, wl[c]);
+            asm volatile("s_waitcnt lgkmcnt(0)" ::: "memory");
+            __builtin_amdgcn_wave_barrier();
+            bf16_t* qdst = p.out + (int64_t)wrow0 * p.ldo + win * 72;
+            uint4 qv[9];
+#pragma unroll
+            for (int it = 0; it < 9; ++it) {
+              const int q = lane + 64 * it;
+              const int m_local = q / 9, c = q - m_local * 9;
+              qv[it] = *reinterpret_cast<const uint4*>(st + m_local * OUT_ROW_BYTES + c * 16);
+            }
+#pragma unroll
+            for (int it = 0; it < 9; ++it) {
+              const int q = lane + 64 * it;
+              const int m_local = q / 9, c = q - m_local * 9;
+              *reinterpret_cast<uint4*>(qdst + (int64_t)m_local * p.ldo + c * 8) = qv[it];
+            }
+          } else if (headwin) {
+            const int h = QKE ? win - H : win - nq;
+            vf0 = QKE ? 24 * win : 24 * h;
             char* rowp = st + lane * OUT_ROW_BYTES;
             const uint4* wl = reinterpret_cast<const uint4*>(smem + G::LDS_BYTES + G::LN_BYTES);
             uint4 kk[9];
@@ -598,7 +631,7 @@
 #pragma unroll
             for (int it = 0; it < 9; ++it) *reinterpret_cast<uint4*>(kdst + (lane + 64 * it) * 8) = kq[it];
           }
-          const bool kwin = win < nq + H;
+          const bool kwin = headwin;
           bf16_t* vdst = p.vt + (int64_t)bt * H * 96 * p.kv_S + key0;
 #pragma unroll
           for (int g = 0; g < 3; ++g) {
@@ -717,25 +750,30 @@
   return hipGetLastError() == hipSuccess ? 0 : VSYS_ERR_LAUNCH;
 }
 
-int launch_gemm2_qkv_kv(const GemmParams& p_, hipStream_t stream) {
+template <int EPI>
+static int launch_gemm2_qkv_t(const GemmParams& p_, hipStream_t stream) {
   using G = G2<2>;
+  constexpr bool QKE = EPI == EPI_LN_QKV_Q;
   if (p_.M <= 0) return 0;
   GemmParams p = p_;
   const int H = p.kv_heads;
   if (H <= 0 || H % 8 != 0 || p.N != 216 * H || p.kv_S <= 0 || p.kv_S % 64 != 0 || p.M % p.kv_S != 0 || p.K <= 0 || p.K % BK != 0)
     return VSYS_ERR_SHAPE;
   if (!p.cs || !p.cv || !p.ln_stats || p.ln_nb < 1 || p.ln_nb > 12 || p.ln_nb * LN_BLOCK != p.K || p.ln_ld < p.M) return VSYS_ERR_SHAPE;
-  if (!p.out || !p.kp || !p.vt || !p.k_norm_w || p.ldo < 72 * H) return VSYS_ERR_ARG;
+  if (!p.out || !p.kp || !p.vt || !p.k_norm_w || p.ldo < 72 * H || (QKE && !p.q_norm_w)) return VSYS_ERR_ARG;
   if ((p.lda % 8) || (p.ldw % 8) || (p.ldo % 8) || ((uintptr_t)p.kp % 16) || ((uintptr_t)p.vt % 16) || ((uintptr_t)p.k_norm_w % 16)) return VSYS_ERR_ALIGN;
+  if (QKE && (((uintptr_t)p.out % 16) || ((uintptr_t)p.q_norm_w % 16))) return VSYS_ERR_ALIGN;
   if (p.lda * 512 + (int64_t)p.K * 2 >= 0x7fffffff || p.ldw * 384 + (int64_t)p.K * 2 >= 0x7fffffff) return VSYS_ERR_SHAPE;
-  constexpr int LDS = G::LDS_BYTES + G::LN_BYTES + G::KW_BYTES;
+  constexpr int LDS = G::LDS_BYTES + G::LN_BYTES + (QKE ? 2 : 1) * G::KW_BYTES;
   static std::atomic<unsigned long long> attr_seen{0};
   for (DeviceOnce once(attr_seen); once.todo(); once.done())
-    (void)hipFuncSetAttribute((const void*)gemm2_kernel<EPI_LN_QKV_KV, 2, 0, 1>, hipFuncAttributeMaxDynamicSharedMemorySize, LDS);
+    (void)hipFuncSetAttribute((const void*)gemm2_kernel<EPI, 2, 0, 1>, hipFuncAttributeMaxDynamicSharedMemorySize, LDS);
   const int grid = ((p.M + BM - 1) / BM) * (p.N / G::BN);
-  hipLaunchKernelGGL((gemm2_kernel<EPI_LN_QKV_KV, 2, 0, 1>), dim3(grid), dim3(G::NT), LDS, stream, p);
+  hipLaunchKernelGGL((gemm2_kernel<EPI, 2, 0, 1>), dim3(grid), dim3(G::NT), LDS, stream, p);
   return hipGetLastError() == hipSuccess ? 0 : VSYS_ERR_LAUNCH;
 }
+int launch_gemm2_qkv_kv(const GemmParams& p, hipStream_t stream) { return launch_gemm2_qkv_t<EPI_LN_QKV_KV>(p, stream); }
+int launch_gemm2_qkv_q(const GemmParams& p, hipStream_t stream) { return launch_gemm2_qkv_t<EPI_LN_QKV_Q>(p, stream); }
 
 #ifdef VSYS_LAB
 int launch_gemm2_stamp(const GemmParams& p_, hipStream_t stream) {
diff --git a/videosys_amd/csrc/gemm_bf16.hip b/videosys_amd/csrc/gemm_bf16.hip
--- a/videosys_amd/csrc/gemm_bf16.hip
+++ b/videosys_amd/csrc/gemm_bf16.hip
@@ -1259,13 +1259,15 @@
 bool gemm_ln_qkv_kv_dispatched(int64_t M, int64_t N, int64_t K) {
   return N > 0 && N % BN == 0 && K > 0 && K % BK == 0 && ln_on_two_workgroup_tile(M, N, K) && mf16_default();
 }
-int launch_gemm_qkv_kv(const GemmParams& p_, hipStream_t stream) {
+static GemmParams with_library_raster(const GemmParams& p_) {
   GemmParams p = p_;
   const int ras = g_gemm_raster_a.load(std::memory_order_relaxed);
   p.raster_gw = ras / 100;
   p.raster_ph = ras % 100;
-  return launch_gemm2_qkv_kv(p, stream);
-}
+  return p;
+}
+int launch_gemm_qkv_kv(const GemmParams& p, hipStream_t stream) { return launch_gemm2_qkv_kv(with_library_raster(p), stream); }
+int launch_gemm_qkv_q(const GemmParams& p, hipStream_t stream) { return launch_gemm2_qkv_q(with_library_raster(p), stream); }
 
 int launch_gemm(const GemmParams& p_, int epi, hipStream_t stream) {
   if (p_.M <= 0) return 0;
diff --git a/videosys_amd/csrc/gen/program_gen.py b/videosys_amd/csrc/gen/program_gen.py
--- a/videosys_amd/csrc/gen/program_gen.py
+++ b/videosys_amd/csrc/gen/program_gen.py
@@ -11,7 +11,8 @@
 NO_OP = {"vsys_vae_first_im2col_nc", "vsys_pixels_to_u8", "vsys_clip_attention_d64", "vsys_splitk_reduce_bias_act",
          "vsys_attn_temporal_d64_img", "vsys_attn_prep_kv96", "vsys_flash_attn_d96", "vsys_upsample_trilinear2x",
          "vsys_cfg_ancestral_step", "vsys_pixels_to_u8_trunc", "vsys_attn_prep_kv96_img", "vsys_flash_attn_d96_img",
-         "vsys_attn_prep_kv_rope", "vsys_flash_attn_d72_rope", "vsys_upsample_time2x", "vsys_cfg_pndm_step"}
+         "vsys_attn_prep_kv_rope", "vsys_flash_attn_d72_rope", "vsys_upsample_time2x", "vsys_cfg_pndm_step",
+         "vsys_gemm_bf16_ln_qkv_q", "vsys_flash_attn_d72_qready"}
 BEGIN, END = "/* >>> VSYS_OP codes (generated: csrc/gen/program_gen.py) */", "/* <<< VSYS_OP codes */"
 
 
diff --git a/videosys_amd/csrc/vsys_internal.h b/videosys_amd/csrc/vsys_internal.h
--- a/videosys_amd/csrc/vsys_internal.h
+++ b/videosys_amd/csrc/vsys_internal.h
@@ -46,6 +46,7 @@
        EPI_LN_BIAS = 3, EPI_LN_GELU = 4,
        EPI_GATE_RES_STATS = 5,
        EPI_LN_QKV_KV = 6,
+       EPI_LN_QKV_Q = 7,
        EPI_F32_SLICES = 100  };
 constexpr int LN_BLOCK = 96;
 enum { ACT_NONE = VSYS_ACT_NONE, ACT_SILU = VSYS_ACT_SILU, ACT_GELU_TANH = VSYS_ACT_GELU_TANH };
@@ -56,12 +57,14 @@
   const bf16_t* bias = nullptr;
   bf16_t* out = nullptr; int64_t ldo = 0;
   int M = 0, N = 0, K = 0;
-  const bf16_t* gate = nullptr; int64_t gate_stride = 0;
+  union { const bf16_t* gate = nullptr; const bf16_t* q_norm_w; };
+  int64_t gate_stride = 0;
   const bf16_t* res = nullptr; int64_t ldr = 0;
   bf16_t* aux = nullptr; int64_t ldaux = 0;
   int rows_per_sample = 0;
   int seg_split = 0; int64_t gate_alt = 0;
-  int ks = 0; float* out32 = nullptr; int64_t slab = 0, ldo32 = 0;
+  union { int ks = 0; float q_eps; };
+  float* out32 = nullptr; int64_t slab = 0, ldo32 = 0;
   const float* cs = nullptr; const float* cv = nullptr;
   const float2* ln_stats = nullptr; int64_t ln_ld = 0; int ln_nb = 0; float ln_eps = 0.f;
   float2* stats_out = nullptr; int64_t stats_ld = 0;
@@ -78,6 +81,13 @@
   if (n < 2 * C) return (nq + (n - C) / 72) * 96 + (n - C) % 72;
   const int f = n - 2 * C;
   return f < 24 * heads ? (nq + f / 24) * 96 + 72 + f % 24 : (nq + heads) * 96 + (f - 24 * heads);
+}
+
+__host__ __device__ inline int qkv_q_column(int n, int heads) {
+  const int C = 72 * heads;
+  if (n < 2 * C) return (n / 72) * 96 + n % 72;
+  const int f = n - 2 * C;
+  return f < 48 * heads ? (f / 24) * 96 + 72 + f % 24 : 2 * heads * 96 + (f - 48 * heads);
 }
 
 struct ConvParams {
@@ -151,6 +161,8 @@
 int launch_gemm2(const GemmParams& p, int epi, int wide, hipStream_t stream);
 int launch_gemm2_qkv_kv(const GemmParams& p, hipStream_t stream);
 int launch_gemm_qkv_kv(const GemmParams& p, hipStream_t stream);
+int launch_gemm2_qkv_q(const GemmParams& p, hipStream_t stream);
+int launch_gemm_qkv_q(const GemmParams& p, hipStream_t stream);
 bool gemm_ln_qkv_kv_dispatched(int64_t M, int64_t N, int64_t K);
 int launch_gemm2_slices(const GemmParams& p, int slices, hipStream_t stream);
 int launch_gemm3(const GemmParams& p, int epi, hipStream_t stream);
@@ -237,6 +249,10 @@
 int launch_flash_attn_d72_rope(const bf16_t* q, int64_t q_stride, const float* rope_cos, const float* rope_sin, const bf16_t* kp,
                                const bf16_t* vt, bf16_t* out, int64_t out_stride, int batch, int heads, int q_len, int kv_len,
                                int kv_pad, hipStream_t stream);
+int launch_flash_attn_d72_qready(const bf16_t* q, int64_t q_stride, const bf16_t* kp, const bf16_t* vt, bf16_t* out, int64_t out_stride,
+                                 int batch, int heads, int q_len, int kv_len, int kv_pad, int form, hipStream_t stream);
+int launch_flash_attn_d72_w64p_qready(const bf16_t* q, int64_t q_stride, const bf16_t* kp, const bf16_t* vt, bf16_t* out,
+                                      int64_t out_stride, int batch, int heads, int q_len, int kv_len, int kv_pad, hipStream_t stream);
 int launch_attn_prep_kv96(const bf16_t* k, int64_t k_stride, const bf16_t* v, int64_t v_stride, const float* rope_cos,
                           const float* rope_sin, bf16_t* kp, bf16_t* vt, int batch, int heads, int kv_len, int kv_pad,
                           hipStream_t stream);
diff --git a/videosys_amd/ops.py b/videosys_amd/ops.py
--- a/videosys_amd/ops.py
+++ b/videosys_amd/ops.py
@@ -358,7 +358,11 @@
     vt[:, :, HEAD_DIM + 4] = 1.0
 
 
-def gemm_ln_qkv_kv(x, wp, cs, cv, stats, k_norm_w, q, kp, vt, S, heads, eps=1e-6, k_eps=1e-6):
+def gemm_ln_qkv_kv(x, wp, cs, cv, stats, k_norm_w, q, kp, vt, S, heads, eps=1e-6, k_eps=1e-6, q_norm_w=None, q_eps=1e-6):
+    if q_norm_w is not None:
+        from . import q_ready_ops
+
+        return q_ready_ops.gemm_ln_qkv_q(x, wp, cs, cv, stats, k_norm_w, q_norm_w, q, kp, vt, S, heads, eps, k_eps, q_eps)
     _chk(x, wp, cs, cv, stats, k_norm_w, q, kp, vt)
     _bf16(x, wp, k_norm_w, q, kp, vt)
     assert x.dim() == 2 and x.stride(1) == 1 and wp.stride(1) == 1 and q.stride(1) == 1 and cs.dtype == torch.float32 and cv.dtype == torch.float32
diff --git a/videosys_amd/q_ready_ops.py b/videosys_amd/q_ready_ops.py
--- /dev/null
+++ b/videosys_amd/q_ready_ops.py
@@ -0,0 +1,63 @@
+from __future__ import annotations
+
+import os
+
+import torch
+
+from .open_sora_plan_ops import _issue
+from .ops import HEAD_DIM, LN_BLOCK, VT_ROWS, _bf16, _chk, _stats_ld
+
+FORM_ROWS32, FORM_STREAM = 0, 1
+ORDER_BIT = 1 << 48
+
+
+def _q_ready_default() -> int:
+    v = os.environ.get("VSYS_Q_READY", "1")
+    return int(v) if v in ("0", "1", "2") else 1
+
+
+Q_READY = _q_ready_default()
+
+
+def qkv_q_column_order(heads: int) -> torch.Tensor:
+    assert heads > 0 and heads % 4 == 0
+    C = 72 * heads
+    n = torch.arange(3 * C, dtype=torch.int64)
+    f = n - 2 * C
+    vcol = torch.where(f < 48 * heads, (f // 24) * 96 + 72 + f % 24, 2 * heads * 96 + (f - 48 * heads))
+    return torch.where(n < 2 * C, (n // 72) * 96 + n % 72, vcol)
+
+
+def stream_takes(batch: int, heads: int, q_len: int, kv_len: int, device) -> bool:
+    ncu = torch.cuda.get_device_properties(device).multi_processor_count
+    return kv_len >= 512 and kv_len % 64 == 0 and q_len >= 256 and batch * heads * ((q_len + 255) // 256) >= 4 * ncu
+
+
+def gemm_ln_qkv_q(x, wp, cs, cv, stats, k_norm_w, q_norm_w, q, kp, vt, S, heads, eps=1e-6, k_eps=1e-6, q_eps=1e-6):
+    _chk(x, wp, cs, cv, stats, k_norm_w, q_norm_w, q, kp, vt)
+    _bf16(x, wp, k_norm_w, q_norm_w, q, kp, vt)
+    assert x.dim() == 2 and x.stride(1) == 1 and wp.stride(1) == 1 and q.stride(1) == 1 and cs.dtype == torch.float32 and cv.dtype == torch.float32
+    M, K = x.shape
+    assert wp.shape == (216 * heads, K) and cs.numel() == cv.numel() == 216 * heads
+    assert k_norm_w.numel() == HEAD_DIM and k_norm_w.is_contiguous() and q_norm_w.numel() == HEAD_DIM and q_norm_w.is_contiguous()
+    assert S > 0 and M % S == 0 and q.shape[0] == M and q.shape[1] >= HEAD_DIM * heads and kp.is_contiguous() and vt.is_contiguous()
+    assert tuple(kp.shape) == (M // S, heads, S, HEAD_DIM) and tuple(vt.shape) == (M // S, heads, VT_ROWS, S)
+    ld = _stats_ld(stats, M, K // LN_BLOCK)
+    _issue("vsys_gemm_bf16_ln_qkv_q", (x, wp, cs, cv, stats, k_norm_w, q_norm_w, q, kp, vt),
+           (x.data_ptr(), x.stride(0), wp.data_ptr(), wp.stride(0), cs.data_ptr(), cv.data_ptr(), stats.data_ptr(), ld, k_norm_w.data_ptr(),
+            q_norm_w.data_ptr(), q.data_ptr(), q.stride(0), kp.data_ptr(), vt.data_ptr(), M, K, S, heads, float(eps), float(k_eps),
+            float(q_eps)))
+    return q
+
+
+def flash_attn_qready(q, kp, vt, out, batch, heads, q_len, kv_len, form=FORM_ROWS32):
+    _chk(q, kp, vt, out)
+    _bf16(q, kp, vt, out)
+    assert q.dim() == 2 and out.dim() == 2 and q.stride(1) == 1 and out.stride(1) == 1
+    assert q.shape[0] >= batch * q_len and out.shape[0] >= batch * q_len and q.shape[1] >= heads * HEAD_DIM and out.shape[1] >= heads * HEAD_DIM
+    kv_pad = kp.shape[-2]
+    assert kp.numel() == batch * heads * kv_pad * HEAD_DIM and vt.numel() == batch * heads * VT_ROWS * kv_pad and kv_len <= kv_pad
+    _issue("vsys_flash_attn_d72_qready", (q, kp, vt, out),
+           (q.data_ptr(), q.stride(0), kp.data_ptr(), vt.data_ptr(), out.data_ptr(), out.stride(0), batch, heads, q_len, kv_len, kv_pad,
+            int(form)))
+    return out
diff --git a/videosys_amd/stdit3.py b/videosys_amd/stdit3.py
--- a/videosys_amd/stdit3.py
+++ b/videosys_amd/stdit3.py
@@ -8,6 +8,7 @@
 import torch
 
 from . import dsp, ops, pab, program
+from . import q_ready_ops as qops
 from .utils import same_tensor
 from .workspace import Workspace
 
@@ -144,6 +145,7 @@
         self.adaln_fold = os.environ.get("VSYS_ADALN_FOLD", "1") != "0"
         self.fold_spatial_qkv = True
         self.fused_kv = ops.FUSED_KV
+        self.q_ready = qops.Q_READY
         self._fold = None
         self._stats_fresh = False
         self._programs = {}
@@ -337,8 +339,9 @@
 
     def _fused_kv_ok(self, N, S):
         C, H = self.hidden_size, self.num_heads
-        return bool(self.fused_kv and self._sp is None and self.fold_spatial_qkv and C == 72 * H and H % 8 == 0 and S % 64 == 0
-                    and ops.gemm_ln_qkv_kv_dispatched(N, 3 * C, C))
+        ok = bool(self.fused_kv and self._sp is None and self.fold_spatial_qkv and C == 72 * H and H % 8 == 0 and S % 64 == 0
+                  and ops.gemm_ln_qkv_kv_dispatched(N, 3 * C, C))
+        return (2 if self.q_ready else 1) if ok else 0
 
     def _fold_tables(self, B, fused_kv=False):
         f = self._fold or None
@@ -358,6 +361,8 @@
                 Wp, cs, cv = bufs[name]
                 base = i * B * 6 * C
                 order = self.num_heads << 32 if (fused_kv and i % 2 == 0 and s_sh == 0) else 0
+                if order and fused_kv == 2:
+                    order |= qops.ORDER_BIT
                 rows.append([W.data_ptr(), b.data_ptr(), Wp.data_ptr(), cs.data_ptr(), cv.data_ptr(), base + s_sh, base + s_sc,
                              N | order, K, blk])
                 blk += -(-N // 4)
@@ -433,7 +438,7 @@
             out = self._forward_device(xz, ts_host.to(dev), static, plan, timestep_int, valid_depth, cp, x_mask, fold=fold)
         else:
             sp = self._sp
-            key = (B, Tx, Hx, Wx, float(height[0]), float(width[0]), fkey, valid_depth, cp, fold, self.fold_spatial_qkv, self.fused_kv,
+            key = (B, Tx, Hx, Wx, float(height[0]), float(width[0]), fkey, valid_depth, cp, fold, self.fold_spatial_qkv, self.fused_kv, self.q_ready,
                    None if plan is None else tuple(d[:2] + d[5:7] for d in plan),
                    None if static[0]["varlen"] is None else static[0]["varlen"].lens,
                    None if sp is None else (sp.P, sp.rank, self._scatter, self._switch, self._overlap))
@@ -663,7 +668,8 @@
                 Wp_, cs_, cv_ = ftab["bufs"][p + ".attn.qkv"]
                 kp, vt = self._kv_spatial(B * T, S, constant_rows=True)
                 q = _buf("qkv", (N, 3 * C)).view(-1)[:N * C].view(N, C)
-                ops.gemm_ln_qkv_kv(x, Wp_, cs_, cv_, stats, w[p + ".attn.k_norm.weight"], q, kp, vt, S, H)
+                ops.gemm_ln_qkv_kv(x, Wp_, cs_, cv_, stats, w[p + ".attn.k_norm.weight"], q, kp, vt, S, H,
+                                   q_norm_w=w[p + ".attn.q_norm.weight"] if ftab["fused_kv"] == 2 else None)
             elif fold_attn and sp_order is None:
                 qkv = folded(p + ".attn.qkv", False, _buf("qkv", (N, 3 * C)))
             elif not fold_attn:
@@ -680,7 +686,11 @@
                 ops.attn_temporal(qkv, C, w[p + ".attn.q_norm.weight"], w[p + ".attn.k_norm.weight"], cos, sin, ao, B, T, S, H)
             elif fused_kv:
                 ao = _buf("attn_out", (N, C))
-                ops.flash_attn(q, w[p + ".attn.q_norm.weight"], kp, vt, ao, B * T, H, S, S, k_norm_bound=self._kbound(p))
+                if ftab["fused_kv"] == 2:
+                    stream = self.q_ready == 2 and qops.stream_takes(B * T, H, S, S, x.device)
+                    qops.flash_attn_qready(q, kp, vt, ao, B * T, H, S, S, qops.FORM_STREAM if stream else qops.FORM_ROWS32)
+                else:
+                    ops.flash_attn(q, w[p + ".attn.q_norm.weight"], kp, vt, ao, B * T, H, S, S, k_norm_bound=self._kbound(p))
             elif sp is None:
                 if not fold_attn:
                     qkv = ops.gemm(xm, w[p + ".attn.qkv.weight"], w[p + ".attn.qkv.bias"], out=_buf("qkv", (N, 3 * C)))
```

Result: no change. 21.18 videos/min, median of 6 (+0.5%).
